# byungsook/neural-flow-style

Measured on AMD Instinct MI355X. Metric: stylization iters/sec on 200^3 smoke grid, 8 views, higher is better.
Workload: dtype f32 (3xbf16 split-limb MFMA, f32 accumulate)

## Files before the change

include/nfs_hip.h:

```cpp
#ifndef NFS_HIP_H
#define NFS_HIP_H

#include <stdint.h>

#ifdef __cplusplus
extern "C" {
#endif

#define NFS_OK 0
#define NFS_EINVAL (-1)
#define NFS_ELAUNCH (-2)

typedef void* nfs_stream_t;

int nfs_version(void);
const char* nfs_last_error(void);
int nfs_device_cus(void);
int nfs_gemm_timer(int enable);

int nfs_gemm_mode(int mode);
int nfs_gemm_force(int variant, int bm, int bn, int nbuf, int pre);
int nfs_gemm_last(long long* out);
int nfs_gemm_timer_read(double* ms_total, double* flops_total, long long* launches);
int nfs_gemm_timer_read_kind(int split_limb, double* ms_total, double* flops_total, long long* launches,
                             double* bytes_total);

int nfs_warp3d_fwd(const float* imgs, const float* coords, float* out,
                   int B, int X, int Y, int Z, int C, nfs_stream_t stream);
int nfs_warp3d_bwd(const float* imgs, const float* coords, const float* g_out,
                   float* g_imgs_acc, float* g_coords,
                   int B, int X, int Y, int Z, int C, nfs_stream_t stream);

int nfs_rotate_fwd(const float* d, const float* rot, float* out,
                   int V, int D, int H, int W, int C, nfs_stream_t stream);
int nfs_rotate_bwd(const float* g_out, const float* rot, float* g_d_acc,
                   int V, int D, int H, int W, int C, float* workspace, const float* g_max,
                   int overwrite, nfs_stream_t stream);

int nfs_advect_fwd(const float* d, const float* vel, float* out,
                   int D, int H, int W, int C, nfs_stream_t stream);
int nfs_advect_bwd(const float* d, const float* vel, const float* g_out,
                   float* g_d_acc, float* g_vel,
                   int D, int H, int W, int C, nfs_stream_t stream);

int nfs_advect_bwd_adam(const float* d, float* vel, const float* g_out, float* m, float* v,
                        int D, int H, int W, float lr_t, float beta1, float beta2, float eps,
                        nfs_stream_t stream);

int nfs_advect_bwd_adam_fwd(const float* d, float* vel, const float* g_out, float* m, float* v, float* adv_next,
                            int D, int H, int W, float lr_t, float beta1, float beta2, float eps,
                            nfs_stream_t stream);

int nfs_advect_fwd_slab(const float* d, const float* vel, float* out, int D, int H, int W, int z0, int nz,
                        nfs_stream_t stream);
int nfs_advect_bwd_adam_slab(const float* d, float* vel, const float* g_out, float* m, float* v,
                             int D, int H, int W, int z0, int nz, float lr_t, float beta1, float beta2, float eps,
                             nfs_stream_t stream);
int nfs_advect_bwd_adam_fwd_slab(const float* d, float* vel, const float* g_out, float* m, float* v, float* adv_next,
                                 int D, int H, int W, int z0, int nz, float lr_t, float beta1, float beta2,
                                 float eps, nfs_stream_t stream);

int nfs_hist_loss(const float* feat, const float* templ, float* loss_acc, float* g_acc,
                  int B, int Bt, int HW, int HWt, int C, float weight, int relu_mask, nfs_stream_t stream);
int nfs_hist_loss_masked(const float* feat, const float* templ, const float* mask, float* loss_acc, float* g_acc,
                         int B, int Bt, int HW, int HWt, int C, float weight, int relu_mask, nfs_stream_t stream);
int64_t nfs_hist_loss_wide_workspace_floats(int B, int C, int HW, int HWt);
int nfs_hist_loss_wide(const float* feat, const float* templ, const float* mask, float* loss_acc, float* g_acc,
                       float* workspace, int64_t workspace_floats, int B, int Bt, int HW, int HWt, int C, float weight,
                       int relu_mask, nfs_stream_t stream);

int nfs_resize_bicubic_tf1(const float* x, float* out, int B, int H, int W, int C, int oh, int ow,
                           nfs_stream_t stream);
int nfs_style_mask_apply(const float* F, const float* mask, float* Fm, float* scale, int B, int HW, int C,
                         nfs_stream_t stream);
int nfs_style_mask_bwd(const float* dFm, const float* mask, const float* F, float* dF, int B, int HW, int C,
                       nfs_stream_t stream);

int nfs_warp2d_fwd(const float* imgs, const float* coords, float* out, int B, int X, int Y, int C,
                   nfs_stream_t stream);
int nfs_warp2d_bwd(const float* imgs, const float* coords, const float* g_out, float* g_imgs_acc,
                   float* g_coords, int B, int X, int Y, int C, nfs_stream_t stream);

int nfs_advect2d_fwd(const float* d, const float* vel, float* out, int H, int W, int C, nfs_stream_t stream);
int nfs_advect2d_bwd(const float* d, const float* vel, const float* g_out, float* g_d_acc, float* g_vel,
                     int H, int W, int C, nfs_stream_t stream);

int nfs_advect_maccormack(const float* d, const float* vel, const float* d_fwd, float* out,
                          int D, int H, int W, int C, int nd, nfs_stream_t stream);
int nfs_maccormack_mask_words(int D, int H, int W, int C);
int nfs_advect_maccormack_keep(const float* d, const float* vel, const float* d_fwd, float* out, unsigned long long* keep,
                               int D, int H, int W, int C, int nd, nfs_stream_t stream);
int64_t nfs_advect_maccormack_bwd_workspace_floats(int D, int H, int W, int C, int nd);
int nfs_advect_maccormack_bwd(const float* d, const float* vel, const float* d_fwd, const unsigned long long* keep,
                              const float* g_out, float* g_d_acc, float* g_vel, float* workspace, int64_t workspace_floats,
                              int D, int H, int W, int C, int nd, nfs_stream_t stream);

int nfs_curl_fwd(const float* s, float* out, int D, int H, int W, int nd, nfs_stream_t stream);
int nfs_curl_bwd(const float* g_out, float* g_s, int D, int H, int W, int nd, nfs_stream_t stream);

int nfs_advect_stream_fwd(const float* d, const float* s, float* out, unsigned long long* live,
                          int D, int H, int W, nfs_stream_t stream);
int nfs_advect_stream_bwd(const float* d, const float* s, const float* g_out, float* g_vel,
                          int D, int H, int W, nfs_stream_t stream);
int nfs_stream_bwd_adam(const float* g_vel, float* s, float* m, float* v, int D, int H, int W,
                        float lr_t, float beta1, float beta2, float eps, nfs_stream_t stream);

int nfs_lap_down(const float* x, const float* k, float* out, int D, int H, int W, int C, int nd, nfs_stream_t stream);
int nfs_lap_up(const float* lo, const float* k, float scale, const float* addend, float* out,
               int D, int H, int W, int C, int nd, nfs_stream_t stream);
int nfs_lap_up_rms_parts(int D, int H, int W, int C, int nd);
int nfs_lap_up_rms(const float* lo, const float* k, float scale, const float* addend, const float* addend_part,
                   int addend_nparts, int64_t addend_n, float eps, float* out, float* out_part, int D, int H, int W, int C,
                   int nd, nfs_stream_t stream);
int nfs_normalize_mean(const float* x, float* out, int64_t n, int use_abs, float eps, float* workspace, int ws_floats,
                       nfs_stream_t stream);

int nfs_transport_step(const float* g, const float* u, float scale, float w_g, const float* addend,
                       float w_addend, float* out, int D, int H, int W, int C, nfs_stream_t stream);

int nfs_smooth3d_relu_fwd(const float* d, float* out, int D, int H, int W, float k,
                          nfs_stream_t stream);
int nfs_smooth3d_relu_bwd(const float* out, const float* g_out, float* g_d,
                          int D, int H, int W, float k, nfs_stream_t stream);

int nfs_render_fwd(const float* d, float* img, float* raysum,
                   int V, int D, int H, int W, float tau, int liquid, nfs_stream_t stream);
int nfs_render_bwd(const float* d, const float* raysum, const float* g_img, float* g_d,
                   int V, int D, int H, int W, float tau, int liquid, float* gmax_out,
                   nfs_stream_t stream);

int nfs_rotate_render_fwd(const float* d, const float* rot, float* img, float* raysum, float* d_rot,
                          int V, int D, int H, int W, float tau, int liquid,
                          nfs_stream_t stream);
int nfs_rotate_render_bwd(const float* d, const float* rot, const float* raysum,
                          const float* g_img, float* g_d_acc,
                          int V, int D, int H, int W, float tau, int liquid,
                          nfs_stream_t stream);

int nfs_render_coef_layout(int V, int D, int H, int W, int* nseg, int* seg_len);
int nfs_rotate_render_fwd_coef(const float* d, const float* rot, float* img, float* raysum, float* u_rot, float* seg,
                               int V, int D, int H, int W, float tau, nfs_stream_t stream);
int nfs_render_ray_coef_bounds(int V, int H, int W);
int nfs_render_ray_coef(const float* g_img, const float* seg, float* ab, float* bounds,
                        int V, int H, int W, float tau, nfs_stream_t stream);
int nfs_rotate_bwd_coef(const float* u_rot, const float* ab, const float* rot, float* g_d_acc,
                        int V, int D, int H, int W, int nseg, int seg_len, const float* bounds, int nbounds,
                        int overwrite, nfs_stream_t stream);

int nfs_live_mask_words(int D, int H, int W);
int nfs_advect_fwd_live(const float* d, const float* vel, float* out, unsigned long long* live,
                        int D, int H, int W, nfs_stream_t stream);
int nfs_advect_bwd_adam_fwd_live(const float* d, float* vel, const float* g_out, float* m, float* v, float* adv_next,
                                 unsigned long long* live_next, int D, int H, int W, float lr_t, float beta1,
                                 float beta2, float eps, nfs_stream_t stream);
int nfs_advect_bwd_adam_fwd_live_ever(const float* d, float* vel, const float* g_out, float* m, float* v, float* adv_next,
                                      unsigned long long* live, unsigned long long* ever, int D, int H, int W,
                                      float lr_t, float beta1, float beta2, float eps, nfs_stream_t stream);
int nfs_rotate_bwd_coef_live(const float* u_rot, const float* ab, const float* rot, float* g_d_acc,
                             int V, int D, int H, int W, int nseg, int seg_len, const float* bounds, int nbounds,
                             int overwrite, const unsigned long long* live, int dilate, int* workspace,
                             nfs_stream_t stream);
int nfs_rotate_live_workspace_ints(int D, int H, int W);

int nfs_maxnorm_fwd(const float* img, float* out, float* gmax, int G, int n,
                    nfs_stream_t stream);
int nfs_maxnorm_bwd(const float* img, const float* gmax, const float* g_out, float* g_img,
                    int G, int n, float* workspace, nfs_stream_t stream);
int nfs_maxnorm_input_fwd(const float* img, float* x, float* gmax, int G, int n, nfs_stream_t stream);
int nfs_maxnorm_input_bwd(const float* img, const float* gmax, const float* g_x, float* g_img, int G, int n,
                          float* workspace, nfs_stream_t stream);


int nfs_loss_net_input_fwd(const float* img, float* d_img, float* x,
                           int B, int H, int W, int Cin, int H2, int W2, nfs_stream_t stream);
int nfs_loss_net_input_bwd(const float* g_x, float* g_img,
                           int B, int H, int W, int Cin, int H2, int W2, nfs_stream_t stream);

int64_t nfs_conv3x3_packed_floats(int Ci, int Co, int kind);
int nfs_conv3x3_pack(const float* w_hwio, float* packed, int Ci, int Co, int kind,
                     nfs_stream_t stream);
int64_t nfs_conv3x3_workspace_floats(int B, int H, int W, int Ci, int Co);
int64_t nfs_conv3x3_relu_bits_words(int B, int H, int W, int Ci, int Co, int pooled);
double nfs_conv3x3_executed_flops(int B, int H, int W, int K, int N, int pooled);
int nfs_conv3x3_fwd(const float* x, const float* packed_fwd, const float* bias, float* y,
                    int B, int H, int W, int Ci, int Co, int relu,
                    float* workspace, int64_t workspace_floats, uint32_t* relu_bits,
                    nfs_stream_t stream);
int nfs_conv3x3_dgrad(const float* gy, const float* packed_dgrad, const float* x_in,
                      const float* addend, float* gx,
                      int B, int H, int W, int Ci, int Co,
                      float* workspace, int64_t workspace_floats, const uint32_t* relu_bits,
                      int addend_unmasked, nfs_stream_t stream);
int nfs_conv3x3_fwd_pool(const float* x, const float* packed_fwd, const float* bias, float* y,
                         float* y_pool, int B, int H, int W, int Ci, int Co, int relu,
                         float* workspace, int64_t workspace_floats, uint32_t* relu_bits,
                         nfs_stream_t stream);
int nfs_conv3x3_dgrad_pool(const float* gy_pool, const float* x_out, const float* packed_dgrad,
                           const float* x_in, const float* addend, float* gx,
                           int B, int H, int W, int Ci, int Co,
                           float* workspace, int64_t workspace_floats, const uint32_t* relu_bits,
                           int addend_unmasked, nfs_stream_t stream);
int nfs_avgpool2_fwd(const float* x, float* y, int B, int H, int W, int C, nfs_stream_t stream);
int nfs_avgpool2_bwd(const float* gy, const float* x, const float* addend, float* gx,
                     int B, int H, int W, int C, nfs_stream_t stream);

int64_t nfs_gram_workspace_floats(int B, int HW, int C);
int nfs_gram_fwd(const float* F, float* G, int B, int HW, int C, const float* scale_dev, float scale,
                 float* workspace, int64_t workspace_floats, nfs_stream_t stream);
int nfs_style_loss_fwd(const float* G, const float* Gs, float* loss_acc, float* Dmat,
                       int B, int Bs, int C, float weight, nfs_stream_t stream);
int nfs_gram_bwd(const float* F, const float* Dmat, float* dF, int B, int HW, int C,
                 const float* scale_dev, float scale, int relu_mask, nfs_stream_t stream);

typedef struct {
  const float* F;
  const float* Gs;
  float* G;
  float* Dmat;
  float* dF;
  int B, Bs, HW, C;
  float scale;
  float weight;
  int relu_mask;
} nfs_gram_layer_t;
int64_t nfs_gram_style_group_workspace_floats(const nfs_gram_layer_t* layers, int n);
int nfs_gram_style_group_parts(const nfs_gram_layer_t* layers, int n);
int nfs_gram_style_group_fwd(const nfs_gram_layer_t* layers, int n, float* loss_parts, float* workspace,
                             int64_t workspace_floats, nfs_stream_t stream);
int nfs_gram_group_bwd(const nfs_gram_layer_t* layers, int n, nfs_stream_t stream);

int nfs_content_loss(const float* F, const float* target, float* loss_acc, float* g_acc, int B, int Bt,
                     int HW, int C, int channel, int mode, float weight, float amp, nfs_stream_t stream);
int nfs_content_loss_signed(const float* F, const float* target, float* loss_acc, float* g_acc, int B, int Bt,
                            int HW, int C, int channel, int mode, float weight, float amp, nfs_stream_t stream);

int64_t nfs_conv2d_packed_floats(int kh, int kw, int Ci, int Co, int transpose);
int nfs_conv2d_pack(const float* w_hwio, float* packed, int kh, int kw, int Ci, int Co, int transpose,
                    nfs_stream_t stream);
int64_t nfs_conv2d_workspace_floats(int B, int H, int W, int Cin, int Cout, int kh, int kw, int stride);
int nfs_conv2d_fwd(const float* x, int ldx, const float* x_mask, int ldm, const float* packed, const float* bias,
                   float* y, int ldy, float* y_pre, int ldp, int B, int H, int W, int Cin, int Cout, int kh, int kw,
                   int stride, int relu, int accumulate, float* workspace, int64_t workspace_floats,
                   nfs_stream_t stream);
typedef struct {
  const float* x;
  const float* x_mask;
  const float* packed;
  const float* bias;
  float* y;
  float* y_pre;
  int ldx, ldm, ldy, ldp;
  int H, W, Cin, Cout, kh, kw;
  int relu, accumulate, sum_with_prev;
} nfs_conv2d_desc_t;
int64_t nfs_conv2d_group_workspace_floats(const nfs_conv2d_desc_t* descs, int n, int B);
int nfs_conv2d_group(const nfs_conv2d_desc_t* descs, int n, int B, float* workspace, int64_t workspace_floats,
                     nfs_stream_t stream);
int nfs_conv2d_dgrad_small(const float* gy, int ldg, const float* y_act, int lda, const float* w_hwio, float* gx,
                           int B, int H, int W, int Ci, int Co, int kh, int kw, int stride, nfs_stream_t stream);
int nfs_maxpool3_fwd(const float* x, float* y, uint8_t* arg, int B, int H, int W, int C, int stride,
                     nfs_stream_t stream);
int nfs_maxpool3_bwd(const float* gy, const uint8_t* arg, float* gx, int B, int H, int W, int C, int stride,
                     int accumulate, const float* relu_of, nfs_stream_t stream);
int nfs_lrn_fwd(const float* x, float* y, float* scale, int64_t npix, int C, int ld, int radius, float bias,
                float alpha, float beta, nfs_stream_t stream);
int nfs_lrn_bwd(const float* x, const float* y, const float* scale, const float* gy, float* gx, int64_t npix, int C,
                int ld, int radius, float alpha, float beta, int accumulate, nfs_stream_t stream);
int nfs_avgpool_valid_fwd(const float* x, float* y, int B, int H, int W, int C, int k, nfs_stream_t stream);
int nfs_avgpool_valid_bwd(const float* gy, float* gx, int B, int H, int W, int C, int k, int accumulate,
                          nfs_stream_t stream);
int nfs_relu_mask_add(const float* g, int ldg, const float* act, int lda, const float* addend, int ldadd, float* out,
                      int ldo, int64_t npix, int C, nfs_stream_t stream);

int nfs_tv_loss(const float* d_img, float* loss_acc, float* g_acc, int B, int H, int W, int C,
                float weight, nfs_stream_t stream);

typedef struct {
  int nd;
  int res[3];
  float domain[3];
  float radius, support, rest_density;
  int nsize, clip, mode;
} nfs_splat_cfg;
int nfs_p2g_fwd(const float* p, const float* attr, const float* pd, float* grid, float* wsum,
                int N, int C, const nfs_splat_cfg* cfg_host, nfs_stream_t stream);
int nfs_p2g_bwd(const float* p, const float* attr, const float* pd, const float* g_grid,
                const float* g_wsum, float* g_p, float* g_attr, float* g_pd,
                int N, int C, const nfs_splat_cfg* cfg_host, nfs_stream_t stream);
int nfs_p2g_wavg_finish(const float* xsum, const float* wsum, float* out, int64_t n, int C,
                        float eps, nfs_stream_t stream);
int nfs_p2g_wavg_bwd(const float* p, const float* attr, const float* xsum, const float* wsum, const float* g_out,
                     float* g_p, float* g_attr, int N, int C, float eps, const nfs_splat_cfg* cfg_host,
                     nfs_stream_t stream);
int nfs_p2g_wavg_finish_bwd(const float* xsum, const float* wsum, const float* g_out,
                            float* g_xsum, float* g_wsum, int64_t n, int C, float eps,
                            nfs_stream_t stream);
int nfs_p2g_has_instance(const nfs_splat_cfg* cfg_host);

int nfs_g2p_fwd(const float* g, const float* p, float* out, int nd, int X, int Y, int Z, int C,
                int64_t N, int cubic, nfs_stream_t stream);

int nfs_adam_tf_step(float* x, float* m, float* v, const float* g, int64_t n,
                     float lr_t, float beta1, float beta2, float eps, nfs_stream_t stream);

int nfs_fill(float* x, float value, int64_t n, nfs_stream_t stream);
int nfs_axpy(float* y, const float* x, float a, int64_t n, nfs_stream_t stream);

int nfs_colour_clamp_gather(const float* var, const long long* order, float* out, int64_t N, int C, nfs_stream_t stream);
int nfs_clamp01_bwd(const float* g, const float* x, float* out, int64_t n, nfs_stream_t stream);
int nfs_colour_clamp_scatter_bwd(const float* g_cc, const long long* order, const float* var, float* g_var, int64_t N,
                                 int C, nfs_stream_t stream);
int nfs_iterate_update(float* x, float* g_opt, int64_t n, nfs_stream_t stream);

int nfs_slab_pack(const float* gpad, float* pack, int D, int64_t plane, int world, int cs, nfs_stream_t stream);

#ifdef __cplusplus
}
#endif
#endif
```

neural-flow-style_amd/_lib.py:

```python
from __future__ import annotations

import ctypes as C
import os
import subprocess

_HERE = os.path.dirname(os.path.abspath(__file__))
LIB_PATH = os.environ.get("NFS_LIB_PATH") or os.path.join(_HERE, "libnfs_hip.so")
CSRC_DIR = os.path.join(_HERE, "csrc")


class NfsLibraryError(RuntimeError):
    pass


NFS_EINVAL, NFS_ELAUNCH = -1, -2


class NfsError(RuntimeError):

    def __init__(self, name, code, msg):
        RuntimeError.__init__(self, "%s failed (%d): %s" % (name, code, msg))
        self.name, self.code = name, int(code)


class SplatCfg(C.Structure):
    _fields_ = [("nd", C.c_int), ("res", C.c_int * 3), ("domain", C.c_float * 3),
                ("radius", C.c_float), ("support", C.c_float), ("rest_density", C.c_float),
                ("nsize", C.c_int), ("clip", C.c_int), ("mode", C.c_int)]


class GramLayer(C.Structure):
    _fields_ = [("F", C.c_void_p), ("Gs", C.c_void_p), ("G", C.c_void_p), ("Dmat", C.c_void_p), ("dF", C.c_void_p),
                ("B", C.c_int), ("Bs", C.c_int), ("HW", C.c_int), ("C", C.c_int),
                ("scale", C.c_float), ("weight", C.c_float), ("relu_mask", C.c_int)]


class ConvDesc(C.Structure):
    _fields_ = [("x", C.c_void_p), ("x_mask", C.c_void_p), ("packed", C.c_void_p), ("bias", C.c_void_p),
                ("y", C.c_void_p), ("y_pre", C.c_void_p),
                ("ldx", C.c_int), ("ldm", C.c_int), ("ldy", C.c_int), ("ldp", C.c_int),
                ("H", C.c_int), ("W", C.c_int), ("Cin", C.c_int), ("Cout", C.c_int), ("kh", C.c_int), ("kw", C.c_int),
                ("relu", C.c_int), ("accumulate", C.c_int), ("sum_with_prev", C.c_int)]


_P, _I, _F, _L = C.c_void_p, C.c_int, C.c_float, C.c_int64

SIGNATURES = {
    "nfs_version": [],
    "nfs_last_error": [],
    "nfs_device_cus": [],
    "nfs_gemm_timer": [_I],
    "nfs_gemm_mode": [_I],
    "nfs_gemm_force": [_I, _I, _I, _I, _I],
    "nfs_gemm_last": [_P],
    "nfs_gemm_timer_read": [_P, _P, _P],
    "nfs_gemm_timer_read_kind": [_I, _P, _P, _P, _P],
    "nfs_warp3d_fwd": [_P, _P, _P, _I, _I, _I, _I, _I, _P],
    "nfs_warp3d_bwd": [_P, _P, _P, _P, _P, _I, _I, _I, _I, _I, _P],
    "nfs_rotate_fwd": [_P, _P, _P, _I, _I, _I, _I, _I, _P],
    "nfs_rotate_bwd": [_P, _P, _P, _I, _I, _I, _I, _I, _P, _P, _I, _P],
    "nfs_advect_fwd": [_P, _P, _P, _I, _I, _I, _I, _P],
    "nfs_advect_bwd": [_P, _P, _P, _P, _P, _I, _I, _I, _I, _P],
    "nfs_advect_bwd_adam": [_P, _P, _P, _P, _P, _I, _I, _I, _F, _F, _F, _F, _P],
    "nfs_advect_fwd_slab": [_P, _P, _P, _I, _I, _I, _I, _I, _P],
    "nfs_advect_bwd_adam_slab": [_P, _P, _P, _P, _P, _I, _I, _I, _I, _I, _F, _F, _F, _F, _P],
    "nfs_advect_bwd_adam_fwd": [_P, _P, _P, _P, _P, _P, _I, _I, _I, _F, _F, _F, _F, _P],
    "nfs_advect_bwd_adam_fwd_slab": [_P, _P, _P, _P, _P, _P, _I, _I, _I, _I, _I, _F, _F, _F, _F, _P],
    "nfs_warp2d_fwd": [_P, _P, _P, _I, _I, _I, _I, _P],
    "nfs_warp2d_bwd": [_P, _P, _P, _P, _P, _I, _I, _I, _I, _P],
    "nfs_advect2d_fwd": [_P, _P, _P, _I, _I, _I, _P],
    "nfs_advect2d_bwd": [_P, _P, _P, _P, _P, _I, _I, _I, _P],
    "nfs_advect_maccormack": [_P, _P, _P, _P, _I, _I, _I, _I, _I, _P],
    "nfs_maccormack_mask_words": [_I, _I, _I, _I],
    "nfs_advect_maccormack_keep": [_P, _P, _P, _P, _P, _I, _I, _I, _I, _I, _P],
    "nfs_advect_maccormack_bwd_workspace_floats": [_I, _I, _I, _I, _I],
    "nfs_advect_maccormack_bwd": [_P, _P, _P, _P, _P, _P, _P, _P, _L, _I, _I, _I, _I, _I, _P],
    "nfs_curl_fwd": [_P, _P, _I, _I, _I, _I, _P],
    "nfs_curl_bwd": [_P, _P, _I, _I, _I, _I, _P],
    "nfs_advect_stream_fwd": [_P, _P, _P, _P, _I, _I, _I, _P],
    "nfs_advect_stream_bwd": [_P, _P, _P, _P, _I, _I, _I, _P],
    "nfs_stream_bwd_adam": [_P, _P, _P, _P, _I, _I, _I, _F, _F, _F, _F, _P],
    "nfs_lap_down": [_P, _P, _P, _I, _I, _I, _I, _I, _P],
    "nfs_lap_up": [_P, _P, _F, _P, _P, _I, _I, _I, _I, _I, _P],
    "nfs_lap_up_rms_parts": [_I, _I, _I, _I, _I],
    "nfs_lap_up_rms": [_P, _P, _F, _P, _P, _I, _L, _F, _P, _P, _I, _I, _I, _I, _I, _P],
    "nfs_normalize_mean": [_P, _P, _L, _I, _F, _P, _I, _P],
    "nfs_transport_step": [_P, _P, _F, _F, _P, _F, _P, _I, _I, _I, _I, _P],
    "nfs_smooth3d_relu_fwd": [_P, _P, _I, _I, _I, _F, _P],
    "nfs_smooth3d_relu_bwd": [_P, _P, _P, _I, _I, _I, _F, _P],
    "nfs_render_fwd": [_P, _P, _P, _I, _I, _I, _I, _F, _I, _P],
    "nfs_render_bwd": [_P, _P, _P, _P, _I, _I, _I, _I, _F, _I, _P, _P],
    "nfs_rotate_render_fwd": [_P, _P, _P, _P, _P, _I, _I, _I, _I, _F, _I, _P],
    "nfs_render_coef_layout": [_I, _I, _I, _I, _P, _P],
    "nfs_rotate_render_fwd_coef": [_P, _P, _P, _P, _P, _P, _I, _I, _I, _I, _F, _P],
    "nfs_render_ray_coef": [_P, _P, _P, _P, _I, _I, _I, _F, _P],
    "nfs_render_ray_coef_bounds": [_I, _I, _I],
    "nfs_rotate_bwd_coef": [_P, _P, _P, _P, _I, _I, _I, _I, _I, _I, _P, _I, _I, _P],
    "nfs_live_mask_words": [_I, _I, _I],
    "nfs_advect_fwd_live": [_P, _P, _P, _P, _I, _I, _I, _P],
    "nfs_advect_bwd_adam_fwd_live": [_P, _P, _P, _P, _P, _P, _P, _I, _I, _I, _F, _F, _F, _F, _P],
    "nfs_advect_bwd_adam_fwd_live_ever": [_P, _P, _P, _P, _P, _P, _P, _P, _I, _I, _I, _F, _F, _F, _F, _P],
    "nfs_rotate_bwd_coef_live": [_P, _P, _P, _P, _I, _I, _I, _I, _I, _I, _P, _I, _I, _P, _I, _P, _P],
    "nfs_rotate_live_workspace_ints": [_I, _I, _I],
    "nfs_rotate_render_bwd": [_P, _P, _P, _P, _P, _I, _I, _I, _I, _F, _I, _P],
    "nfs_maxnorm_fwd": [_P, _P, _P, _I, _I, _P],
    "nfs_maxnorm_bwd": [_P, _P, _P, _P, _I, _I, _P, _P],
    "nfs_maxnorm_input_fwd": [_P, _P, _P, _I, _I, _P],
    "nfs_maxnorm_input_bwd": [_P, _P, _P, _P, _I, _I, _P, _P],
    "nfs_loss_net_input_fwd": [_P, _P, _P, _I, _I, _I, _I, _I, _I, _P],
    "nfs_loss_net_input_bwd": [_P, _P, _I, _I, _I, _I, _I, _I, _P],
    "nfs_conv3x3_packed_floats": [_I, _I, _I],
    "nfs_conv3x3_pack": [_P, _P, _I, _I, _I, _P],
    "nfs_conv3x3_workspace_floats": [_I, _I, _I, _I, _I],
    "nfs_conv3x3_relu_bits_words": [_I, _I, _I, _I, _I, _I],
    "nfs_conv3x3_fwd": [_P, _P, _P, _P, _I, _I, _I, _I, _I, _I, _P, _L, _P, _P],
    "nfs_conv3x3_dgrad": [_P, _P, _P, _P, _P, _I, _I, _I, _I, _I, _P, _L, _P, _I, _P],
    "nfs_conv3x3_fwd_pool": [_P, _P, _P, _P, _P, _I, _I, _I, _I, _I, _I, _P, _L, _P, _P],
    "nfs_conv3x3_dgrad_pool": [_P, _P, _P, _P, _P, _P, _I, _I, _I, _I, _I, _P, _L, _P, _I, _P],
    "nfs_avgpool2_fwd": [_P, _P, _I, _I, _I, _I, _P],
    "nfs_avgpool2_bwd": [_P, _P, _P, _P, _I, _I, _I, _I, _P],
    "nfs_gram_workspace_floats": [_I, _I, _I],
    "nfs_gram_fwd": [_P, _P, _I, _I, _I, _P, _F, _P, _L, _P],
    "nfs_style_loss_fwd": [_P, _P, _P, _P, _I, _I, _I, _F, _P],
    "nfs_content_loss": [_P, _P, _P, _P, _I, _I, _I, _I, _I, _I, _F, _F, _P],
    "nfs_content_loss_signed": [_P, _P, _P, _P, _I, _I, _I, _I, _I, _I, _F, _F, _P],
    "nfs_gram_bwd": [_P, _P, _P, _I, _I, _I, _P, _F, _I, _P],
    "nfs_hist_loss": [_P, _P, _P, _P, _I, _I, _I, _I, _I, _F, _I, _P],
    "nfs_conv3x3_executed_flops": [_I, _I, _I, _I, _I, _I],
    "nfs_conv2d_packed_floats": [_I, _I, _I, _I, _I],
    "nfs_conv2d_pack": [_P, _P, _I, _I, _I, _I, _I, _P],
    "nfs_conv2d_workspace_floats": [_I, _I, _I, _I, _I, _I, _I, _I],
    "nfs_conv2d_fwd": [_P, _I, _P, _I, _P, _P, _P, _I, _P, _I, _I, _I, _I, _I, _I, _I, _I, _I, _I, _I, _P, _L, _P],
    "nfs_conv2d_group_workspace_floats": [_P, _I, _I],
    "nfs_conv2d_group": [_P, _I, _I, _P, _L, _P],
    "nfs_conv2d_dgrad_small": [_P, _I, _P, _I, _P, _P, _I, _I, _I, _I, _I, _I, _I, _I, _P],
    "nfs_maxpool3_fwd": [_P, _P, _P, _I, _I, _I, _I, _I, _P],
    "nfs_maxpool3_bwd": [_P, _P, _P, _I, _I, _I, _I, _I, _I, _P, _P],
    "nfs_lrn_fwd": [_P, _P, _P, _L, _I, _I, _I, _F, _F, _F, _P],
    "nfs_lrn_bwd": [_P, _P, _P, _P, _P, _L, _I, _I, _I, _F, _F, _I, _P],
    "nfs_avgpool_valid_fwd": [_P, _P, _I, _I, _I, _I, _I, _P],
    "nfs_avgpool_valid_bwd": [_P, _P, _I, _I, _I, _I, _I, _I, _P],
    "nfs_relu_mask_add": [_P, _I, _P, _I, _P, _I, _P, _I, _L, _I, _P],
    "nfs_gram_style_group_workspace_floats": [_P, _I],
    "nfs_gram_style_group_parts": [_P, _I],
    "nfs_gram_style_group_fwd": [_P, _I, _P, _P, _L, _P],
    "nfs_gram_group_bwd": [_P, _I, _P],
    "nfs_hist_loss_masked": [_P, _P, _P, _P, _P, _I, _I, _I, _I, _I, _F, _I, _P],
    "nfs_hist_loss_wide_workspace_floats": [_I, _I, _I, _I],
    "nfs_hist_loss_wide": [_P, _P, _P, _P, _P, _P, _L, _I, _I, _I, _I, _I, _F, _I, _P],
    "nfs_resize_bicubic_tf1": [_P, _P, _I, _I, _I, _I, _I, _I, _P],
    "nfs_style_mask_apply": [_P, _P, _P, _P, _I, _I, _I, _P],
    "nfs_style_mask_bwd": [_P, _P, _P, _P, _I, _I, _I, _P],
    "nfs_tv_loss": [_P, _P, _P, _I, _I, _I, _I, _F, _P],
    "nfs_p2g_fwd": [_P, _P, _P, _P, _P, _I, _I, C.POINTER(SplatCfg), _P],
    "nfs_p2g_bwd": [_P, _P, _P, _P, _P, _P, _P, _P, _I, _I, C.POINTER(SplatCfg), _P],
    "nfs_p2g_wavg_finish": [_P, _P, _P, _L, _I, _F, _P],
    "nfs_p2g_wavg_finish_bwd": [_P, _P, _P, _P, _P, _L, _I, _F, _P],
    "nfs_p2g_has_instance": [C.POINTER(SplatCfg)],
    "nfs_p2g_wavg_bwd": [_P, _P, _P, _P, _P, _P, _P, _I, _I, _F, C.POINTER(SplatCfg), _P],
    "nfs_g2p_fwd": [_P, _P, _P, _I, _I, _I, _I, _I, _L, _I, _P],
    "nfs_adam_tf_step": [_P, _P, _P, _P, _L, _F, _F, _F, _F, _P],
    "nfs_fill": [_P, _F, _L, _P],
    "nfs_axpy": [_P, _P, _F, _L, _P],
    "nfs_slab_pack": [_P, _P, _I, _L, _I, _I, _P],
    "nfs_colour_clamp_gather": [_P, _P, _P, _L, _I, _P],
    "nfs_clamp01_bwd": [_P, _P, _P, _L, _P],
    "nfs_colour_clamp_scatter_bwd": [_P, _P, _P, _P, _L, _I, _P],
    "nfs_iterate_update": [_P, _P, _L, _P],
}
_RESTYPE = {"nfs_last_error": C.c_char_p, "nfs_conv3x3_packed_floats": C.c_int64,
            "nfs_conv3x3_workspace_floats": C.c_int64, "nfs_gram_workspace_floats": C.c_int64,
            "nfs_conv3x3_relu_bits_words": C.c_int64, "nfs_gram_style_group_workspace_floats": C.c_int64, "nfs_hist_loss_wide_workspace_floats": C.c_int64,
            "nfs_advect_maccormack_bwd_workspace_floats": C.c_int64,
            "nfs_conv3x3_executed_flops": C.c_double, "nfs_conv2d_packed_floats": C.c_int64,
            "nfs_conv2d_workspace_floats": C.c_int64, "nfs_conv2d_group_workspace_floats": C.c_int64}

_lib = None
ABI_VERSION = 154


def build(verbose=False):
    jobs = os.environ.get("MAX_JOBS") or str(min(os.cpu_count() or 4, 16))
    r = subprocess.run(["make", "-C", CSRC_DIR, "-j", jobs],
                       capture_output=True, text=True)
    if verbose or r.returncode != 0:
        print(r.stdout[-4000:], r.stderr[-4000:])
    if r.returncode != 0:
        raise NfsLibraryError("building libnfs_hip.so failed")
    return LIB_PATH


def lib():
    global _lib
    if _lib is None:
        if not os.path.exists(LIB_PATH):
            raise NfsLibraryError(
                "libnfs_hip.so is missing (%s): run `python -c 'import __graft_entry__ as g; g.build()'` "
                "-- there is no CPU fallback for the product path" % LIB_PATH)
        import torch
        try:
            L = C.CDLL(LIB_PATH)
        except OSError as e:
            raise NfsLibraryError("cannot load %s: %s" % (LIB_PATH, e))
        for name, argt in SIGNATURES.items():
            try:
                f = getattr(L, name)
            except AttributeError:
                raise NfsLibraryError("libnfs_hip.so does not export %s (stale build?)" % name)
            f.argtypes = argt
            f.restype = _RESTYPE.get(name, C.c_int)
        if L.nfs_version() < ABI_VERSION:
            raise NfsLibraryError("libnfs_hip.so reports ABI %d, this binding needs >= %d: rebuild (make -C %s)"
                                  % (L.nfs_version(), ABI_VERSION, CSRC_DIR))
        _lib = L
    return _lib


PROFILE = None


def call(name, *args):
    L = lib()
    if PROFILE is not None:
        import torch
        e0 = torch.cuda.Event(enable_timing=True); e1 = torch.cuda.Event(enable_timing=True)
        e0.record()
        rc = getattr(L, name)(*args)
        e1.record()
        PROFILE.setdefault(name, []).append((e0, e1, args))
    else:
        rc = getattr(L, name)(*args)
    if rc != 0:
        raise NfsError(name, rc, L.nfs_last_error().decode())
    return rc
```

neural-flow-style_amd/csrc/api.hip:

```cpp
#include "common.h"

namespace nfs {
static thread_local char g_err[512] = "";
void set_error(const char* fmt, ...) {
  va_list ap;
  va_start(ap, fmt);
  vsnprintf(g_err, sizeof(g_err), fmt, ap);
  va_end(ap);
}
}

extern "C" {
int nfs_version(void) { return 154; }
const char* nfs_last_error(void) { return nfs::g_err; }
int nfs_device_cus(void) {
  int dev = 0;
  hipDeviceProp_t p;
  if (hipGetDevice(&dev) != hipSuccess || hipGetDeviceProperties(&p, dev) != hipSuccess) {
    nfs::set_error("nfs_device_cus: no HIP device");
    return NFS_ELAUNCH;
  }
  return p.multiProcessorCount;
}
}
```

neural-flow-style_amd/csrc/gram.hip:

```cpp
#include "common.h"

namespace nfs {

typedef float f32x16 __attribute__((ext_vector_type(16)));

struct GramArgs {
  const float* F;
  float* G;
  float* ws;
  const float* scale_dev;
  float scale;
  int B, HW, C;
  int ts;
  int cps;
  int nslab;
  int ntile;
  const float* Gs = nullptr;
  float* Dmat = nullptr;
  float* part = nullptr;
  float weight = 0.f;
  int Bs = 1;
  int slot0 = 0;
};

constexpr int GR_MAXL = 8;
struct GramGroupArgs {
  GramArgs L[GR_MAXL];
  int ustart[GR_MAXL + 1];
  int n;
};

constexpr int GR_KC = 32;

template <int TS>
__device__ __forceinline__ void gram_tn_block(const GramArgs& a, float* smem, int block, int nblocks) {
  constexpr int MT = TS / 64;
  constexpr int J = TS / 32;
  constexpr int R4 = TS / 4;
  float* As = smem;
  float* Bs = smem + 2 * GR_KC * TS;
  const int t = threadIdx.x, lane = t & 63, wid = t >> 6;
  const int wm = wid >> 1, wn = wid & 1, i = lane & 31, h = lane >> 5;
  const int npair = a.ntile * (a.ntile + 1) / 2;
  const int64_t per_xcd = nblocks / 8;
  int64_t unit = (int64_t)(block % 8) * per_xcd + block / 8;
  const int64_t per_img = (int64_t)a.nslab * npair;
  if (unit >= per_img * a.B) return;
  const int b = (int)(unit / per_img);
  unit -= (int64_t)b * per_img;
  const int sl = (int)(unit / npair);
  const int pair = (int)(unit - (int64_t)sl * npair);
  int t1 = 0, t2 = pair;
  while (t2 >= a.ntile - t1) { t2 -= a.ntile - t1; ++t1; }
  t2 += t1;
  const bool diag = t1 == t2;
  const int total_chunks = (a.HW + GR_KC - 1) / GR_KC;
  const int c_begin = sl * a.cps;
  const int nchunks = min(a.cps, total_chunks - c_begin);
  const float* Fb = a.F + (int64_t)b * a.HW * a.C;

  const int col4 = t % R4, row0 = t / R4;
  constexpr int RSTEP = 256 / R4;
  const float* ga = Fb + t1 * TS + 4 * col4;
  const float* gb = Fb + t2 * TS + 4 * col4;
  float4 a0, a1, a2, a3, b0, b1, b2, b3;
#define NFS_GR_LD(dst_, base_, j_, c_)                                                          \
  {                                                                                             \
    const int p_ = (c_begin + (c_)) * GR_KC + row0 + RSTEP * (j_);                              \
    dst_ = make_float4(0.f, 0.f, 0.f, 0.f);                                                     \
    if (p_ < a.HW) dst_ = *reinterpret_cast<const float4*>(base_ + (int64_t)p_ * a.C);          \
  }
#define NFS_GR_LOAD(c_)                                                                         \
  {                                                                                             \
    NFS_GR_LD(a0, ga, 0, c_) NFS_GR_LD(a1, ga, 1, c_)                                           \
    if (J > 2) { NFS_GR_LD(a2, ga, 2, c_) NFS_GR_LD(a3, ga, 3, c_) }                            \
    if (!diag) {                                                                                \
      NFS_GR_LD(b0, gb, 0, c_) NFS_GR_LD(b1, gb, 1, c_)                                         \
      if (J > 2) { NFS_GR_LD(b2, gb, 2, c_) NFS_GR_LD(b3, gb, 3, c_) }                          \
    }                                                                                           \
  }
  b0 = b1 = b2 = b3 = make_float4(0.f, 0.f, 0.f, 0.f);
  a2 = a3 = b0;
  NFS_GR_LOAD(0)

  f32x16 acc[MT][MT];
#pragma unroll
  for (int x = 0; x < MT; ++x)
#pragma unroll
    for (int y = 0; y < MT; ++y)
#pragma unroll
      for (int r = 0; r < 16; ++r) acc[x][y][r] = 0.f;

  const int afrag = h * TS + wm * (TS / 2) + i;
  const int bfrag = h * TS + wn * (TS / 2) + i;
  for (int c = 0; c < nchunks; ++c) {
    float* Ac = As + (c & 1) * GR_KC * TS;
    float* Bc = diag ? Ac : Bs + (c & 1) * GR_KC * TS;
    {
      float* ad = Ac + row0 * TS + 4 * col4;
      *reinterpret_cast<float4*>(ad) = a0;
      *reinterpret_cast<float4*>(ad + RSTEP * TS) = a1;
      if (J > 2) {
        *reinterpret_cast<float4*>(ad + 2 * RSTEP * TS) = a2;
        *reinterpret_cast<float4*>(ad + 3 * RSTEP * TS) = a3;
      }
      if (!diag) {
        float* bd = Bc + row0 * TS + 4 * col4;
        *reinterpret_cast<float4*>(bd) = b0;
        *reinterpret_cast<float4*>(bd + RSTEP * TS) = b1;
        if (J > 2) {
          *reinterpret_cast<float4*>(bd + 2 * RSTEP * TS) = b2;
          *reinterpret_cast<float4*>(bd + 3 * RSTEP * TS) = b3;
        }
      }
    }
    __syncthreads();
    if (c + 1 < nchunks) NFS_GR_LOAD(c + 1)
#pragma unroll
    for (int st = 0; st < GR_KC / 2; ++st) {
      float af[MT], bf[MT];
#pragma unroll
      for (int m = 0; m < MT; ++m) af[m] = Ac[afrag + 2 * st * TS + 32 * m];
#pragma unroll
      for (int n = 0; n < MT; ++n) bf[n] = Bc[bfrag + 2 * st * TS + 32 * n];
#pragma unroll
      for (int n = 0; n < MT; ++n)
#pragma unroll
        for (int m = 0; m < MT; ++m)
          acc[m][n] = __builtin_amdgcn_mfma_f32_32x32x2f32(af[m], bf[n], acc[m][n], 0, 0, 0);
    }
  }
#undef NFS_GR_LOAD
#undef NFS_GR_LD

  constexpr int OS = TS + 4;
  float* otile = smem;
  __syncthreads();
#pragma unroll
  for (int m = 0; m < MT; ++m)
#pragma unroll
    for (int r = 0; r < 16; ++r) {
      const int row = wm * (TS / 2) + m * 32 + (r & 3) + 8 * (r >> 2) + 4 * h;
#pragma unroll
      for (int n = 0; n < MT; ++n) otile[row * OS + wn * (TS / 2) + n * 32 + i] = acc[m][n][r];
    }
  __syncthreads();
  if (a.ws) {
    float* wt = a.ws + (((int64_t)b * npair + pair) * a.nslab + sl) * TS * TS;
#pragma unroll
    for (int e = 0; e < (TS * R4) / 256; ++e) {
      const int f = t + 256 * e;
      const int row = f / R4, q = f - row * R4;
      *reinterpret_cast<float4*>(wt + row * TS + 4 * q) = *reinterpret_cast<const float4*>(otile + row * OS + 4 * q);
    }
    return;
  }
  const float sc = a.scale * (a.scale_dev ? a.scale_dev[b] : 1.f);
  float* Gb = a.G + (int64_t)b * a.C * a.C;
  if (a.nslab == 1 && a.Dmat) {
    const float* Gsb = a.Gs + (int64_t)(b % a.Bs) * a.C * a.C;
    float* Db = a.Dmat + (int64_t)b * a.C * a.C;
    float* Go = a.G ? a.G + (int64_t)b * a.C * a.C : nullptr;
    const float w2 = 2.f * a.weight;
    float lp = 0.f;
    for (int f = t; f < TS * R4; f += 256) {
      const int row = f / R4, q = f - row * R4;
      const int64_t o = (int64_t)(t1 * TS + row) * a.C + t2 * TS + 4 * q;
      float4 v = *reinterpret_cast<const float4*>(otile + row * OS + 4 * q);
      v.x *= sc; v.y *= sc; v.z *= sc; v.w *= sc;
      if (Go) *reinterpret_cast<float4*>(Go + o) = v;
      const float4 g = *reinterpret_cast<const float4*>(Gsb + o);
      const float4 d = make_float4(v.x - g.x, v.y - g.y, v.z - g.z, v.w - g.w);
      lp += (d.x * d.x + d.y * d.y) + (d.z * d.z + d.w * d.w);
      *reinterpret_cast<float4*>(Db + o) = make_float4(w2 * d.x, w2 * d.y, w2 * d.z, w2 * d.w);
    }
    if (!diag)
      for (int f = t; f < TS * R4; f += 256) {
        const int col = f / R4, q = f - col * R4;
        const float4 v = make_float4(otile[(4 * q) * OS + col] * sc, otile[(4 * q + 1) * OS + col] * sc,
                                     otile[(4 * q + 2) * OS + col] * sc, otile[(4 * q + 3) * OS + col] * sc);
        const int64_t o = (int64_t)(t2 * TS + col) * a.C + t1 * TS + 4 * q;
        if (Go) *reinterpret_cast<float4*>(Go + o) = v;
        const float4 g = *reinterpret_cast<const float4*>(Gsb + o);
        *reinterpret_cast<float4*>(Db + o) = make_float4(w2 * (v.x - g.x), w2 * (v.y - g.y), w2 * (v.z - g.z),
                                                         w2 * (v.w - g.w));
      }
    lp = block_sum(lp, smem + TS * OS);
    if (t == 0) a.part[(int64_t)(a.slot0 + pair) * a.B + b] = a.weight * (diag ? lp : 2.f * lp);
    return;
  }
  if (a.nslab == 1) {
    for (int f = t; f < TS * R4; f += 256) {
      const int row = f / R4, q = f - row * R4;
      float4 v = *reinterpret_cast<const float4*>(otile + row * OS + 4 * q);
      v.x *= sc; v.y *= sc; v.z *= sc; v.w *= sc;
      *reinterpret_cast<float4*>(Gb + (int64_t)(t1 * TS + row) * a.C + t2 * TS + 4 * q) = v;
    }
    if (!diag)
      for (int f = t; f < TS * R4; f += 256) {
        const int col = f / R4, q = f - col * R4;
        const float4 v = make_float4(otile[(4 * q) * OS + col] * sc, otile[(4 * q + 1) * OS + col] * sc,
                                     otile[(4 * q + 2) * OS + col] * sc, otile[(4 * q + 3) * OS + col] * sc);
        *reinterpret_cast<float4*>(Gb + (int64_t)(t2 * TS + col) * a.C + t1 * TS + 4 * q) = v;
      }
    return;
  }
  for (int f = t; f < TS * TS; f += 256) {
    const int row = f / TS, col = f - row * TS;
    const float v = otile[row * OS + col] * sc;
    const int gr = t1 * TS + row, gc = t2 * TS + col;
    atomicAdd(Gb + (int64_t)gr * a.C + gc, v);
    if (!diag) atomicAdd(Gb + (int64_t)gc * a.C + gr, v);
  }
}

template <int TS>
__global__ void __launch_bounds__(256, 2) gram_tn_kernel(GramArgs a) {
  extern __shared__ __attribute__((aligned(16))) float smem[];
  gram_tn_block<TS>(a, smem, (int)blockIdx.x, (int)gridDim.x);
}

__global__ void __launch_bounds__(256, 2) gram_tn_group_kernel(GramGroupArgs g) {
  extern __shared__ __attribute__((aligned(16))) float smem[];
  int l = 0;
  while (l + 1 < g.n && (int)blockIdx.x >= g.ustart[l + 1]) ++l;
  gram_tn_block<64>(g.L[l], smem, (int)blockIdx.x - g.ustart[l], g.ustart[l + 1] - g.ustart[l]);
}

constexpr int GRD_ROWS = 4;
__device__ __forceinline__ void gram_reduce_block(const GramArgs& a, int unit) {
  constexpr int TS = 64;
  __shared__ float4 part[4][64];
  __shared__ float tile[GRD_ROWS][TS + 1];
  const int t = threadIdx.x, lane = t & 63, g = t >> 6;
  const int row = lane >> 4, q = lane & 15;
  constexpr int groups = TS / GRD_ROWS;
  const int npair = a.ntile * (a.ntile + 1) / 2;
  const int rg = unit % groups;
  unit /= groups;
  const int pair = unit % npair, b = unit / npair;
  int t1 = 0, t2 = pair;
  while (t2 >= a.ntile - t1) { t2 -= a.ntile - t1; ++t1; }
  t2 += t1;
  const int64_t tsz = (int64_t)TS * TS;
  const float* p = a.ws + (((int64_t)b * npair + pair) * a.nslab) * tsz + (int64_t)(rg * GRD_ROWS + row) * TS + 4 * q;
  float4 s = make_float4(0.f, 0.f, 0.f, 0.f);
  for (int k = g; k < a.nslab; k += 4) {
    const float4 x = *reinterpret_cast<const float4*>(p + (int64_t)k * tsz);
    s.x += x.x; s.y += x.y; s.z += x.z; s.w += x.w;
  }
  part[g][lane] = s;
  __syncthreads();
  if (g > 0) return;
  const float sc = a.scale * (a.scale_dev ? a.scale_dev[b] : 1.f);
  const float4 p1 = part[1][lane], p2 = part[2][lane], p3 = part[3][lane];
  s.x = ((s.x + p1.x) + (p2.x + p3.x)) * sc; s.y = ((s.y + p1.y) + (p2.y + p3.y)) * sc;
  s.z = ((s.z + p1.z) + (p2.z + p3.z)) * sc; s.w = ((s.w + p1.w) + (p2.w + p3.w)) * sc;
  float* Gb = a.G ? a.G + (int64_t)b * a.C * a.C : nullptr;
  const int64_t o = (int64_t)(t1 * TS + rg * GRD_ROWS + row) * a.C + t2 * TS + 4 * q;
  if (Gb) *reinterpret_cast<float4*>(Gb + o) = s;
  const float* Gsb = a.Dmat ? a.Gs + (int64_t)(b % a.Bs) * a.C * a.C : nullptr;
  float* Db = a.Dmat ? a.Dmat + (int64_t)b * a.C * a.C : nullptr;
  const float w2 = 2.f * a.weight;
  if (Db) {
    const float4 gs = *reinterpret_cast<const float4*>(Gsb + o);
    const float4 d = make_float4(s.x - gs.x, s.y - gs.y, s.z - gs.z, s.w - gs.w);
    *reinterpret_cast<float4*>(Db + o) = make_float4(w2 * d.x, w2 * d.y, w2 * d.z, w2 * d.w);
    const float lp = wave_sum((d.x * d.x + d.y * d.y) + (d.z * d.z + d.w * d.w));
    if (lane == 0) a.part[(int64_t)(a.slot0 + pair * groups + rg) * a.B + b] = a.weight * (t1 == t2 ? lp : 2.f * lp);
  }
  if (t1 == t2) return;
  tile[row][4 * q] = s.x; tile[row][4 * q + 1] = s.y; tile[row][4 * q + 2] = s.z; tile[row][4 * q + 3] = s.w;
  __builtin_amdgcn_s_waitcnt(0xc07f);
  __builtin_amdgcn_wave_barrier();
  const float4 v = make_float4(tile[0][lane], tile[1][lane], tile[2][lane], tile[3][lane]);
  const int64_t om = (int64_t)(t2 * TS + lane) * a.C + t1 * TS + rg * GRD_ROWS;
  if (Gb) *reinterpret_cast<float4*>(Gb + om) = v;
  if (Db) {
    const float4 gs = *reinterpret_cast<const float4*>(Gsb + om);
    *reinterpret_cast<float4*>(Db + om) = make_float4(w2 * (v.x - gs.x), w2 * (v.y - gs.y), w2 * (v.z - gs.z),
                                                      w2 * (v.w - gs.w));
  }
}

__global__ void __launch_bounds__(256) gram_reduce_kernel(GramArgs a) { gram_reduce_block(a, (int)blockIdx.x); }

__global__ void __launch_bounds__(256) gram_reduce_group_kernel(GramGroupArgs g) {
  int l = 0;
  while (l + 1 < g.n && (int)blockIdx.x >= g.ustart[l + 1]) ++l;
  gram_reduce_block(g.L[l], (int)blockIdx.x - g.ustart[l]);
}

__global__ void __launch_bounds__(256) style_loss_kernel(const float* __restrict__ G, const float* __restrict__ Gs,
                                                         float* __restrict__ loss, float* __restrict__ Dmat, int B,
                                                         int Bs, int CC, float weight) {
  __shared__ float red[16];
  const int b = blockIdx.y;
  float part = 0.f;
  for (int64_t e = (int64_t)blockIdx.x * blockDim.x + threadIdx.x; e < CC; e += (int64_t)gridDim.x * blockDim.x) {
    const float diff = G[(int64_t)b * CC + e] - Gs[(int64_t)(b % Bs) * CC + e];
    part += weight * diff * diff;
    Dmat[(int64_t)b * CC + e] = 2.f * weight * diff;
  }
  part = block_sum(part, red);
  if (threadIdx.x == 0) atomicAdd(loss + b, part);
}

__global__ void __launch_bounds__(256) content_loss_kernel(const float* __restrict__ F, const float* __restrict__ target,
                                                           float* __restrict__ loss, float* __restrict__ g_acc,
                                                           int B, int Bt, int64_t HWC, int C, int channel, int mode,
                                                           float weight, float amp, int signed_f) {
  __shared__ float red[16];
  const int b = blockIdx.y;
  const float n_all = (float)B * (float)HWC;
  const float n_pix = n_all / (float)C;
  const float c_on = -weight / n_pix;
  const float c_lo = channel > 0 ? weight / (n_pix * (float)channel) : 0.f;
  const float c_hi = channel + 1 < C ? weight / (n_pix * (float)(C - channel - 1)) : 0.f;
  float part = 0.f;
  for (int64_t e = (int64_t)blockIdx.x * blockDim.x + threadIdx.x; e < HWC; e += (int64_t)gridDim.x * blockDim.x) {
    const int64_t i = (int64_t)b * HWC + e;
    const float f = F[i];
    float l, g;
    if (mode == 0) {
      const int ch = (int)(e % C);
      const float k = ch == channel ? c_on : (ch < channel ? c_lo : c_hi);
      if (ch == channel || !signed_f) {
        l = k * f;
        g = k;
      } else {
        l = k * fabsf(f);
        g = f > 0.f ? k : (f < 0.f ? -k : 0.f);
      }
    } else if (mode == 1) {
      l = -weight / n_all * f;
      g = -weight / n_all;
    } else {
      const float diff = f - amp * target[(int64_t)(b % Bt) * HWC + e];
      l = weight / n_all * diff * diff;
      g = 2.f * weight / n_all * diff;
    }
    part += l;
    if (signed_f || f > 0.f) g_acc[i] += g;
  }
  part = block_sum(part, red);
  if (threadIdx.x == 0) atomicAdd(loss + b, part);
}

int gram_bwd_gemm(const float* F, const float* Dm, float* dF, int B, int HW, int C, float alpha, const float* alpha_dev,
                  int relu_mask, int cus, hipStream_t s);
int gram_bwd_gemm_group(const float* const* F, const float* const* Dm, float* const* dF, const int* HW, const int* C,
                        const float* alpha, const int* relu_mask, int n, int B, hipStream_t s);

}

using namespace nfs;

extern "C" {

static int gram_cus() {
  static int cus = 0;
  if (cus == 0) { const int c = nfs_device_cus(); cus = c > 0 ? c : 256; }
  return cus;
}

static void gram_plan(GramArgs& a, int cus) {
  static const int env_cps = [] { const char* e = getenv("NFS_GRAM_CPS"); return e ? atoi(e) : 0; }();
  a.ts = 64;
  a.ntile = a.C / a.ts;
  const int64_t pairs = (int64_t)a.B * a.ntile * (a.ntile + 1) / 2;
  const int total_chunks = (a.HW + GR_KC - 1) / GR_KC;
  int cps = 16;
  while (cps > 4 && pairs * ((total_chunks + cps - 1) / cps) < 2 * (int64_t)cus) cps >>= 1;
  if (cps > total_chunks) cps = total_chunks;
  if ((total_chunks + cps - 1) / cps > 256) cps = (total_chunks + 255) / 256;
  if (pairs >= cus && total_chunks <= 32) cps = total_chunks;
  if (env_cps > 0) cps = env_cps < total_chunks ? env_cps : total_chunks;
  a.cps = cps;
  a.nslab = (total_chunks + cps - 1) / cps;
}

int64_t nfs_gram_workspace_floats(int B, int HW, int C) {
  if (B <= 0 || HW <= 0 || C <= 0 || C % 64) return 0;
  GramArgs a;
  a.B = B; a.HW = HW; a.C = C;
  gram_plan(a, gram_cus());
  return (int64_t)B * (a.ntile * (a.ntile + 1) / 2) * a.nslab * a.ts * a.ts + 4 * 4096;
}

int nfs_gram_fwd(const float* F, float* G, int B, int HW, int C, const float* scale_dev, float scale,
                 float* workspace, int64_t workspace_floats, nfs_stream_t stream) {
  NFS_REQUIRE(F && G, "nfs_gram_fwd: null pointer");
  NFS_REQUIRE(B > 0 && HW > 0, "nfs_gram_fwd: non-positive dimension");
  NFS_REQUIRE(C > 0 && C % 64 == 0, "nfs_gram_fwd: C must be a multiple of 64");
  GramArgs a;
  a.F = F; a.G = G; a.scale_dev = scale_dev; a.scale = scale; a.B = B; a.HW = HW; a.C = C;
  gram_plan(a, gram_cus());
  const int64_t units = (int64_t)B * (a.ntile * (a.ntile + 1) / 2) * a.nslab;
  a.ws = (workspace && workspace_floats >= nfs_gram_workspace_floats(B, HW, C) && a.nslab > 1) ? workspace : nullptr;
  const size_t lds = 4 * GR_KC * 64 * sizeof(float);
  hipLaunchKernelGGL(gram_tn_kernel<64>, dim3((unsigned)((units + 7) / 8 * 8)), dim3(256), lds, as_stream(stream), a);
  if (a.ws) {
    const unsigned rb = (unsigned)((int64_t)B * (a.ntile * (a.ntile + 1) / 2) * (64 / GRD_ROWS));
    hipLaunchKernelGGL(gram_reduce_kernel, dim3(rb), dim3(256), 0, as_stream(stream), a);
  }
  return check_launch("nfs_gram_fwd");
}

struct GramGroupPlan {
  GramGroupArgs tn, rd;
  int tn_blocks, rd_blocks, parts;
  int64_t ws_floats;
};

static int gram_group_plan(const nfs_gram_layer_t* layers, int n, GramGroupPlan& P) {
  if (!layers || n < 1 || n > GR_MAXL) return -1;
  int order[GR_MAXL];
  GramArgs L[GR_MAXL];
  for (int l = 0; l < n; ++l) {
    const nfs_gram_layer_t& y = layers[l];
    if (!y.F || !y.Gs || !y.Dmat || y.B <= 0 || y.Bs <= 0 || y.HW <= 0 || y.C <= 0 || y.C % 64 || y.B != layers[0].B)
      return -1;
    GramArgs& a = L[l];
    a = GramArgs();
    a.F = y.F; a.G = y.G; a.scale_dev = nullptr; a.scale = y.scale; a.B = y.B; a.HW = y.HW; a.C = y.C;
    a.Gs = y.Gs; a.Dmat = y.Dmat; a.weight = y.weight; a.Bs = y.Bs;
    a.ts = 64;
    a.ntile = y.C / 64;
    const int total_chunks = (y.HW + GR_KC - 1) / GR_KC;
    a.cps = total_chunks <= 32 ? total_chunks : 16;
    a.nslab = (total_chunks + a.cps - 1) / a.cps;
    order[l] = l;
  }
  for (int i = 1; i < n; ++i)
    for (int j = i; j > 0 && (L[order[j]].cps > L[order[j - 1]].cps ||
                              (L[order[j]].cps == L[order[j - 1]].cps && L[order[j]].ntile > L[order[j - 1]].ntile)); --j) {
      const int tmp = order[j]; order[j] = order[j - 1]; order[j - 1] = tmp;
    }
  P.tn.n = n;
  P.rd.n = 0;
  int ub = 0, rb = 0, slot = 0;
  int64_t ws = 0;
  for (int k = 0; k < n; ++k) {
    GramArgs a = L[order[k]];
    const int npair = a.ntile * (a.ntile + 1) / 2;
    a.slot0 = slot;
    a.ws = nullptr;
    P.tn.ustart[k] = ub;
    ub += (int)(((int64_t)a.B * npair * a.nslab + 7) / 8 * 8);
    if (a.nslab > 1) {
      a.ws = reinterpret_cast<float*>(ws * sizeof(float));
      ws += (int64_t)a.B * npair * a.nslab * 64 * 64;
      slot += npair * (64 / GRD_ROWS);
      P.rd.ustart[P.rd.n] = rb;
      rb += a.B * npair * (64 / GRD_ROWS);
      P.rd.L[P.rd.n++] = a;
    } else {
      slot += npair;
    }
    P.tn.L[k] = a;
  }
  P.tn.ustart[n] = ub;
  P.rd.ustart[P.rd.n] = rb;
  P.tn_blocks = ub; P.rd_blocks = rb; P.parts = slot; P.ws_floats = ws;
  return 0;
}

int64_t nfs_gram_style_group_workspace_floats(const nfs_gram_layer_t* layers, int n) {
  GramGroupPlan P;
  return gram_group_plan(layers, n, P) == 0 ? P.ws_floats : -1;
}

int nfs_gram_style_group_parts(const nfs_gram_layer_t* layers, int n) {
  GramGroupPlan P;
  return gram_group_plan(layers, n, P) == 0 ? P.parts : -1;
}

int nfs_gram_style_group_fwd(const nfs_gram_layer_t* layers, int n, float* loss_parts, float* workspace,
                             int64_t workspace_floats, nfs_stream_t stream) {
  GramGroupPlan P;
  NFS_REQUIRE(gram_group_plan(layers, n, P) == 0,
              "nfs_gram_style_group_fwd: 1..8 layers with F, Gs, Dmat set, one batch size, C a multiple of 64");
  NFS_REQUIRE(loss_parts, "nfs_gram_style_group_fwd: null loss_parts");
  NFS_REQUIRE(P.ws_floats == 0 || (workspace && workspace_floats >= P.ws_floats),
              "nfs_gram_style_group_fwd: workspace smaller than nfs_gram_style_group_workspace_floats");
  for (int k = 0; k < n; ++k) {
    P.tn.L[k].part = loss_parts;
    if (P.tn.L[k].nslab > 1) P.tn.L[k].ws = workspace + reinterpret_cast<int64_t>(P.tn.L[k].ws) / (int64_t)sizeof(float);
  }
  for (int k = 0; k < P.rd.n; ++k) {
    P.rd.L[k].part = loss_parts;
    P.rd.L[k].ws = workspace + reinterpret_cast<int64_t>(P.rd.L[k].ws) / (int64_t)sizeof(float);
  }
  const size_t lds = 4 * GR_KC * 64 * sizeof(float);
  hipLaunchKernelGGL(gram_tn_group_kernel, dim3((unsigned)P.tn_blocks), dim3(256), lds, as_stream(stream), P.tn);
  if (P.rd_blocks > 0)
    hipLaunchKernelGGL(gram_reduce_group_kernel, dim3((unsigned)P.rd_blocks), dim3(256), 0, as_stream(stream), P.rd);
  return check_launch("nfs_gram_style_group_fwd");
}

int nfs_gram_group_bwd(const nfs_gram_layer_t* layers, int n, nfs_stream_t stream) {
  NFS_REQUIRE(layers && n >= 1 && n <= GR_MAXL, "nfs_gram_group_bwd: 1..8 layers");
  const float* F[GR_MAXL]; const float* Dm[GR_MAXL]; float* dF[GR_MAXL];
  int HW[GR_MAXL], C[GR_MAXL], mask[GR_MAXL];
  float alpha[GR_MAXL];
  for (int l = 0; l < n; ++l) {
    const nfs_gram_layer_t& y = layers[l];
    NFS_REQUIRE(y.F && y.Dmat && y.dF, "nfs_gram_group_bwd: null pointer");
    NFS_REQUIRE(y.B > 0 && y.B == layers[0].B && y.HW > 0 && y.C > 0 && y.C % 64 == 0,
                "nfs_gram_group_bwd: one batch size, C a multiple of 64");
    F[l] = y.F; Dm[l] = y.Dmat; dF[l] = y.dF; HW[l] = y.HW; C[l] = y.C; mask[l] = y.relu_mask; alpha[l] = 2.f * y.scale;
  }
  NFS_REQUIRE(gram_bwd_gemm_group(F, Dm, dF, HW, C, alpha, mask, n, layers[0].B, as_stream(stream)) == 0,
              "nfs_gram_group_bwd: shape outside the 16-row GEMM's 32-bit operand offsets");
  return 0;
}

int nfs_style_loss_fwd(const float* G, const float* Gs, float* loss_acc, float* Dmat, int B, int Bs, int C,
                       float weight, nfs_stream_t stream) {
  NFS_REQUIRE(G && Gs && loss_acc && Dmat, "nfs_style_loss_fwd: null pointer");
  NFS_REQUIRE(B > 0 && Bs > 0 && C > 0, "nfs_style_loss_fwd: non-positive dimension");
  const int CC = C * C;
  const unsigned nb = blocks_for(CC, 256) < 32u ? blocks_for(CC, 256) : 32u;
  hipLaunchKernelGGL(style_loss_kernel, dim3(nb, B), dim3(256), 0, as_stream(stream), G, Gs, loss_acc, Dmat, B, Bs,
                     CC, weight);
  return check_launch("nfs_style_loss_fwd");
}

static int content_loss_launch(const char* who, const float* F, const float* target, float* loss_acc, float* g_acc, int B,
                               int Bt, int HW, int C, int channel, int mode, float weight, float amp, int signed_f,
                               nfs_stream_t stream) {
  NFS_REQUIRE(F && loss_acc && g_acc, "%s: null pointer", who);
  NFS_REQUIRE(B > 0 && HW > 0 && C > 0, "%s: non-positive dimension", who);
  NFS_REQUIRE(mode >= 0 && mode <= 2, "%s: mode must be 0 (channel), 1 (all) or 2 (target)", who);
  NFS_REQUIRE(mode != 0 || (channel > 0 && channel < C), "%s: channel out of range", who);
  NFS_REQUIRE(mode != 2 || (target && Bt > 0), "%s: mode 2 needs the target features", who);
  const int64_t HWC = (int64_t)HW * C;
  const unsigned nb = blocks_for(HWC, 256) < 64u ? blocks_for(HWC, 256) : 64u;
  hipLaunchKernelGGL(content_loss_kernel, dim3(nb, B), dim3(256), 0, as_stream(stream), F, target, loss_acc, g_acc, B,
                     Bt > 0 ? Bt : 1, HWC, C, channel, mode, weight, amp, signed_f);
  return check_launch(who);
}

int nfs_content_loss(const float* F, const float* target, float* loss_acc, float* g_acc, int B, int Bt, int HW, int C,
                     int channel, int mode, float weight, float amp, nfs_stream_t stream) {
  return content_loss_launch("nfs_content_loss", F, target, loss_acc, g_acc, B, Bt, HW, C, channel, mode, weight, amp, 0,
                             stream);
}

int nfs_content_loss_signed(const float* F, const float* target, float* loss_acc, float* g_acc, int B, int Bt, int HW,
                            int C, int channel, int mode, float weight, float amp, nfs_stream_t stream) {
  return content_loss_launch("nfs_content_loss_signed", F, target, loss_acc, g_acc, B, Bt, HW, C, channel, mode, weight,
                             amp, 1, stream);
}

int nfs_gram_bwd(const float* F, const float* Dmat, float* dF, int B, int HW, int C, const float* scale_dev,
                 float scale, int relu_mask, nfs_stream_t stream) {
  NFS_REQUIRE(F && Dmat && dF, "nfs_gram_bwd: null pointer");
  NFS_REQUIRE(B > 0 && HW > 0, "nfs_gram_bwd: non-positive dimension");
  NFS_REQUIRE(C > 0 && C % 64 == 0, "nfs_gram_bwd: C must be a multiple of 64");
  return gram_bwd_gemm(F, Dmat, dF, B, HW, C, 2.f * scale, scale_dev, relu_mask, gram_cus(), as_stream(stream));
}

}
```

neural-flow-style_amd/csrc/render.hip:

```cpp
#include "common.h"

namespace nfs {

__global__ void __launch_bounds__(256) render_fwd_kernel(const float* __restrict__ d, float* __restrict__ img,
                                                         float* __restrict__ raysum, int V, int D, int HW, float tau,
                                                         int liquid) {
  const int64_t gid = (int64_t)blockIdx.x * blockDim.x + threadIdx.x;
  if (gid >= (int64_t)V * HW) return;
  const int v = (int)(gid / HW);
  const int px = (int)(gid - (int64_t)v * HW);
  const float* col = d + (int64_t)v * D * HW + px;
  if (liquid >= 2) {
    float m = -INFINITY, sum = 0.f;
#pragma unroll 4
    for (int z = 0; z < D; ++z) {
      const float s = col[(int64_t)z * HW];
      m = fmaxf(m, s);
      sum += s;
    }
    img[gid] = liquid == 2 ? m : sum / (float)D;
    if (raysum) raysum[gid] = liquid == 2 ? m : sum;
    return;
  }
  float acc = 0.f, I = 0.f;
// ... 533 lines not shown
  const float corr = s / (m * m) / ties;
  for (int i = blockIdx.x * blockDim.x + threadIdx.x; i < n; i += gridDim.x * blockDim.x) {
    float g = gy[i] / m;
    if (x[i] == m) g -= corr;
    gx[i] = g;
  }
}

__constant__ float kInputMean[3] = {0.485f * 255.f, 0.456f * 255.f, 0.406f * 255.f};

__global__ void __launch_bounds__(256) maxnorm_input_kernel(const float* __restrict__ img, const float* __restrict__ gmax,
                                                            float* __restrict__ xo, int n) {
  const float m = gmax[blockIdx.y];
  const float* x = img + (int64_t)blockIdx.y * n;
  float* o = xo + (int64_t)blockIdx.y * n * 3;
  for (int i = blockIdx.x * blockDim.x + threadIdx.x; i < n; i += gridDim.x * blockDim.x) {
    const float v = __fmul_rn(x[i] / m, 255.f);
    o[3 * (int64_t)i] = __fsub_rn(v, kInputMean[0]);
    o[3 * (int64_t)i + 1] = __fsub_rn(v, kInputMean[1]);
    o[3 * (int64_t)i + 2] = __fsub_rn(v, kInputMean[2]);
  }
}

__global__ void __launch_bounds__(256) maxnorm_input_allmax_kernel(const float* __restrict__ img, float* __restrict__ gmax,
                                                                   float* __restrict__ xo, int n) {
  __shared__ float red[16];
  const float* x = img + (int64_t)blockIdx.y * n;
  float* o = xo + (int64_t)blockIdx.y * n * 3;
  float m = -INFINITY;
  const int n4 = n >> 2;
  if ((reinterpret_cast<uintptr_t>(x) & 15) == 0) {
    const float4* x4 = reinterpret_cast<const float4*>(x);
    for (int i = threadIdx.x; i < n4; i += 256) {
      const float4 v = x4[i];
      m = fmaxf(m, fmaxf(fmaxf(v.x, v.y), fmaxf(v.z, v.w)));
    }
    for (int i = 4 * n4 + threadIdx.x; i < n; i += 256) m = fmaxf(m, x[i]);
  } else {
    for (int i = threadIdx.x; i < n; i += 256) m = fmaxf(m, x[i]);
  }
  m = block_max(m, red);
  if (blockIdx.x == 0 && threadIdx.x == 0) gmax[blockIdx.y] = m;
  for (int i = blockIdx.x * blockDim.x + threadIdx.x; i < n; i += gridDim.x * blockDim.x) {
    const float v = __fmul_rn(x[i] / m, 255.f);
    o[3 * (int64_t)i] = __fsub_rn(v, kInputMean[0]);
    o[3 * (int64_t)i + 1] = __fsub_rn(v, kInputMean[1]);
    o[3 * (int64_t)i + 2] = __fsub_rn(v, kInputMean[2]);
  }
}

__global__ void __launch_bounds__(1024) maxnorm_input_small_kernel(const float* __restrict__ img, float* __restrict__ gmax,
                                                                   float* __restrict__ xo, int n) {
  __shared__ float red[16];
  const float* x = img + (int64_t)blockIdx.x * n;
  float* o = xo + (int64_t)blockIdx.x * n * 3;
  float m = -INFINITY;
  for (int i = threadIdx.x; i < n; i += blockDim.x) m = fmaxf(m, x[i]);
  m = block_max(m, red);
  if (threadIdx.x == 0) gmax[blockIdx.x] = m;
  for (int i = threadIdx.x; i < n; i += blockDim.x) {
    const float v = __fmul_rn(x[i] / m, 255.f);
    o[3 * (int64_t)i] = __fsub_rn(v, kInputMean[0]);
    o[3 * (int64_t)i + 1] = __fsub_rn(v, kInputMean[1]);
    o[3 * (int64_t)i + 2] = __fsub_rn(v, kInputMean[2]);
  }
}

__device__ __forceinline__ float input_grad_sum(const float* g, int64_t i) {
  return __fadd_rn(__fadd_rn(__fmul_rn(g[3 * i], 255.f), __fmul_rn(g[3 * i + 1], 255.f)), __fmul_rn(g[3 * i + 2], 255.f));
}

__global__ void __launch_bounds__(256) maxnorm_input_bwd_part_kernel(const float* __restrict__ img,
                                                                     const float* __restrict__ gmax,
                                                                     const float* __restrict__ g_x,
                                                                     float* __restrict__ part, int n) {
  __shared__ float red[16];
  const float* x = img + (int64_t)blockIdx.y * n;
  const float* gx = g_x + (int64_t)blockIdx.y * n * 3;
  const float m = gmax[blockIdx.y];
  float s = 0.f, ties = 0.f;
  for (int i = blockIdx.x * blockDim.x + threadIdx.x; i < n; i += gridDim.x * blockDim.x) {
    const float xi = x[i];
    s += input_grad_sum(gx, i) * xi;
    ties += (xi == m) ? 1.f : 0.f;
  }
  s = block_sum(s, red);
  ties = block_sum(ties, red);
  if (threadIdx.x == 0) {
    part[((int64_t)blockIdx.y * MN_NB + blockIdx.x) * 2] = s;
    part[((int64_t)blockIdx.y * MN_NB + blockIdx.x) * 2 + 1] = ties;
  }
}

__global__ void __launch_bounds__(256) maxnorm_input_bwd_apply_kernel(const float* __restrict__ img,
                                                                      const float* __restrict__ gmax,
                                                                      const float* __restrict__ g_x,
                                                                      const float* __restrict__ part,
                                                                      float* __restrict__ g_img, int n) {
  const float* x = img + (int64_t)blockIdx.y * n;
  const float* gx = g_x + (int64_t)blockIdx.y * n * 3;
  float* go = g_img + (int64_t)blockIdx.y * n;
  const float m = gmax[blockIdx.y];
  float s = 0.f, ties = 0.f;
#pragma unroll 8
  for (int k = 0; k < MN_NB; ++k) {
    s += part[((int64_t)blockIdx.y * MN_NB + k) * 2];
    ties += part[((int64_t)blockIdx.y * MN_NB + k) * 2 + 1];
  }
  const float corr = s / (m * m) / ties;
  for (int i = blockIdx.x * blockDim.x + threadIdx.x; i < n; i += gridDim.x * blockDim.x) {
    float g = input_grad_sum(gx, i) / m;
    if (x[i] == m) g -= corr;
    go[i] = g;
  }
}

__global__ void __launch_bounds__(1024) maxnorm_fwd_kernel(const float* __restrict__ img, float* __restrict__ out,
                                                           float* __restrict__ gmax, int n) {
  __shared__ float red[16];
  const float* x = img + (int64_t)blockIdx.x * n;
  float* o = out + (int64_t)blockIdx.x * n;
  float m = -INFINITY;
  for (int i = threadIdx.x; i < n; i += blockDim.x) m = fmaxf(m, x[i]);
  m = block_max(m, red);
  if (threadIdx.x == 0) gmax[blockIdx.x] = m;
  for (int i = threadIdx.x; i < n; i += blockDim.x) o[i] = x[i] / m;
}

__global__ void __launch_bounds__(1024) maxnorm_bwd_kernel(const float* __restrict__ img,
                                                           const float* __restrict__ gmax,
                                                           const float* __restrict__ g_out,
                                                           float* __restrict__ g_img, int n) {
  __shared__ float red[16];
  const float* x = img + (int64_t)blockIdx.x * n;
  const float* gy = g_out + (int64_t)blockIdx.x * n;
  float* gx = g_img + (int64_t)blockIdx.x * n;
  const float m = gmax[blockIdx.x];
  float s = 0.f, ties = 0.f;
  for (int i = threadIdx.x; i < n; i += blockDim.x) {
    const float xi = x[i];
    s += gy[i] * xi;
    ties += (xi == m) ? 1.f : 0.f;
  }
  s = block_sum(s, red);
  ties = block_sum(ties, red);
  const float corr = s / (m * m) / ties;
  for (int i = threadIdx.x; i < n; i += blockDim.x) {
    float g = gy[i] / m;
    if (x[i] == m) g -= corr;
    gx[i] = g;
  }
}

__global__ void __launch_bounds__(256) render_ray_coef_kernel(const float* __restrict__ g_img,
                                                              const float* __restrict__ seg, float2* __restrict__ ab,
                                                              int V, int HW, float tau, float* __restrict__ bounds) {
  __shared__ float red[16];
  const int64_t total = (int64_t)V * HW, gid = (int64_t)blockIdx.x * blockDim.x + threadIdx.x;
  float bound = 0.f;
  if (gid < total) {
    const int v = (int)(gid / HW), px = (int)(gid - (int64_t)v * HW);
    const int64_t plane = (int64_t)V * RR_SEG * HW, at0 = (int64_t)v * RR_SEG * HW + px;
    const float ntau = -tau * 1.44269504088896341f, g = g_img[gid];
    float S[RR_SEG], Is[RR_SEG], um[RR_SEG], E[RR_SEG], F[RR_SEG];
    float P = 0.f, Itot = 0.f;
#pragma unroll
    for (int s2 = 0; s2 < RR_SEG; ++s2) {
      S[s2] = seg[at0 + (int64_t)s2 * HW];
      Is[s2] = seg[plane + at0 + (int64_t)s2 * HW];
      um[s2] = seg[2 * plane + at0 + (int64_t)s2 * HW];
      E[s2] = __builtin_amdgcn_exp2f(P * ntau);
      F[s2] = Itot;
      Itot = fmaf(E[s2], Is[s2], Itot);
      P += S[s2];
    }
#pragma unroll
    for (int s2 = 0; s2 < RR_SEG; ++s2) {
      const float A = g * E[s2], B = g * tau * (Itot - F[s2]);
      ab[at0 + (int64_t)s2 * HW] = make_float2(A, B);
      bound = fmaxf(bound, fmaf(fabsf(A), um[s2], fabsf(B)));
    }
  }
  bound = block_max(bound, red);
  if (threadIdx.x == 0) bounds[blockIdx.x] = bound > 0.f ? fminf(bound, 3.0e38f) : 0.f;
}

}

using namespace nfs;

extern "C" {

int nfs_render_fwd(const float* d, float* img, float* raysum, int V, int D, int H, int W, float tau, int liquid,
                   nfs_stream_t stream) {
  NFS_REQUIRE(d && img, "nfs_render_fwd: null pointer");
  NFS_REQUIRE(V > 0 && D > 0 && H > 0 && W > 0, "nfs_render_fwd: non-positive dimension");
  NFS_REQUIRE(liquid >= 0 && liquid <= 3, "nfs_render_fwd: mode must be 0 (transmittance), 1 (liquid), 2 (max) or 3 (mean)");
  const int64_t n = (int64_t)V * H * W;
  hipLaunchKernelGGL(render_fwd_kernel, dim3(blocks_for(n, 256)), dim3(256), 0, as_stream(stream), d, img, raysum, V, D,
                     H * W, tau, liquid);
  return check_launch("nfs_render_fwd");
}

extern "C++" {
template <int NSEG>
__global__ void __launch_bounds__(64 * NSEG) render_bwd_seg_kernel(const float* d, const float* __restrict__ raysum,
                                                                   const float* __restrict__ g_img, float* g_d, int V,
                                                                   int D, int HW, float tau,
                                                                   unsigned* __restrict__ gmax_bits) {
  __shared__ float seg_S[NSEG][64], seg_R[NSEG][64], red[16];
  const int lane = threadIdx.x & 63, seg = threadIdx.x >> 6;
  const int64_t total_rays = (int64_t)V * HW;
  const int64_t gid_raw = (int64_t)blockIdx.x * 64 + lane;
  const bool live = gid_raw < total_rays;
  const int64_t gid = live ? gid_raw : total_rays - 1;
  const int v = (int)(gid / HW);
  const int px = (int)(gid - (int64_t)v * HW);
  const int64_t base = (int64_t)v * D * HW + px;
  const float total = raysum[gid], g = g_img[gid];
  const float ntau = -tau * 1.44269504088896341f;
  const int L = (D + NSEG - 1) / NSEG;
  const int zlo = min(seg * L, D), zhi = min(zlo + L, D);
  float S = 0.f, R = 0.f;
#pragma unroll 4
  for (int z = zlo; z < zhi; ++z) {
    const float sv = d[base + (int64_t)z * HW];
    R = fmaf(sv, __builtin_amdgcn_exp2f((total - S) * ntau), R);
    S += sv;
  }
  seg_S[seg][lane] = S;
  seg_R[seg][lane] = R;
  __syncthreads();
  float p0 = 0.f, P = 0.f;
  for (int j = 0; j < seg; ++j) {
    P = fmaf(__builtin_amdgcn_exp2f(-p0 * ntau), seg_R[j][lane], P);
    p0 += seg_S[j][lane];
  }
  float prefix = p0, amax = 0.f;
#pragma unroll 4
  for (int z = zlo; z < zhi; ++z) {
    const float sv = d[base + (int64_t)z * HW];
    const float T = __builtin_amdgcn_exp2f((total - prefix) * ntau);
    P = fmaf(sv, T, P);
    const float o = g * (T - tau * P);
    if (live) g_d[base + (int64_t)z * HW] = o;
    amax = fmaxf(amax, fabsf(o));
    prefix += sv;
  }
  if (gmax_bits) {
    amax = block_max(live ? amax : 0.f, red);
    if (threadIdx.x == 0 && amax > 0.f) atomicMax(gmax_bits, __float_as_uint(fminf(amax, 3.0e38f)));
  }
}
}

int nfs_render_bwd(const float* d, const float* raysum, const float* g_img, float* g_d, int V, int D, int H, int W,
                   float tau, int liquid, float* gmax_out, nfs_stream_t stream) {
  NFS_REQUIRE(d && raysum && g_img && g_d, "nfs_render_bwd: null pointer");
  NFS_REQUIRE(V > 0 && D > 0 && H > 0 && W > 0, "nfs_render_bwd: non-positive dimension");
  const int64_t n = (int64_t)V * H * W;
  if (gmax_out) zero_words(gmax_out, 1, as_stream(stream));
  static const bool no_seg = getenv("NFS_RB_NOSEG") != nullptr;
  NFS_REQUIRE(liquid >= 0 && liquid <= 3, "nfs_render_bwd: mode must be 0 (transmittance), 1 (liquid), 2 (max) or 3 (mean)");
  if (!liquid && !no_seg && D >= 4 * RR_SEG && (int64_t)V * D * H * W <= ((int64_t)16 << 20)) {
    static const int seg_env = getenv("NFS_RB_SEG") ? atoi(getenv("NFS_RB_SEG")) : 0;
    const int64_t blocks = blocks_for(n, 64);
    int nseg = blocks >= 2048 ? 4 : 8;
    if (seg_env == 4 || seg_env == 8 || seg_env == 16) nseg = seg_env;
    while (nseg > 4 && D < 4 * nseg) nseg /= 2;
    unsigned* gm = reinterpret_cast<unsigned*>(gmax_out);
    if (nseg == 16)
      hipLaunchKernelGGL(render_bwd_seg_kernel<16>, dim3(blocks), dim3(1024), 0, as_stream(stream), d, raysum, g_img, g_d,
                         V, D, H * W, tau, gm);
    else if (nseg == 8)
      hipLaunchKernelGGL(render_bwd_seg_kernel<8>, dim3(blocks), dim3(512), 0, as_stream(stream), d, raysum, g_img, g_d,
                         V, D, H * W, tau, gm);
    else
      hipLaunchKernelGGL(render_bwd_seg_kernel<4>, dim3(blocks), dim3(256), 0, as_stream(stream), d, raysum, g_img, g_d,
                         V, D, H * W, tau, gm);
    return check_launch("nfs_render_bwd(segmented)");
  }
  hipLaunchKernelGGL(render_bwd_kernel, dim3(blocks_for(n, 256)), dim3(256), 0, as_stream(stream), d, raysum, g_img, g_d,
                     V, D, H * W, tau, liquid, reinterpret_cast<unsigned*>(gmax_out));
  return check_launch("nfs_render_bwd");
}

int nfs_rotate_render_fwd(const float* d, const float* rot, float* img, float* raysum, float* d_rot, int V, int D,
                          int H, int W, float tau, int liquid, nfs_stream_t stream) {
  NFS_REQUIRE(d && rot && img, "nfs_rotate_render_fwd: null pointer");
  NFS_REQUIRE(V > 0 && D > 0 && H > 0 && W > 0, "nfs_rotate_render_fwd: non-positive dimension");
  NFS_REQUIRE(liquid == 0 || liquid == 1, "nfs_rotate_render_fwd: ray modes 2 / 3 go through nfs_rotate_fwd + nfs_render_fwd");
  const int64_t n = (int64_t)V * H * W;
  static const bool no_seg = getenv("NFS_RR_NOSEG") != nullptr;
  static const bool no_reuse = getenv("NFS_RR_NOREUSE") != nullptr;
  static const int tile_env = getenv("NFS_RR_TILE") ? atoi(getenv("NFS_RR_TILE")) : -1;
  if (W >= 2 && H >= 2 && D >= 4 * RR_SEG && (int64_t)D * H * W < (1ll << 31) && !no_seg) {
    const int lxb = tile_env >= 0 ? tile_env : (W >= 16 && H >= 4 ? 4 : 0);
    static const int band = getenv("NFS_RR_BAND") ? atoi(getenv("NFS_RR_BAND")) : 1;
    int64_t waves = blocks_for(n, 64);
    const int64_t tiles_v = (int64_t)((W + (1 << lxb) - 1) >> lxb) * ((H + (64 >> lxb) - 1) / (64 >> lxb));
    if (lxb) waves = (int64_t)V * tiles_v;
    if (lxb && band) waves = (int64_t)V * ((tiles_v + 7) / 8) * 8;
    const dim3 grid((waves + 7) / 8 * 8);
    const bool fits32 = (int64_t)V * D * H * W < (1ll << 30);
    if (fits32 && !no_reuse)
      hipLaunchKernelGGL(rotate_render_fwd_seg_kernel<true>, grid, dim3(256), 0, as_stream(stream), d, rot, img,
                         raysum, d_rot, V, D, H, W, tau, liquid, lxb, lxb ? band : 0);
    else
      hipLaunchKernelGGL(rotate_render_fwd_seg_kernel<false>, grid, dim3(256), 0, as_stream(stream), d, rot, img,
                         raysum, d_rot, V, D, H, W, tau, liquid, lxb, lxb ? band : 0);
  } else
    hipLaunchKernelGGL(rotate_render_fwd_kernel, dim3(blocks_for(n, 256)), dim3(256), 0, as_stream(stream), d, rot,
                       img, raysum, d_rot, V, D, H, W, tau, liquid);
  return check_launch("nfs_rotate_render_fwd");
}

int nfs_render_coef_layout(int V, int D, int H, int W, int* nseg, int* seg_len) {
  NFS_REQUIRE(V > 0 && D > 0 && H > 0 && W > 0, "nfs_render_coef_layout: non-positive dimension");
  if (nseg) *nseg = RR_SEG;
  if (seg_len) *seg_len = (D + RR_SEG - 1) / RR_SEG;
  const bool ok = W >= 2 && H >= 2 && D >= 4 * RR_SEG && (int64_t)D * H * W < (1ll << 31) &&
                  (int64_t)V * D * H * W < (1ll << 30);
  if (!ok) {
    set_error("nfs_render_coef_layout: shape outside the segmented forward (needs D >= 16, H, W >= 2, V*D*H*W < 2^30)");
    return NFS_EINVAL;
  }
  return NFS_OK;
}

int nfs_rotate_render_fwd_coef(const float* d, const float* rot, float* img, float* raysum, float* u_rot, float* seg,
                               int V, int D, int H, int W, float tau, nfs_stream_t stream) {
  NFS_REQUIRE(d && rot && img && u_rot && seg, "nfs_rotate_render_fwd_coef: null pointer");
  if (int e = nfs_render_coef_layout(V, D, H, W, nullptr, nullptr)) return e;
  const int lxb = W >= 16 && H >= 4 ? 4 : 0;
  int64_t waves = blocks_for((int64_t)V * H * W, 64);
  const int64_t tiles_v = (int64_t)((W + (1 << lxb) - 1) >> lxb) * ((H + (64 >> lxb) - 1) / (64 >> lxb));
  if (lxb) waves = (int64_t)V * ((tiles_v + 7) / 8) * 8;
  hipLaunchKernelGGL((rotate_render_fwd_seg_kernel<true, true>), dim3((waves + 7) / 8 * 8), dim3(256), 0,
                     as_stream(stream), d, rot, img, raysum, u_rot, V, D, H, W, tau, 0, lxb, lxb ? 1 : 0, seg);
  return check_launch("nfs_rotate_render_fwd_coef");
}

int nfs_render_ray_coef_bounds(int V, int H, int W) {
  if (V <= 0 || H <= 0 || W <= 0) return 0;
  return (int)blocks_for((int64_t)V * H * W, 256);
}

int nfs_render_ray_coef(const float* g_img, const float* seg, float* ab, float* bounds, int V, int H, int W, float tau,
                        nfs_stream_t stream) {
  NFS_REQUIRE(g_img && seg && ab && bounds, "nfs_render_ray_coef: null pointer");
  NFS_REQUIRE(V > 0 && H > 0 && W > 0, "nfs_render_ray_coef: non-positive dimension");
  const int64_t n = (int64_t)V * H * W;
  hipLaunchKernelGGL(render_ray_coef_kernel, dim3(blocks_for(n, 256)), dim3(256), 0, as_stream(stream), g_img, seg,
                     reinterpret_cast<float2*>(ab), V, H * W, tau, bounds);
  return check_launch("nfs_render_ray_coef");
}

int nfs_rotate_render_bwd(const float* d, const float* rot, const float* raysum, const float* g_img, float* g_d_acc,
                          int V, int D, int H, int W, float tau, int liquid, nfs_stream_t stream) {
  NFS_REQUIRE(d && rot && raysum && g_img && g_d_acc, "nfs_rotate_render_bwd: null pointer");
  NFS_REQUIRE(V > 0 && D > 0 && H > 0 && W > 0, "nfs_rotate_render_bwd: non-positive dimension");
  NFS_REQUIRE(liquid == 0 || liquid == 1, "nfs_rotate_render_bwd: ray modes 2 / 3 go through nfs_render_bwd + nfs_rotate_bwd");
  const int64_t n = (int64_t)V * H * W;
  hipLaunchKernelGGL(rotate_render_bwd_kernel, dim3(blocks_for(n, 256)), dim3(256), 0, as_stream(stream), d, rot, raysum,
                     g_img, g_d_acc, V, D, H, W, tau, liquid);
  return check_launch("nfs_rotate_render_bwd");
}

int nfs_maxnorm_fwd(const float* img, float* out, float* gmax, int G, int n, nfs_stream_t stream) {
  NFS_REQUIRE(img && out && gmax, "nfs_maxnorm_fwd: null pointer");
  NFS_REQUIRE(G > 0 && n > 0, "nfs_maxnorm_fwd: non-positive size");
  if (n >= 16384) {
    hipLaunchKernelGGL(maxnorm_init_kernel, dim3((G + 63) / 64), dim3(64), 0, as_stream(stream), gmax, G);
    hipLaunchKernelGGL(maxnorm_max_kernel, dim3(MN_NB, G), dim3(256), 0, as_stream(stream), img, gmax, n);
    hipLaunchKernelGGL(maxnorm_div_kernel, dim3(MN_NB, G), dim3(256), 0, as_stream(stream), img, gmax, out, n);
    return check_launch("nfs_maxnorm_fwd(multi-block)");
  }
  hipLaunchKernelGGL(maxnorm_fwd_kernel, dim3(G), dim3(1024), 0, as_stream(stream), img, out, gmax, n);
  return check_launch("nfs_maxnorm_fwd");
}

int nfs_maxnorm_input_fwd(const float* img, float* x, float* gmax, int G, int n, nfs_stream_t stream) {
  NFS_REQUIRE(img && x && gmax, "nfs_maxnorm_input_fwd: null pointer");
  NFS_REQUIRE(G > 0 && n > 0, "nfs_maxnorm_input_fwd: non-positive size");
  if (n < 16384) {
    hipLaunchKernelGGL(maxnorm_input_small_kernel, dim3(G), dim3(1024), 0, as_stream(stream), img, gmax, x, n);
    return check_launch("nfs_maxnorm_input_fwd");
  }
  static const bool three = [] { const char* e = getenv("NFS_MAXNORM_3K"); return e && atoi(e) != 0; }();
  if (!three && (int64_t)n <= (1 << 20)) {
    hipLaunchKernelGGL(maxnorm_input_allmax_kernel, dim3(MN_NB, G), dim3(256), 0, as_stream(stream), img, gmax, x, n);
    return check_launch("nfs_maxnorm_input_fwd(one launch)");
  }
  hipLaunchKernelGGL(maxnorm_init_kernel, dim3((G + 63) / 64), dim3(64), 0, as_stream(stream), gmax, G);
  hipLaunchKernelGGL(maxnorm_max_kernel, dim3(MN_NB, G), dim3(256), 0, as_stream(stream), img, gmax, n);
  hipLaunchKernelGGL(maxnorm_input_kernel, dim3(MN_NB, G), dim3(256), 0, as_stream(stream), img, gmax, x, n);
  return check_launch("nfs_maxnorm_input_fwd");
}

int nfs_maxnorm_input_bwd(const float* img, const float* gmax, const float* g_x, float* g_img, int G, int n,
                          float* workspace, nfs_stream_t stream) {
  NFS_REQUIRE(img && gmax && g_x && g_img && workspace, "nfs_maxnorm_input_bwd: null pointer");
  NFS_REQUIRE(G > 0 && n > 0, "nfs_maxnorm_input_bwd: non-positive size");
  hipLaunchKernelGGL(maxnorm_input_bwd_part_kernel, dim3(MN_NB, G), dim3(256), 0, as_stream(stream), img, gmax, g_x,
                     workspace, n);
  hipLaunchKernelGGL(maxnorm_input_bwd_apply_kernel, dim3(MN_NB, G), dim3(256), 0, as_stream(stream), img, gmax, g_x,
                     workspace, g_img, n);
  return check_launch("nfs_maxnorm_input_bwd");
}

int nfs_maxnorm_bwd(const float* img, const float* gmax, const float* g_out, float* g_img, int G, int n,
                    float* workspace, nfs_stream_t stream) {
  NFS_REQUIRE(img && gmax && g_out && g_img, "nfs_maxnorm_bwd: null pointer");
  NFS_REQUIRE(G > 0 && n > 0, "nfs_maxnorm_bwd: non-positive size");
  if (workspace && n >= 16384) {
    hipLaunchKernelGGL(maxnorm_bwd_part_kernel, dim3(MN_NB, G), dim3(256), 0, as_stream(stream), img, gmax, g_out,
                       workspace, n);
    hipLaunchKernelGGL(maxnorm_bwd_apply_kernel, dim3(MN_NB, G), dim3(256), 0, as_stream(stream), img, gmax, g_out,
                       workspace, g_img, n);
    return check_launch("nfs_maxnorm_bwd(multi-block)");
  }
  hipLaunchKernelGGL(maxnorm_bwd_kernel, dim3(G), dim3(1024), 0, as_stream(stream), img, gmax, g_out, g_img, n);
  return check_launch("nfs_maxnorm_bwd");
}

}
```

neural-flow-style_amd/csrc/vgg.hip:

```cpp
#include "common.h"

#include <mutex>
#include <stdlib.h>

namespace nfs {

int64_t winograd_workspace_floats(int B, int H, int W, int K, int N);
int64_t winograd_packed_floats(int Ci, int Co);
int winograd_path(int B, int H, int W, int K, int N);
int winograd_tile();
int64_t winograd5_bits_words(int B, int H, int W, int C);
int winograd_pack(const float* w_hwio, float* up, int Ci, int Co, int kind, hipStream_t s);
int winograd_conv(const float* x, const float* U, const float* aux0, const float* aux1, float* y, float* ws, int B,
                  int H, int W, int K, int N, int mode, int relu, int cus, hipStream_t s, float* ypool,
                  const float* xmask, uint32_t* in_bits, uint32_t* out_bits, bool pooled_grad);
static inline bool winograd_eligible(int K, int N) {
  static const int min_ch = [] { const char* e = getenv("NFS_WINOGRAD_MIN_CH"); return e ? atoi(e) : 64; }();
  return K >= min_ch && N >= min_ch && K % 32 == 0 && N % 64 == 0;
}

typedef float f32x16 __attribute__((ext_vector_type(16)));

constexpr int KC = 32;
constexpr int LDS_STRIDE = 36;
// ... 260 lines not shown
    const int k = 2 * s2 + h;
#pragma unroll
    for (int nt = 0; nt < 2; ++nt) bfr[s2][nt] = k < 27 ? w[k * 64 + nt * 32 + i] : 0.f;
  }
  float bv2[2];
#pragma unroll
  for (int nt = 0; nt < 2; ++nt) bv2[nt] = bias ? bias[nt * 32 + i] : 0.f;
  const int ntiles_all = B * tiles_x * tiles_y;
  for (int tile_id = blockIdx.x; tile_id < ntiles_all; tile_id += gridDim.x) {
  const int tx = tile_id % tiles_x, ty = (tile_id / tiles_x) % tiles_y, b = tile_id / (tiles_x * tiles_y);
  const int y0 = ty * C3F_TH, x0 = tx * C3F_TW;
  for (int e = t; e < (C3F_TH + 2) * C3F_PW * 3; e += 256) {
    const int r = e / (C3F_PW * 3), rem = e - r * (C3F_PW * 3);
    const int c = rem / 3, ci = rem - c * 3;
    const int gy_ = y0 - 1 + r, gx_ = x0 - 1 + c;
    float v = 0.f;
    if (gy_ >= 0 && gy_ < H && gx_ >= 0 && gx_ < W) v = x[(((int64_t)b * H + gy_) * W + gx_) * 3 + ci];
    patch[e] = v;
  }
  __syncthreads();
  const int m = wid * 32 + i;
  const int base = ((m / C3F_TW) * C3F_PW + (m % C3F_TW)) * 3;
  f32x16 acc[2];
#pragma unroll
  for (int nt = 0; nt < 2; ++nt)
#pragma unroll
    for (int r = 0; r < 16; ++r) acc[nt][r] = 0.f;
#pragma unroll
  for (int s2 = 0; s2 < 14; ++s2) {
    const int k = 2 * s2 + h;
    const int ky = k / 9, kx = (k / 3) % 3, ci = k % 3;
    const float av = k < 27 ? patch[base + (ky * C3F_PW + kx) * 3 + ci] : 0.f;
    acc[0] = __builtin_amdgcn_mfma_f32_32x32x2f32(av, bfr[s2][0], acc[0], 0, 0, 0);
    acc[1] = __builtin_amdgcn_mfma_f32_32x32x2f32(av, bfr[s2][1], acc[1], 0, 0, 0);
  }
#pragma unroll
  for (int nt = 0; nt < 2; ++nt) {
    const float bv = bv2[nt];
#pragma unroll
    for (int r = 0; r < 16; ++r) {
      const int row = wid * 32 + (r & 3) + 8 * (r >> 2) + 4 * h;
      float v = acc[nt][r] + bv;
      if (relu) v = fmaxf(v, 0.f);
      otile[row * C3F_OS + nt * 32 + i] = v;
    }
  }
  __syncthreads();
  for (int f = t; f < C3F_TH * C3F_TW * 16; f += 256) {
    const int row = f >> 4, q = f & 15;
    const int gy_ = y0 + row / C3F_TW, gx_ = x0 + row % C3F_TW;
    if (gy_ < H && gx_ < W)
      *reinterpret_cast<float4*>(y + (((int64_t)b * H + gy_) * W + gx_) * 64 + 4 * q) =
          *reinterpret_cast<const float4*>(otile + row * C3F_OS + 4 * q);
  }
  __syncthreads();
  }
}

__global__ void __launch_bounds__(256) conv3x3_c3_fwd_kernel(const float* __restrict__ x, const float* __restrict__ w,
                                                             const float* __restrict__ bias, float* __restrict__ y,
                                                             int B, int H, int W, int Co, int relu) {
  extern __shared__ __attribute__((aligned(16))) float sw[];
  for (int k = threadIdx.x; k < 27 * Co; k += blockDim.x) sw[k] = w[k];
  __syncthreads();
  const int CQ = Co >> 2;
  const int64_t gid = (int64_t)blockIdx.x * blockDim.x + threadIdx.x;
  if (gid >= (int64_t)B * H * W * CQ) return;
  const int cq = (int)(gid % CQ);
  const int64_t pix = gid / CQ;
  const int xx = (int)(pix % W);
  const int yy = (int)((pix / W) % H);
  float4 acc = bias ? *reinterpret_cast<const float4*>(bias + 4 * cq) : make_float4(0.f, 0.f, 0.f, 0.f);
#pragma unroll
  for (int dy = -1; dy <= 1; ++dy) {
    if (yy + dy < 0 || yy + dy >= H) continue;
#pragma unroll
    for (int dx = -1; dx <= 1; ++dx) {
      if (xx + dx < 0 || xx + dx >= W) continue;
      const float* xp = x + (pix + (int64_t)dy * W + dx) * 3;
      const int tap = (dy + 1) * 3 + dx + 1;
#pragma unroll
      for (int ci = 0; ci < 3; ++ci) {
        const float xv = xp[ci];
        const float4 wv = *reinterpret_cast<const float4*>(sw + (tap * 3 + ci) * Co + 4 * cq);
        acc.x += xv * wv.x; acc.y += xv * wv.y; acc.z += xv * wv.z; acc.w += xv * wv.w;
      }
    }
  }
  if (relu) { acc.x = fmaxf(acc.x, 0.f); acc.y = fmaxf(acc.y, 0.f); acc.z = fmaxf(acc.z, 0.f); acc.w = fmaxf(acc.w, 0.f); }
  *reinterpret_cast<float4*>(y + pix * Co + 4 * cq) = acc;
}

constexpr int C3D_TH = 14, C3D_TW = 14, C3D_PH = C3D_TH + 2, C3D_PW = C3D_TW + 2, C3D_M = 256, C3D_TS = 33;
__global__ void __launch_bounds__(256) conv3x3_c3co64_dgrad_kernel(const float* __restrict__ gy,
                                                                   const float* __restrict__ wd,
                                                                   float* __restrict__ gx, int B, int H, int W,
                                                                   int tiles_x, int tiles_y) {
  __shared__ float Tt[C3D_M * C3D_TS];
  const int t = threadIdx.x, lane = t & 63, wid = t >> 6, i = lane & 31, h = lane >> 5;
  float bw[8][4];
#pragma unroll
  for (int j = 0; j < 8; ++j)
#pragma unroll
    for (int u = 0; u < 4; ++u) bw[j][u] = i < 27 ? wd[((i / 3) * 64 + 8 * j + 4 * h + u) * 3 + i % 3] : 0.f;
  const int ntiles_all = B * tiles_x * tiles_y;
  for (int tile_id = blockIdx.x; tile_id < ntiles_all; tile_id += gridDim.x) {
  const int tx = tile_id % tiles_x, ty = (tile_id / tiles_x) % tiles_y, b = tile_id / (tiles_x * tiles_y);
  const int y0 = ty * C3D_TH, x0 = tx * C3D_TW;
  constexpr int ntile = C3D_PH * C3D_PW / 128;
  static_assert(ntile * 128 == C3D_M && C3D_PH * C3D_PW == C3D_M, "the halo'd tile must fill whole M tiles");
  const int tile0 = ntile * wid;
  for (int mt = 0; mt < ntile; ++mt) {
    const int q = (tile0 + mt) * 32 + i;
    const int qy = y0 - 1 + q / C3D_PW, qx = x0 - 1 + q % C3D_PW;
    const bool ok = qy >= 0 && qy < H && qx >= 0 && qx < W;
    const float* gp = gy + (((int64_t)b * H + (ok ? qy : 0)) * W + (ok ? qx : 0)) * 64 + 4 * h;
    float4 av[8];
#pragma unroll
    for (int j = 0; j < 8; ++j) av[j] = ok ? *reinterpret_cast<const float4*>(gp + 8 * j) : make_float4(0.f, 0.f, 0.f, 0.f);
    f32x16 acc;
#pragma unroll
    for (int r = 0; r < 16; ++r) acc[r] = 0.f;
#pragma unroll
    for (int j = 0; j < 8; ++j) {
      acc = __builtin_amdgcn_mfma_f32_32x32x2f32(av[j].x, bw[j][0], acc, 0, 0, 0);
      acc = __builtin_amdgcn_mfma_f32_32x32x2f32(av[j].y, bw[j][1], acc, 0, 0, 0);
      acc = __builtin_amdgcn_mfma_f32_32x32x2f32(av[j].z, bw[j][2], acc, 0, 0, 0);
      acc = __builtin_amdgcn_mfma_f32_32x32x2f32(av[j].w, bw[j][3], acc, 0, 0, 0);
    }
#pragma unroll
    for (int r = 0; r < 16; ++r) {
      const int row = (tile0 + mt) * 32 + (r & 3) + 8 * (r >> 2) + 4 * h;
      Tt[row * C3D_TS + i] = acc[r];
    }
  }
  __syncthreads();
  if (t < C3D_TH * C3D_TW) {
    const int ly = t / C3D_TW, lx = t % C3D_TW;
    const int py = y0 + ly, px = x0 + lx;
    if (py < H && px < W) {
      float o0 = 0.f, o1 = 0.f, o2 = 0.f;
#pragma unroll
      for (int dy = 0; dy < 3; ++dy)
#pragma unroll
        for (int dx = 0; dx < 3; ++dx) {
          const float* tp = Tt + ((ly + dy) * C3D_PW + lx + dx) * C3D_TS + (dy * 3 + dx) * 3;
          o0 += tp[0]; o1 += tp[1]; o2 += tp[2];
        }
      float* o = gx + (((int64_t)b * H + py) * W + px) * 3;
      o[0] = o0; o[1] = o1; o[2] = o2;
    }
  }
  __syncthreads();
  }
}

__global__ void __launch_bounds__(256) conv3x3_c3_dgrad_kernel(const float* __restrict__ gy,
                                                               const float* __restrict__ wp, float* __restrict__ gx,
                                                               int B, int H, int W, int Co) {
  extern __shared__ __attribute__((aligned(16))) float sw[];
  for (int k = threadIdx.x; k < 27 * Co; k += blockDim.x) sw[k] = wp[k];
  __syncthreads();
  const int64_t pix = (int64_t)blockIdx.x * blockDim.x + threadIdx.x;
  if (pix >= (int64_t)B * H * W) return;
  const int xx = (int)(pix % W);
  const int yy = (int)((pix / W) % H);
  float a0 = 0.f, a1 = 0.f, a2 = 0.f;
  for (int dy = -1; dy <= 1; ++dy) {
    if (yy + dy < 0 || yy + dy >= H) continue;
    for (int dx = -1; dx <= 1; ++dx) {
      if (xx + dx < 0 || xx + dx >= W) continue;
      const float4* gp = reinterpret_cast<const float4*>(gy + (pix + (int64_t)dy * W + dx) * Co);
      const float* ws = sw + ((dy + 1) * 3 + dx + 1) * Co * 3;
      for (int c4 = 0; c4 < (Co >> 2); ++c4) {
        const float4 g = gp[c4];
        const float* wq = ws + c4 * 12;
        a0 += g.x * wq[0] + g.y * wq[3] + g.z * wq[6] + g.w * wq[9];
        a1 += g.x * wq[1] + g.y * wq[4] + g.z * wq[7] + g.w * wq[10];
        a2 += g.x * wq[2] + g.y * wq[5] + g.z * wq[8] + g.w * wq[11];
      }
    }
  }
  gx[pix * 3] = a0; gx[pix * 3 + 1] = a1; gx[pix * 3 + 2] = a2;
}

__global__ void __launch_bounds__(256) pack_kernel(const float* __restrict__ w, float* __restrict__ wp, int Ci, int Co,
                                                   int kind) {
  const int64_t gid = (int64_t)blockIdx.x * blockDim.x + threadIdx.x;
  if (gid >= (int64_t)9 * Ci * Co) return;
  if (Ci == 3) {
    if (kind == 0) { wp[gid] = w[gid]; return; }
    const int ci = (int)(gid % 3);
    const int co = (int)((gid / 3) % Co);
    const int tp = (int)(gid / (3 * Co));
    wp[gid] = w[((int64_t)(8 - tp) * 3 + ci) * Co + co];
    return;
  }
  const int Nc = kind == 0 ? Co : Ci;
  const int kc = (int)(gid % KC);
  const int n = (int)((gid / KC) % Nc);
  const int tap = (int)((gid / ((int64_t)KC * Nc)) % 9);
  const int chunk = (int)(gid / ((int64_t)KC * Nc * 9));
  float v;
  if (kind == 0) v = w[((int64_t)tap * Ci + chunk * KC + kc) * Co + n];
  else v = w[((int64_t)(8 - tap) * Ci + n) * Co + chunk * KC + kc];
  wp[gid] = v;
}

static void pick_tile(int B, int H, int W, int& TH, int& TW, int& tiles_r, int& tiles_c) {
  double best = -1.0;
  const int rows = B * H;
  for (int tw = 4; tw <= 128 && tw <= ((W + 3) / 4) * 4; ++tw) {
    const int twc = tw > W ? W : tw;
    int th = BM / twc;
    if (th > rows) th = rows;
    if (th < 1) continue;
    while (th > 1 && (th + 2) * (twc + 2) > PATCH_MAX) --th;
    if ((th + 2) * (twc + 2) > PATCH_MAX) continue;
    const int tr = (rows + th - 1) / th, tcn = (W + twc - 1) / twc;
    const double eff = (double)rows * W / ((double)tr * tcn * BM);
    if (eff > best + 1e-9) { best = eff; TH = th; TW = twc; tiles_r = tr; tiles_c = tcn; }
  }
}

static int g_cus = 0;
static int device_cus() {
  if (g_cus == 0) {
    int c = nfs_device_cus();
    g_cus = c > 0 ? c : 256;
  }
  return g_cus;
}

struct ConvPlan { int bn, ksplit; };
static ConvPlan plan_conv(int mtiles, int Nc, int nchunks, int64_t mn, int64_t ws_floats) {
  const int cus = device_cus();
  ConvPlan best{64, 1};
  double best_t = 1e30;
  for (int bn = 64; bn <= 128; bn += 64) {
    if (Nc % bn) continue;
    const int slots = cus * (bn == 64 ? 3 : 2);
    const double unit = bn == 64 ? 0.55 : 1.0;
    for (int ks = 1; ks <= nchunks && ks <= 16; ++ks) {
      if (ks > 1 && (int64_t)ks * mn > ws_floats) break;
      const int64_t blocks = (int64_t)mtiles * (Nc / bn) * ks;
      const double rounds = (double)((blocks + slots - 1) / slots);
      const int steps = ((nchunks + ks - 1) / ks) * 9 + 3;
      double tms = rounds * steps * unit * 1.9e-3 * (slots / (double)cus) / 2.0;
      if (ks > 1) tms += (double)(ks + 1) * mn * 4.0 / 4.0e9 + 2.5e-3;
      if (tms < best_t) { best_t = tms; best = ConvPlan{bn, ks}; }
    }
  }
  return best;
}

static bool takes_winograd(const ConvArgs& a, const float* ws, int64_t ws_floats) {
  static const bool no_wg = getenv("NFS_NO_WINOGRAD") != nullptr;
  return !no_wg && winograd_eligible(a.Kc, a.Nc) && a.H >= 2 && a.W >= 2 && ws &&
         ws_floats >= winograd_workspace_floats(a.B, a.H, a.W, a.Kc, a.Nc);
}

static bool takes_fused_pool(const ConvArgs& a, const float* ws, int64_t ws_floats) {
  static const bool tile4 = [] { const char* e = getenv("NFS_WINOGRAD_TILE"); return !(e && atoi(e) == 2); }();
  static const bool off = getenv("NFS_NO_POOL_FUSION") != nullptr;
  return tile4 && !off && takes_winograd(a, ws, ws_floats);
}

template <int MODE>
static int launch_conv(const ConvArgs& base, float* ws, int64_t ws_floats, hipStream_t s, float* ypool = nullptr,
                       const float* xmask = nullptr, uint32_t* in_bits = nullptr, uint32_t* out_bits = nullptr,
                       bool pooled_grad = false) {
  ConvArgs a = base;
  if (takes_winograd(a, ws, ws_floats)) {
    const float* U = a.wp + (int64_t)9 * a.Kc * a.Nc;
    const bool cache = takes_fused_pool(a, ws, ws_floats);
    return winograd_conv(a.x, U, a.aux0, a.aux1, a.y, ws, a.B, a.H, a.W, a.Kc, a.Nc, MODE, a.relu, device_cus(), s,
                         ypool, xmask, cache ? in_bits : nullptr, cache ? out_bits : nullptr, pooled_grad);
  }
  NFS_REQUIRE(!ypool && !xmask && !pooled_grad, "conv3x3: fused pooling needs the Winograd path");
  int tiles_r = 0;
  a.TH = 0;
  pick_tile(a.B, a.H, a.W, a.TH, a.TW, tiles_r, a.tiles_c);
  NFS_REQUIRE(a.TH > 0, "conv3x3: no valid tile for %dx%dx%d", a.B, a.H, a.W);
  const int mtiles = tiles_r * a.tiles_c;
  const int64_t mn = (int64_t)a.B * a.H * a.W * a.Nc;
  const ConvPlan plan = plan_conv(mtiles, a.Nc, a.Kc / KC, mn, ws ? ws_floats : 0);
  a.ksplit = plan.ksplit;
  a.ws = ws;
#ifdef NFS_ABLATE
  static const int dbg = getenv("NFS_CONV_DBG") ? atoi(getenv("NFS_CONV_DBG")) : 0;
  a.dbg = dbg;
#endif
  const dim3 grid(mtiles, a.Nc / plan.bn, plan.ksplit);
  if (plan.bn == 128) {
    constexpr int BN = 128;
    const size_t oper = PATCH_MAX * LDS_STRIDE + 2 * BN * LDS_STRIDE, tile = BM * (BN + 4);
    const size_t lds = (oper > tile ? oper : tile) * sizeof(float) + BM * sizeof(int);
    static std::once_flag attr_once;
    std::call_once(attr_once, [&] {
      (void)hipFuncSetAttribute(reinterpret_cast<const void*>(conv3x3_mfma_kernel<BN, MODE>),
                          hipFuncAttributeMaxDynamicSharedMemorySize, (int)lds); });
    hipLaunchKernelGGL((conv3x3_mfma_kernel<BN, MODE>), grid, dim3(256), lds, s, a);
  } else {
    constexpr int BN = 64;
    const size_t oper = PATCH_MAX * LDS_STRIDE + 2 * BN * LDS_STRIDE, tile = BM * (BN + 4);
    const size_t lds = (oper > tile ? oper : tile) * sizeof(float) + BM * sizeof(int);
    hipLaunchKernelGGL((conv3x3_mfma_kernel<BN, MODE>), grid, dim3(256), lds, s, a);
  }
  if (plan.ksplit > 1)
    hipLaunchKernelGGL(conv_reduce_kernel<MODE>, dim3(blocks_for(mn / 4, 256)), dim3(256), 0, s, a, mn);
  return check_launch(MODE == 0 ? "nfs_conv3x3_fwd" : "nfs_conv3x3_dgrad");
}

}

using namespace nfs;

extern "C" {

int64_t nfs_conv3x3_packed_floats(int Ci, int Co, int kind) {
  if (Ci <= 0 || Co <= 0) return 0;
  const int K = kind == 0 ? Ci : Co, N = kind == 0 ? Co : Ci;
  return (int64_t)9 * Ci * Co + (winograd_eligible(K, N) ? winograd_packed_floats(Ci, Co) : 0);
}

int nfs_conv3x3_pack(const float* w_hwio, float* packed, int Ci, int Co, int kind, nfs_stream_t stream) {
  NFS_REQUIRE(w_hwio && packed, "nfs_conv3x3_pack: null pointer");
  NFS_REQUIRE(kind == 0 || kind == 1, "nfs_conv3x3_pack: kind must be 0 or 1");
  NFS_REQUIRE(Ci == 3 || (Ci % 64 == 0), "nfs_conv3x3_pack: Ci must be 3 or a multiple of 64");
  NFS_REQUIRE(Co % 64 == 0, "nfs_conv3x3_pack: Co must be a multiple of 64");
  const int64_t n = (int64_t)9 * Ci * Co;
  hipLaunchKernelGGL(pack_kernel, dim3(blocks_for(n, 256)), dim3(256), 0, as_stream(stream), w_hwio, packed, Ci, Co,
                     kind);
  const int K = kind == 0 ? Ci : Co, N = kind == 0 ? Co : Ci;
  if (winograd_eligible(K, N))
    if (int e = winograd_pack(w_hwio, packed + n, Ci, Co, kind, as_stream(stream))) return e;
  return check_launch("nfs_conv3x3_pack");
}

int64_t nfs_conv3x3_workspace_floats(int B, int H, int W, int Ci, int Co) {
  if (B <= 0 || H <= 0 || W <= 0 || Ci <= 0 || Co <= 0) return 0;
  if (winograd_eligible(Ci, Co) && winograd_eligible(Co, Ci) && H >= 2 && W >= 2)
    return winograd_workspace_floats(B, H, W, Ci > Co ? Ci : Co, Ci > Co ? Ci : Co);
  const int64_t n = Ci > Co ? Ci : Co;
  const int64_t want = (int64_t)16 * B * H * W * n;
  return want < ((int64_t)32 << 20) ? want : ((int64_t)32 << 20);
}

int64_t nfs_conv3x3_relu_bits_words(int B, int H, int W, int Ci, int Co, int pooled) {
  if (B <= 0 || H < 2 || W < 2 || Ci <= 0 || Co <= 0 || Ci % 64 || Co % 64) return 0;
  static const bool off = getenv("NFS_NO_RELU_BITS") != nullptr;
  ConvArgs a{nullptr, nullptr, nullptr, nullptr, nullptr, nullptr, B, H, W, Ci, Co, 0, 0, 0, 1, 1, 0};
  float dummy = 0.f;
  if (off || !takes_fused_pool(a, &dummy, INT64_MAX)) return 0;
  if (!pooled && winograd_path(B, H, W, Ci, Co) == 2) return winograd5_bits_words(B, H, W, Ci);
  const int64_t T = (int64_t)B * ((H + 3) / 4) * ((W + 3) / 4);
  return T * (Ci / 2) + (pooled ? T * (Co / 2) : 0);
}

double nfs_conv3x3_executed_flops(int B, int H, int W, int K, int N, int pooled) {
  if (B <= 0 || H <= 0 || W <= 0 || K <= 0 || N <= 0) return 0.0;
  static const bool no_wg = getenv("NFS_NO_WINOGRAD") != nullptr;
  const double direct = 2.0 * B * H * W * 9.0 * K * N;
  if (no_wg || !winograd_eligible(K, N) || H < 2 || W < 2) return direct;
  const int m = winograd_tile();
  if (m == 4 && !pooled && winograd_path(B, H, W, K, N) == 2)
    return 2.0 * 49.0 * B * ((H + 4) / 5) * ((W + 4) / 5) * (double)K * N;
  return 2.0 * (m + 2) * (m + 2) * B * ((H + m - 1) / m) * ((W + m - 1) / m) * (double)K * N;
}

static inline uint32_t* out_bits_of(uint32_t* relu_bits, int B, int H, int W, int Ci) {
  return relu_bits ? relu_bits + (int64_t)B * ((H + 3) / 4) * ((W + 3) / 4) * (Ci / 2) : nullptr;
}

int nfs_conv3x3_fwd(const float* x, const float* packed_fwd, const float* bias, float* y, int B, int H, int W, int Ci,
                    int Co, int relu, float* workspace, int64_t workspace_floats, uint32_t* relu_bits,
                    nfs_stream_t stream) {
  NFS_REQUIRE(x && packed_fwd && y, "nfs_conv3x3_fwd: null pointer");
  NFS_REQUIRE(B > 0 && H > 0 && W > 0, "nfs_conv3x3_fwd: non-positive dimension");
  NFS_REQUIRE((int64_t)B * H * W < ((int64_t)1 << 31) / 4, "nfs_conv3x3_fwd: too many pixels");
  NFS_REQUIRE(Co > 0 && Co % 64 == 0, "nfs_conv3x3_fwd: Co must be a multiple of 64");
  static const bool old_c3 = getenv("NFS_C3_OLD") != nullptr;
  if (Ci == 3 && Co == 64 && !old_c3) {
    const int tiles_x = (W + C3F_TW - 1) / C3F_TW, tiles_y = (H + C3F_TH - 1) / C3F_TH;
    static const int per_cu = [] { const char* e = getenv("NFS_C3F_BLOCKS"); return e ? atoi(e) : 4; }();
    const int64_t ntiles = (int64_t)B * tiles_x * tiles_y, cap = 256 * (int64_t)per_cu;
    hipLaunchKernelGGL(conv3x3_c3co64_fwd_kernel, dim3((unsigned)(per_cu > 0 && ntiles > cap ? cap : ntiles)), dim3(256), 0,
                       as_stream(stream), x, packed_fwd, bias, y, B, H, W, relu, tiles_x, tiles_y);
    return check_launch("nfs_conv3x3_fwd(c3, Co=64, MFMA)");
  }
  if (Ci == 3) {
    const int64_t n = (int64_t)B * H * W * (Co / 4);
    hipLaunchKernelGGL(conv3x3_c3_fwd_kernel, dim3(blocks_for(n, 256)), dim3(256), 27 * Co * sizeof(float),
                       as_stream(stream), x, packed_fwd, bias, y, B, H, W, Co, relu);
    return check_launch("nfs_conv3x3_fwd(c3)");
  }
  NFS_REQUIRE(Ci > 0 && Ci % 32 == 0, "nfs_conv3x3_fwd: Ci must be 3 or a multiple of 32");
  ConvArgs a{x, packed_fwd, bias, nullptr, y, nullptr, B, H, W, Ci, Co, 0, 0, 0, relu, 1, 0};
  return launch_conv<0>(a, workspace, workspace_floats, as_stream(stream), nullptr, nullptr, relu_bits, nullptr);
}

int nfs_conv3x3_dgrad(const float* gy, const float* packed_dgrad, const float* x_in, const float* addend, float* gx,
                      int B, int H, int W, int Ci, int Co, float* workspace, int64_t workspace_floats,
                      const uint32_t* relu_bits, int addend_unmasked, nfs_stream_t stream) {
  NFS_REQUIRE(gy && packed_dgrad && gx, "nfs_conv3x3_dgrad: null pointer");
  NFS_REQUIRE(B > 0 && H > 0 && W > 0, "nfs_conv3x3_dgrad: non-positive dimension");
  NFS_REQUIRE((int64_t)B * H * W < ((int64_t)1 << 31) / 4, "nfs_conv3x3_dgrad: too many pixels");
  NFS_REQUIRE(Co > 0 && Co % 32 == 0, "nfs_conv3x3_dgrad: Co must be a multiple of 32");
  if (Ci == 3) {
    NFS_REQUIRE(!x_in && !addend, "nfs_conv3x3_dgrad: Ci=3 takes no mask/addend");
    static const bool old_c3 = getenv("NFS_C3_OLD") != nullptr;
    if (Co == 64 && !old_c3) {
      const int tiles_x = (W + C3D_TW - 1) / C3D_TW, tiles_y = (H + C3D_TH - 1) / C3D_TH;
      static const int per_cu = [] { const char* e = getenv("NFS_C3D_BLOCKS"); return e ? atoi(e) : 2; }();
      const int64_t ntiles = (int64_t)B * tiles_x * tiles_y, cap = 256 * (int64_t)per_cu;
      hipLaunchKernelGGL(conv3x3_c3co64_dgrad_kernel, dim3((unsigned)(per_cu > 0 && ntiles > cap ? cap : ntiles)),
                         dim3(256), 0, as_stream(stream), gy, packed_dgrad, gx, B, H, W, tiles_x, tiles_y);
      return check_launch("nfs_conv3x3_dgrad(c3, Co=64, MFMA)");
    }
    const int64_t n = (int64_t)B * H * W;
    hipLaunchKernelGGL(conv3x3_c3_dgrad_kernel, dim3(blocks_for(n, 256)), dim3(256), 27 * Co * sizeof(float),
                       as_stream(stream), gy, packed_dgrad, gx, B, H, W, Co);
    return check_launch("nfs_conv3x3_dgrad(c3)");
  }
  NFS_REQUIRE(Ci > 0 && Ci % 64 == 0, "nfs_conv3x3_dgrad: Ci must be 3 or a multiple of 64");
  ConvArgs a{gy, packed_dgrad, x_in, addend, gx, nullptr, B, H, W, Co, Ci, 0, 0, 0, addend_unmasked ? 1 : 0, 1, 0};
  NFS_REQUIRE(!addend_unmasked || (x_in && takes_fused_pool(a, workspace, workspace_floats)),
              "nfs_conv3x3_dgrad: addend_unmasked needs x_in and the F(4x4) Winograd path");
  return launch_conv<1>(a, workspace, workspace_floats, as_stream(stream), nullptr, nullptr,
                        const_cast<uint32_t*>(relu_bits), nullptr);
}

int nfs_conv3x3_fwd_pool(const float* x, const float* packed_fwd, const float* bias, float* y, float* y_pool, int B, int H,
                         int W, int Ci, int Co, int relu, float* workspace, int64_t workspace_floats,
                         uint32_t* relu_bits, nfs_stream_t stream) {
  NFS_REQUIRE(x && packed_fwd && y_pool, "nfs_conv3x3_fwd_pool: null pointer");
  NFS_REQUIRE(B > 0 && H > 1 && W > 1, "nfs_conv3x3_fwd_pool: need H, W >= 2");
  NFS_REQUIRE((int64_t)B * H * W < ((int64_t)1 << 31) / 4, "nfs_conv3x3_fwd_pool: too many pixels");
  NFS_REQUIRE(Co > 0 && Co % 64 == 0 && Ci > 0 && Ci % 32 == 0, "nfs_conv3x3_fwd_pool: Ci %% 32, Co %% 64 required");
  ConvArgs a{x, packed_fwd, bias, nullptr, y, nullptr, B, H, W, Ci, Co, 0, 0, 0, relu, 1, 0};
  if (takes_fused_pool(a, workspace, workspace_floats)) {
    NFS_REQUIRE(y || relu_bits, "nfs_conv3x3_fwd_pool: without y the ReLU bit cache must be recorded");
    return launch_conv<0>(a, workspace, workspace_floats, as_stream(stream), y_pool, nullptr, relu_bits,
                          out_bits_of(relu_bits, B, H, W, Ci));
  }
  NFS_REQUIRE(!relu_bits, "nfs_conv3x3_fwd_pool: the ReLU bit cache needs the fused Winograd path "
                          "(nfs_conv3x3_relu_bits_words returned 0 for this layer)");
  NFS_REQUIRE(y, "nfs_conv3x3_fwd_pool: y may only be NULL on the fused Winograd path with a ReLU bit cache");
  if (int e = launch_conv<0>(a, workspace, workspace_floats, as_stream(stream))) return e;
  return nfs_avgpool2_fwd(y, y_pool, B, H, W, Co, stream);
}

int nfs_conv3x3_dgrad_pool(const float* gy_pool, const float* x_out, const float* packed_dgrad, const float* x_in,
                           const float* addend, float* gx, int B, int H, int W, int Ci, int Co, float* workspace,
                           int64_t workspace_floats, const uint32_t* relu_bits, int addend_unmasked,
                           nfs_stream_t stream) {
  NFS_REQUIRE(gy_pool && packed_dgrad && gx, "nfs_conv3x3_dgrad_pool: null pointer");
  NFS_REQUIRE(x_out || relu_bits, "nfs_conv3x3_dgrad_pool: x_out or the layer's ReLU bit cache is required");
  NFS_REQUIRE(B > 0 && H > 1 && W > 1, "nfs_conv3x3_dgrad_pool: need H, W >= 2");
  NFS_REQUIRE((int64_t)B * H * W < ((int64_t)1 << 31) / 4, "nfs_conv3x3_dgrad_pool: too many pixels");
  NFS_REQUIRE(Co > 0 && Co % 32 == 0 && Ci > 0 && Ci % 64 == 0, "nfs_conv3x3_dgrad_pool: Co %% 32, Ci %% 64 required");
  ConvArgs a{gy_pool, packed_dgrad, x_in, addend, gx, nullptr, B, H, W, Co, Ci, 0, 0, 0, addend_unmasked ? 1 : 0, 1, 0};
  NFS_REQUIRE(!addend_unmasked || (x_in && takes_fused_pool(a, workspace, workspace_floats)),
              "nfs_conv3x3_dgrad_pool: addend_unmasked needs x_in and the F(4x4) Winograd path");
  if (takes_fused_pool(a, workspace, workspace_floats)) {
    uint32_t* rb = const_cast<uint32_t*>(relu_bits);
    return launch_conv<1>(a, workspace, workspace_floats, as_stream(stream), nullptr, x_out, rb,
                          out_bits_of(rb, B, H, W, Ci), true);
  }
  NFS_REQUIRE(x_out, "nfs_conv3x3_dgrad_pool: x_out may only be NULL on the fused Winograd path");
  const int64_t n = (int64_t)B * H * W * Co;
  NFS_REQUIRE(workspace && workspace_floats >= n, "nfs_conv3x3_dgrad_pool: workspace of >= B*H*W*Co floats required");
  if (int e = nfs_avgpool2_bwd(gy_pool, x_out, nullptr, workspace, B, H, W, Co, stream)) return e;
  a.x = workspace;
  return launch_conv<1>(a, workspace + n, workspace_floats - n, as_stream(stream));
}

}
```

neural-flow-style_amd/engine.py:

```python
from __future__ import annotations

import os

import numpy as np
import torch

from . import ops, parallel


def _channels(acts, name, F):
    ch = getattr(acts, "channels", None)
    return int(ch[name]) if ch is not None and name in ch else int(F.shape[-1])


def _post_relu(name):
    return not (name.endswith("_pre_relu") or name.endswith("_pre_activation"))


def _logical(acts, name):
    F = acts[name]
    c = _channels(acts, name, F)
    return (F, False) if c == F.shape[-1] else (F[..., :c].contiguous(), True)


# ... 50 lines not shown
        for name in self.hist_layers:
            if "input" not in name and name not in order:
                raise KeyError("hist_layer %r is not a layer of the loss network" % (name,))
        self.hist_targets = None
        vgg_hist = [n for n in self.hist_layers if "input" not in n]
        wanted = self.layers + vgg_hist + ([self.content_layer] if self.content_layer else [])
        if not wanted:
            raise ValueError("no loss term reaches the loss network: w_style 0 (or no style layer) and no content / "
                             "histogram layer")
        for n in wanted:
            if n not in order:
                raise KeyError("%r is not a tensor of the loss network" % (n,))
        self.top = max(wanted, key=order.index)
        self.style_grams = None

    @property
    def liquid(self):
        return self.mode != 0

    @liquid.setter
    def liquid(self, on):
        self.mode = (1 if on else 0) if self.mode < 2 else self.mode

    def set_hist_image(self, style_img):
        if not self.hist_layers:
            self.hist_targets = None
            return None
        dev = self.net.device
        s = torch.as_tensor(np.asarray(style_img, np.float32)).to(dev)
        mean = torch.tensor([0.485 * 255, 0.456 * 255, 0.406 * 255], dtype=torch.float32, device=dev)
        vgg_hist = [n for n in self.hist_layers if "input" not in n]
        acts = {}
        if vgg_hist:
            order = [q[0] for q in self.net.seq]
            acts = self.net.forward((s - mean).unsqueeze(0).contiguous(), max(vgg_hist, key=order.index))
        self.hist_targets = {n: (s.unsqueeze(0).contiguous() if "input" in n else _logical(acts, n)[0].clone())
                             for n in self.hist_layers}
        return self.hist_targets

    def _hist_job(self, acts, sg, loss, d_gray=None):
        for name, wl in zip(self.hist_layers, self.w_hist_layers):
            if "input" in name:
                continue
            assert self.hist_targets is not None, "call set_hist_image first"
            F, padded = _logical(acts, name)
            m = None if d_gray is None else ops.resize_bicubic_tf1(d_gray.contiguous(), F.shape[1], F.shape[2])
            if padded:
                g = torch.zeros_like(F)
            else:
                g = sg.get(name)
                if g is None:
                    g = sg[name] = torch.zeros_like(F)
            ops.hist_loss(F, self.hist_targets[name], wl * self.w_hist, loss, g, relu_mask=_post_relu(name), mask=m)
            if padded:
                _add_logical(sg, name, acts[name], g)

    def _hist_input(self, dimg, loss, g_x, d_gray=None):
        for name, wl in zip(self.hist_layers, self.w_hist_layers):
            if "input" in name:
                assert self.hist_targets is not None, "call set_hist_image first"
                m = None if d_gray is None else ops.resize_bicubic_tf1(d_gray.contiguous(), dimg.shape[1], dimg.shape[2])
                ops.hist_loss(dimg, self.hist_targets[name], wl * self.w_hist, loss, g_x, relu_mask=False, mask=m)

    def set_content_image(self, content_img, top_k=0):
        if content_img is None or self.content_layer is None:
            self.content_feature = None
            return None
        dev = self.net.device
        s = torch.as_tensor(np.asarray(content_img, np.float32)).to(dev)
        mean = torch.tensor([0.485 * 255, 0.456 * 255, 0.406 * 255], dtype=torch.float32, device=dev)
        acts = self.net.forward((s - mean).unsqueeze(0).contiguous(), self.content_layer)
        cf = _logical(acts, self.content_layer)[0].clone()
        if top_k and top_k > 0:
            if "softmax2_pre_activation" not in self.content_layer:
                raise AssertionError("top_k > 0 needs content_layer softmax2_pre_activation (styler_base.py:241)")
            rows = cf.reshape(-1, cf.shape[-1])
            keep = torch.zeros_like(rows, dtype=torch.bool)
            keep.scatter_(1, rows.abs().topk(int(top_k), dim=1).indices, True)
            cf = (rows * keep).reshape(cf.shape).contiguous()
        self.content_feature = cf
        return self.content_feature

    def out_hw(self, H, W):
        if np.isclose(self.resize_scale, 1):
            return H, W
        return int(np.float32(self.resize_scale) * np.float32(H)), int(np.float32(self.resize_scale) * np.float32(W))

    def set_style_image(self, style_img):
        dev = self.net.device
        s = torch.as_tensor(np.asarray(style_img, np.float32)).to(dev)
        mean = torch.tensor([0.485 * 255, 0.456 * 255, 0.406 * 255], dtype=torch.float32, device=dev)
        x = (s - mean).unsqueeze(0).contiguous()
        acts = self.net.forward(x, self.top)
        self.style_grams = {}
        for name in self.layers:
            F = acts[name]
            _, h, w, _ = F.shape
            self.style_grams[name] = ops.gram_fwd(F, 1.0 / (2.0 * h * w * _channels(acts, name, F)))
        return self.style_grams

    def _coef_form(self, V, shape):
        return (self.mode == 0 and os.environ.get("NFS_RENDER_COEF", "1") != "0"
                and ops.render_coef_layout(V, *shape) is not None)

    def render(self, d, rot, keep_rotated=False, normalise=True):
        self.d_rot = None
        self._seg = None
        if self.rotate:
            if keep_rotated:
                self.d_rot = torch.empty((rot.shape[0],) + tuple(d.shape), dtype=torch.float32, device=d.device)
            if self.mode >= 2:
                self.d_rot = ops.rotate_fwd(d.unsqueeze(-1), rot).squeeze(-1)
                img, rs = ops.render_fwd(self.d_rot, self.tau, self.mode)
                if not keep_rotated:
                    self.d_rot = None
            elif keep_rotated and self._coef_form(rot.shape[0], d.shape):
                img, rs, _, self._seg = ops.rotate_render_fwd_coef(d, rot, self.tau, u_rot=self.d_rot)
            else:
                img, rs = ops.rotate_render_fwd(d, rot, self.tau, self.mode, d_rot=self.d_rot)
        else:
            img, rs = ops.render_fwd(d.unsqueeze(0), self.tau, self.mode)
        gmax = None
        V = img.shape[0]
        if self.liquid:
            norm = img
        elif normalise:
            norm, gmax = ops.maxnorm_fwd(img, max(V // self.v_batch, 1))
        else:
            norm = None
        return img, rs, norm, gmax

    def d_img(self, d, rot):
        _, _, norm, _ = self.render(d, rot)
        V, H, W = norm.shape
        H2, W2 = self.out_hw(H, W)
        dimg, _ = ops.loss_net_input_fwd(norm.unsqueeze(-1), H2, W2, want_x=False)
        return dimg

    def _gram_job(self, name, F, loss, unmasked=None, channels=None):
        wl = self.w_layers[self.layers.index(name)]
        _, h, w, c = F.shape
        scale = 1.0 / (2.0 * h * w * (channels or c))
        G = ops.gram_fwd(F, scale)
        Dm = ops.style_loss_fwd(G, self.style_grams[name], wl * self.w_style, loss)
        defer = unmasked is not None and self._defers_mask(name, F)
        if defer:
            unmasked.add(name)
        return ops.gram_bwd(F, Dm, scale, relu_mask=_post_relu(name) and not defer)

    def _defers_mask(self, name, F):
        return (name != self.top and name != self.content_layer and os.environ.get("NFS_NO_DEFER_MASK") is None
                and self.net.masks_addend_of(name, F.shape))

    def _vgg_loss_grad(self, x, total_out=None):
        sg = {}
        unmasked = set()
        if not self.layers:
            acts = self.net.forward(x, self.top, keep=self._keep())
            loss = torch.zeros(x.shape[0], dtype=torch.float32, device=x.device)
            self._content_job(acts, sg, loss)
            self._hist_job(acts, sg, loss)
            return self.net.backward(acts, sg, self.top, unmasked=unmasked), loss
        if self.gram_grouped:
            acts = self.net.forward(x, self.top, keep=self._keep())
            Fs = [acts[n] for n in self.layers]
            masks = []
            for n, F in zip(self.layers, Fs):
                d = self._defers_mask(n, F)
                if d:
                    unmasked.add(n)
                masks.append(_post_relu(n) and not d)
            parts, dFs, _ = ops.gram_style_group(Fs, [self.style_grams[n] for n in self.layers],
                                                 [w * self.w_style for w in self.w_layers], masks,
                                                 channels=[_channels(acts, n, F) for n, F in zip(self.layers, Fs)])
            sg.update(zip(self.layers, dFs))
            if total_out is not None:
                torch.sum(parts.view(-1), dim=0, keepdim=True, out=total_out)
                return self.net.backward(acts, sg, self.top, unmasked=unmasked), None
            loss = parts.sum(0)
            self._content_job(acts, sg, loss)
            self._hist_job(acts, sg, loss)
            return self.net.backward(acts, sg, self.top, unmasked=unmasked), loss
        loss = torch.zeros(x.shape[0], dtype=torch.float32, device=x.device)
        if not self.gram_side_stream:
            acts = self.net.forward(x, self.top, keep=self._keep())
            for name in self.layers:
                sg[name] = self._gram_job(name, acts[name], loss, unmasked, _channels(acts, name, acts[name]))
            self._content_job(acts, sg, loss)
            self._hist_job(acts, sg, loss)
            return self.net.backward(acts, sg, self.top, unmasked=unmasked), loss
        main = torch.cuda.current_stream(x.device)
        if self._side is None:
            self._side = torch.cuda.Stream(device=x.device)
        side = self._side
        side.wait_stream(main)

        top_inline = os.environ.get("NFS_GRAM_TOP_INLINE", "1") != "0"

        def on_layer(name, F):
            if name not in self.layers:
                return
            if name == self.top and top_inline:
                sg[name] = self._gram_job(name, F, loss, unmasked)
                return
            ev = torch.cuda.Event()
            ev.record(main)
            side.wait_event(ev)
            capturing = torch.cuda.is_current_stream_capturing()
            if not capturing:
                F.record_stream(side)
            with torch.cuda.stream(side):
                sg[name] = self._gram_job(name, F, loss, unmasked)
            if not capturing:
                sg[name].record_stream(main)

        acts = self.net.forward(x, self.top, on_layer=on_layer, keep=self._keep())
        main.wait_stream(side)
        self._content_job(acts, sg, loss)
        self._hist_job(acts, sg, loss)
        return self.net.backward(acts, sg, self.top, unmasked=unmasked), loss

    def _batch_views(self, V):
        return float(V) if self.v_batch is None else float(max(int(self.v_batch), 1))

    def _keep(self):
        return (set(self.layers) | ({self.content_layer} if self.content_layer else set())
                | set(n for n in getattr(self, "hist_layers", []) if "input" not in n))

    def _content_job(self, acts, sg, loss):
        if self.content_layer is None:
            return
        F, padded = _logical(acts, self.content_layer)
        V = F.shape[0]
        w = self.w_content * V / self._batch_views(V)
        if padded:
            g = torch.zeros_like(F)
        else:
            g = sg.get(self.content_layer)
            if g is None:
                g = sg[self.content_layer] = torch.zeros_like(F)
        ops.content_loss(F, w, loss, g, channel=self.content_channel, target=self.content_feature,
                         amp=self.w_content_amp, signed=not _post_relu(self.content_layer))
        if padded:
            _add_logical(sg, self.content_layer, acts[self.content_layer], g)

    accepts_live = True

    def _chain(self, d, rot, g_d, overwrite=False, total_out=None, live=None, dilate=1):
        D, H, W = d.shape
        H2, W2 = self.out_hw(H, W)
        hist_in = any("input" in n for n in self.hist_layers)
        fused_in = (not self.liquid and (H2, W2) == (H, W) and not (self.w_tv > 0 or hist_in)
                    and os.environ.get("NFS_FUSE_INPUT", "1") != "0")
        img, rs, norm, gmax = self.render(d, rot, keep_rotated=self.two_pass_adjoint, normalise=not fused_in)
        d_rot, seg = self.d_rot, self._seg
        self.d_rot = self._seg = None
        V = img.shape[0]
        if fused_in:
            dimg = None
            x, gmax = ops.maxnorm_input_fwd(img, max(V // self.v_batch, 1))
        else:
            dimg, x = ops.loss_net_input_fwd(norm.unsqueeze(-1), H2, W2, want_d_img=self.w_tv > 0 or hist_in)
        g_x, loss = self._vgg_loss_grad(x, total_out=total_out)
        if hist_in:
            self._hist_input(dimg, loss, g_x)
        if self.w_tv > 0:
            tv = torch.zeros(1, dtype=torch.float32, device=d.device)
            ops.tv_loss(dimg, self.w_tv * V / self._batch_views(V), tv, g_x)
            loss = loss + tv / V
        if fused_in:
            g_img = ops.maxnorm_input_bwd(img, gmax, g_x)
        else:
            g_norm = ops.loss_net_input_bwd(g_x, H, W, 1).reshape(V, H, W)
            g_img = g_norm if self.liquid else ops.maxnorm_bwd(img, gmax, g_norm)
        if self.rotate and d_rot is not None and seg is not None:
            ab, bounds = ops.render_ray_coef(g_img, seg, self.tau)
            ops.rotate_bwd_coef(d_rot, ab, rot, bounds, g_d_acc=g_d, overwrite=overwrite, live=live, dilate=dilate)
        elif self.rotate and d_rot is not None:
            g_rot, g_max = ops.render_bwd(d_rot, rs, g_img, self.tau, self.mode, g_d=d_rot, want_max=True)
            ops.rotate_bwd(g_rot.unsqueeze(-1), rot, g_d_acc=g_d.unsqueeze(-1), g_max=g_max, overwrite=overwrite)
        elif self.rotate:
            assert self.mode < 2, "the max / mean ray modes use the two-pass adjoint"
            ops.rotate_render_bwd(d, rot, rs, g_img, self.tau, self.mode, g_d_acc=g_d)
        elif overwrite:
            ops.render_bwd(d.unsqueeze(0), rs, g_img, self.tau, self.mode, g_d=g_d.unsqueeze(0))
        else:
            g_d.add_(ops.render_bwd(d.unsqueeze(0), rs, g_img, self.tau, self.mode)[0])
        return loss

    def writes_gradient(self, V):
        if not self.rotate:
            return True
        ngroups = self.view_groups if (V >= 4 and self.rotate and self.v_batch == 1) else 1
        return bool(self.two_pass_adjoint and min(ngroups, V) <= 1)

    def sums_total(self, V):
        ngroups = self.view_groups if (V >= 4 and self.rotate and self.v_batch == 1) else 1
        return bool(self.gram_grouped and self.layers and not self.w_tv and not self.hist_layers
                    and not self.content_layer and min(ngroups, V) <= 1)

    def loss_and_grad(self, d, rot, g_d, overwrite=False, total_out=None, live=None, dilate=1):
        assert self.style_grams is not None or not self.layers, "call set_style_image first"
        V = rot.shape[0] if self.rotate else 1
        ngroups = self.view_groups if (V >= 4 and self.rotate and self.v_batch == 1) else 1
        ngroups = min(ngroups, V)
        if ngroups <= 1:
            return self._chain(d, rot, g_d, overwrite=overwrite and self.writes_gradient(V),
                               total_out=total_out if (total_out is not None and self.sums_total(V)) else None,
                               live=live, dilate=dilate)
        assert not overwrite, "overwrite needs a single view batch (see writes_gradient)"
        assert total_out is None, "total_out needs a single view batch (see sums_total)"
        nst = min(self.vgg_streams, ngroups)
        main = torch.cuda.current_stream(d.device)
        if len(self._streams) < nst:
            self._streams = [torch.cuda.Stream(d.device) for _ in range(nst)]
        loss = torch.empty(V, dtype=torch.float32, device=d.device)
        g_parts = [torch.zeros_like(g_d) for _ in range(nst)]
        bounds = [V * i // ngroups for i in range(ngroups + 1)]
        for si in range(nst):
            self._streams[si].wait_stream(main)
        for gi in range(ngroups):
            si = gi % nst
            with torch.cuda.stream(self._streams[si]):
                lo, hi = bounds[gi], bounds[gi + 1]
                loss[lo:hi].copy_(self._chain(d, rot[lo:hi].contiguous(), g_parts[si], live=live, dilate=dilate))
        for si in range(nst):
            main.wait_stream(self._streams[si])
        for gp in g_parts:
            ops.axpy(g_d, gp, 1.0)
        return loss


def loss_capture_key(L):
    grams = tuple(int(t.data_ptr()) for t in (L.style_grams or {}).values())
    cf = getattr(L, "content_feature", None)
    hyper = tuple(getattr(L, a, None) for a in ("w_style", "tau", "mode", "resize_scale", "rotate", "w_tv",
                                                "v_batch", "w_content", "content_layer", "content_channel",
                                                "w_content_amp"))
    hist = (tuple(sorted((n, int(t.data_ptr())) for n, t in (getattr(L, "hist_targets", None) or {}).items())),
            getattr(L, "w_hist", 0.0), tuple(getattr(L, "hist_layers", ())), tuple(getattr(L, "w_hist_layers", ())),
            getattr(L, "style_mask", False))
    return (grams, tuple(getattr(L, "layers", ())), tuple(getattr(L, "w_layers", ())), hyper,
            None if cf is None else int(cf.data_ptr()), hist, id(getattr(L, "net", None)))


class GraphedLoss(object):

    def __init__(self, loss, force=None):
        self.loss = loss
        self.force = force
        self._reset()

    def _reset(self):
        self._graph = None
        self._key = None
        self._calls = 0
        self.mode = None if self.force is None else ("graph" if self.force else "eager")
        self.trial = None
        self._trials = []

    def _eager(self, d, rot):
        if isinstance(self.loss, ImageStyleLoss):
            return self.loss.loss_and_grad(d, rot)
        V = 1 if rot is None else int(rot.shape[0])
        if hasattr(self.loss, "writes_gradient") and self.loss.writes_gradient(V):
            g_d = torch.empty_like(d)
            return self.loss.loss_and_grad(d, rot, g_d, overwrite=True), g_d
        g_d = torch.zeros_like(d)
        return self.loss.loss_and_grad(d, rot, g_d), g_d

    def __call__(self, d, rot):
        import time
        key = (loss_capture_key(self.loss), tuple(d.shape), None if rot is None else tuple(rot.shape))
        if self._key is not None and key != self._key:
            self._reset()
        self._key = key
        self._calls += 1
        if self.mode == "eager" or self._calls == 1:
            return self._eager(d, rot)
        if self.mode is None:
            torch.cuda.synchronize()
            t0 = time.perf_counter()
            out = self._eager(d, rot)
            t_issue = time.perf_counter() - t0
            torch.cuda.synchronize()
            t_wall = time.perf_counter() - t0
            self._trials.append((t_issue, t_wall))
            if len(self._trials) == 3:
                self.trial = sorted(self._trials, key=lambda tw: tw[0] / tw[1])[1]
                self.mode = "graph" if self.trial[0] > 0.85 * self.trial[1] else "eager"
                if os.environ.get("NFS_VERBOSE"):
                    print("GraphedLoss: %s (issue %.3f ms of %.3f ms wall, median of 3; NFS_GRAPH=0/1 fixes the choice)"
                          % (self.mode, 1e3 * self.trial[0], 1e3 * self.trial[1]))
            return out
        if self._graph is None:
            self._d = d.clone()
            self._rot = None if rot is None else rot.clone()
            self._gd = torch.zeros_like(d)
            torch.cuda.synchronize()
            g = torch.cuda.CUDAGraph()
            with torch.cuda.graph(g):
                if isinstance(self.loss, ImageStyleLoss):
                    self._losses, self._gd = self.loss.loss_and_grad(self._d, self._rot)
                elif hasattr(self.loss, "writes_gradient") and self.loss.writes_gradient(
                        1 if self._rot is None else int(self._rot.shape[0])):
                    self._losses = self.loss.loss_and_grad(self._d, self._rot, self._gd, overwrite=True)
                else:
                    self._gd.zero_()
                    self._losses = self.loss.loss_and_grad(self._d, self._rot, self._gd)
            self._graph = g
        else:
            self._d.copy_(d)
            if rot is not None and rot.data_ptr() != self._rot.data_ptr():
                self._rot.copy_(rot)
        self._graph.replay()
        return self._losses, self._gd


class argparse_ns(object):
    """plain attribute bag"""


class TFAdamState(object):

    def __init__(self, beta1=0.9, beta2=0.999, eps=1e-8):
        self.b1, self.b2, self.eps = np.float32(beta1), np.float32(beta2), np.float32(eps)
        self.b1p, self.b2p = np.float32(1.0), np.float32(1.0)
        self.m = None
        self.v = None
# ... 614 lines not shown
```

neural-flow-style_amd/ops.py:

```python
from __future__ import annotations

import ctypes as C

import torch

from . import _lib
from ._lib import SplatCfg


def _ptr(t):
    if t is None:
        return None
    if not (t.is_cuda and t.dtype == torch.float32 and t.is_contiguous()):
        raise ValueError("expected a contiguous float32 CUDA tensor, got %s %s contiguous=%s"
                         % (t.device, t.dtype, t.is_contiguous()))
    return t.data_ptr()


_raw_stream = getattr(torch._C, "_cuda_getCurrentRawStream", None)


def _stream(device=None):
    if _raw_stream is not None:
        idx = torch.cuda.current_device() if device is None or device.index is None else device.index
# ... 333 lines not shown
        out = _empty(d.shape, d)
    _lib.call("nfs_smooth3d_relu_fwd", _ptr(d), _ptr(out), D, H, W, float(k), _stream())
    return out


def smooth3d_relu_bwd(out, g_out, k, g_d=None):
    D, H, W = out.shape
    if g_d is None:
        g_d = _empty(out.shape, out)
    _lib.call("nfs_smooth3d_relu_bwd", _ptr(out), _ptr(g_out), _ptr(g_d), D, H, W, float(k), _stream())
    return g_d



def render_fwd(d, tau, liquid=False):
    V, D, H, W = d.shape
    img = _empty((V, H, W), d); rs = _empty((V, H, W), d)
    _lib.call("nfs_render_fwd", _ptr(d), _ptr(img), _ptr(rs), V, D, H, W, float(tau), int(liquid), _stream())
    return img, rs


def render_bwd(d, raysum, g_img, tau, liquid=False, g_d=None, want_max=False):
    V, D, H, W = d.shape
    if g_d is None:
        g_d = _empty(d.shape, d)
    gmax = _empty((1,), d) if want_max else None
    _lib.call("nfs_render_bwd", _ptr(d), _ptr(raysum), _ptr(g_img), _ptr(g_d), V, D, H, W, float(tau),
              int(liquid), _ptr(gmax), _stream())
    return (g_d, gmax) if want_max else g_d


def rotate_render_fwd(d, rot, tau, liquid=False, img=None, raysum=None, d_rot=None):
    D, H, W = d.shape
    V = rot.shape[0]
    if img is None:
        img = _empty((V, H, W), d)
    if raysum is None:
        raysum = _empty((V, H, W), d)
    _lib.call("nfs_rotate_render_fwd", _ptr(d), _ptr(rot), _ptr(img), _ptr(raysum), _ptr(d_rot), V, D, H, W,
              float(tau), int(liquid), _stream())
    return img, raysum


_coef_layouts = {}


def render_coef_layout(V, D, H, W):
    key = (int(V), int(D), int(H), int(W))
    if key not in _coef_layouts:
        import ctypes
        nseg, seg_len = ctypes.c_int(0), ctypes.c_int(0)
        rc = _lib.lib().nfs_render_coef_layout(key[0], key[1], key[2], key[3], ctypes.byref(nseg), ctypes.byref(seg_len))
        _coef_layouts[key] = (nseg.value, seg_len.value) if rc == 0 else None
    return _coef_layouts[key]


def rotate_render_fwd_coef(d, rot, tau, img=None, raysum=None, u_rot=None, seg=None):
    D, H, W = d.shape
    V = rot.shape[0]
    nseg, _ = render_coef_layout(V, D, H, W)
    if img is None:
        img = _empty((V, H, W), d)
    if raysum is None:
        raysum = _empty((V, H, W), d)
    if u_rot is None:
        u_rot = _empty((V, D, H, W), d)
    if seg is None:
        seg = _empty((3, V, nseg, H, W), d)
    _lib.call("nfs_rotate_render_fwd_coef", _ptr(d), _ptr(rot), _ptr(img), _ptr(raysum), _ptr(u_rot), _ptr(seg), V, D, H, W,
              float(tau), _stream())
    return img, raysum, u_rot, seg


def render_ray_coef(g_img, seg, tau, ab=None, bounds=None):
    V, H, W = g_img.shape
    nseg = seg.shape[2]
    if ab is None:
        ab = _empty((V, nseg, H, W, 2), g_img)
    if bounds is None:
        bounds = _empty((_lib.lib().nfs_render_ray_coef_bounds(V, H, W),), g_img)
    _lib.call("nfs_render_ray_coef", _ptr(g_img), _ptr(seg), _ptr(ab), _ptr(bounds), V, H, W, float(tau), _stream())
    return ab, bounds


_LIVE_WS = {}


def rotate_bwd_coef(u_rot, ab, rot, bounds, g_d_acc=None, overwrite=False, live=None, dilate=1):
    V, D, H, W = u_rot.shape
    nseg, seg_len = render_coef_layout(V, D, H, W)
    if g_d_acc is None:
        overwrite = True
        g_d_acc = _empty((D, H, W), u_rot)
    if live is not None:
        key = (u_rot.device, D, H, W, int(_stream(u_rot.device) or 0))
        ws = _LIVE_WS.get(key)
        if ws is None:
            ws = _LIVE_WS[key] = _zeros((int(_lib.lib().nfs_rotate_live_workspace_ints(D, H, W)),), u_rot)
        _lib.call("nfs_rotate_bwd_coef_live", _ptr(u_rot), _ptr(ab), _ptr(rot), _ptr(g_d_acc), V, D, H, W, nseg, seg_len,
                  _ptr(bounds), int(bounds.numel()), int(bool(overwrite)), _ptr(live), int(dilate), _ptr(ws), _stream())
    else:
        _lib.call("nfs_rotate_bwd_coef", _ptr(u_rot), _ptr(ab), _ptr(rot), _ptr(g_d_acc), V, D, H, W, nseg, seg_len,
                  _ptr(bounds), int(bounds.numel()), int(bool(overwrite)), _stream())
    return g_d_acc


def rotate_render_bwd(d, rot, raysum, g_img, tau, liquid=False, g_d_acc=None):
    D, H, W = d.shape
    V = rot.shape[0]
    if g_d_acc is None:
        g_d_acc = _zeros(d.shape, d)
    _lib.call("nfs_rotate_render_bwd", _ptr(d), _ptr(rot), _ptr(raysum), _ptr(g_img), _ptr(g_d_acc), V, D, H, W,
              float(tau), int(liquid), _stream())
    return g_d_acc


def maxnorm_fwd(img, groups, out=None, gmax=None):
    n = img.numel() // groups
    if out is None:
        out = _empty(img.shape, img)
    if gmax is None:
        gmax = _empty((groups,), img)
    _lib.call("nfs_maxnorm_fwd", _ptr(img), _ptr(out), _ptr(gmax), groups, n, _stream())
    return out, gmax


def maxnorm_bwd(img, gmax, g_out, g_img=None):
    groups = gmax.numel()
    n = img.numel() // groups
    if g_img is None:
        g_img = _empty(img.shape, img)
    ws = _empty((64 * groups,), img)
    _lib.call("nfs_maxnorm_bwd", _ptr(img), _ptr(gmax), _ptr(g_out), _ptr(g_img), groups, n, _ptr(ws), _stream())
    return g_img


def maxnorm_input_fwd(img, groups):
    V, H, W = img.shape
    x = _empty((V, H, W, 3), img)
    gmax = _empty((groups,), img)
    _lib.call("nfs_maxnorm_input_fwd", _ptr(img), _ptr(x), _ptr(gmax), groups, img.numel() // groups, _stream())
    return x, gmax


def maxnorm_input_bwd(img, gmax, g_x):
    groups = gmax.numel()
    g_img = _empty(img.shape, img)
    ws = _empty((64 * groups,), img)
    _lib.call("nfs_maxnorm_input_bwd", _ptr(img), _ptr(gmax), _ptr(g_x), _ptr(g_img), groups, img.numel() // groups,
              _ptr(ws), _stream())
    return g_img



def loss_net_input_fwd(img, H2=None, W2=None, want_d_img=True, want_x=True):
    B, H, W, Cin = img.shape
    H2 = H if H2 is None else H2
    W2 = W if W2 is None else W2
    d_img = _empty((B, H2, W2, 3), img) if want_d_img else None
    x = _empty((B, H2, W2, 3), img) if want_x else None
    _lib.call("nfs_loss_net_input_fwd", _ptr(img), _ptr(d_img), _ptr(x), B, H, W, Cin, H2, W2, _stream())
    return d_img, x


def loss_net_input_bwd(g_x, H, W, Cin):
    B, H2, W2, _ = g_x.shape
    g_img = _empty((B, H, W, Cin), g_x)
    _lib.call("nfs_loss_net_input_bwd", _ptr(g_x), _ptr(g_img), B, H, W, Cin, H2, W2, _stream())
    return g_img



def gemm_mode(mode=None):
    return int(_lib.lib().nfs_gemm_mode(-1 if mode is None else int(mode)))


def conv3x3_pack(w_hwio, kind):
    _, _, Ci, Co = w_hwio.shape
    n = _lib.lib().nfs_conv3x3_packed_floats(Ci, Co, kind)
    packed = _empty((n,), w_hwio)
    _lib.call("nfs_conv3x3_pack", _ptr(w_hwio), _ptr(packed), Ci, Co, kind, _stream())
    return packed


_conv_ws = {}


def conv_workspace(device, floats):
    if torch.cuda.is_current_stream_capturing():
        return torch.empty(int(floats), dtype=torch.float32, device=device)
    key = (device.type, device.index, _stream(device))
    cur = _conv_ws.get(key)
    if cur is None or cur.numel() < floats:
        cur = torch.empty(int(floats), dtype=torch.float32, device=device)
        _conv_ws[key] = cur
    return cur


def _conv_ws_for(B, H, W, Ci, Co, device, splitk):
    if not splitk:
        return None, 0
    want = _lib.lib().nfs_conv3x3_workspace_floats(B, H, W, Ci, Co)
    ws = conv_workspace(device, want)
    return ws, ws.numel()


def conv3x3_relu_bits_words(B, H, W, Ci, Co, pooled):
    return int(_lib.lib().nfs_conv3x3_relu_bits_words(B, H, W, Ci, Co, int(bool(pooled))))


def conv3x3_relu_bits(B, H, W, Ci, Co, pooled, device):
    n = _lib.lib().nfs_conv3x3_relu_bits_words(B, H, W, Ci, Co, int(bool(pooled)))
    return torch.empty(n, dtype=torch.float32, device=device) if n > 0 else None


def conv3x3_fwd(x, packed, bias, Co, relu=True, out=None, splitk=True, relu_bits=None):
    B, H, W, Ci = x.shape
    if out is None:
        out = _empty((B, H, W, Co), x)
    ws, nws = _conv_ws_for(B, H, W, Ci, Co, x.device, splitk)
    _lib.call("nfs_conv3x3_fwd", _ptr(x), _ptr(packed), _ptr(bias), _ptr(out), B, H, W, Ci, Co, int(relu),
              _ptr(ws), nws, _ptr(relu_bits if splitk else None), _stream())
    return out


def conv3x3_dgrad(gy, packed, Ci, x_in=None, addend=None, out=None, splitk=True, relu_bits=None,
                  addend_unmasked=False):
    B, H, W, Co = gy.shape
    if out is None:
        out = _empty((B, H, W, Ci), gy)
    ws, nws = _conv_ws_for(B, H, W, Ci, Co, gy.device, splitk)
    _lib.call("nfs_conv3x3_dgrad", _ptr(gy), _ptr(packed), _ptr(x_in), _ptr(addend), _ptr(out), B, H, W, Ci, Co,
              _ptr(ws), nws, _ptr(relu_bits if (splitk and x_in is not None) else None), int(bool(addend_unmasked)),
              _stream())
    return out


def conv3x3_fwd_pool(x, packed, bias, Co, relu=True, relu_bits=None, want_y=True):
    B, H, W, Ci = x.shape
    out = _empty((B, H, W, Co), x) if (want_y or relu_bits is None) else None
    pooled = _empty((B, H // 2, W // 2, Co), x)
    ws, nws = _conv_ws_for(B, H, W, Ci, Co, x.device, True)
    _lib.call("nfs_conv3x3_fwd_pool", _ptr(x), _ptr(packed), _ptr(bias), _ptr(out), _ptr(pooled), B, H, W, Ci, Co,
              int(relu), _ptr(ws), nws, _ptr(relu_bits), _stream())
    return out, pooled


def conv3x3_dgrad_pool(gy_pool, x_out, packed, Ci, x_in=None, addend=None, relu_bits=None, hw=None,
                       addend_unmasked=False):
    if x_out is not None:
        B, H, W, Co = x_out.shape
    else:
        assert relu_bits is not None and hw is not None
        B, Co = gy_pool.shape[0], gy_pool.shape[-1]
        H, W = hw
    out = _empty((B, H, W, Ci), gy_pool)
    ws, nws = _conv_ws_for(B, H, W, Ci, Co, gy_pool.device, True)
    _lib.call("nfs_conv3x3_dgrad_pool", _ptr(gy_pool), _ptr(x_out), _ptr(packed), _ptr(x_in), _ptr(addend), _ptr(out),
              B, H, W, Ci, Co, _ptr(ws), nws, _ptr(relu_bits), int(bool(addend_unmasked)), _stream())
    return out


def avgpool2_fwd(x, out=None):
    B, H, W, Cn = x.shape
    if out is None:
        out = _empty((B, H // 2, W // 2, Cn), x)
    _lib.call("nfs_avgpool2_fwd", _ptr(x), _ptr(out), B, H, W, Cn, _stream())
    return out


def avgpool2_bwd(gy, x_shape, x=None, addend=None, out=None):
    B, H, W, Cn = x_shape
    if out is None:
        out = _empty(tuple(x_shape), gy)
    _lib.call("nfs_avgpool2_bwd", _ptr(gy), _ptr(x), _ptr(addend), _ptr(out), B, H, W, Cn, _stream())
    return out



def gram_fwd(F, scale, scale_dev=None, G=None, two_pass=True):
    B, Cn = F.shape[0], F.shape[-1]
    HW = F.numel() // (B * Cn)
    ws, nws = None, 0
    if two_pass:
        nws = _lib.lib().nfs_gram_workspace_floats(B, HW, Cn)
        ws = conv_workspace(F.device, nws)
        nws = ws.numel()
    if G is None:
        G = _empty((B, Cn, Cn), F) if two_pass else _zeros((B, Cn, Cn), F)
    elif not two_pass:
        G.zero_()
    _lib.call("nfs_gram_fwd", _ptr(F), _ptr(G), B, HW, Cn, _ptr(scale_dev), float(scale), _ptr(ws), nws, _stream())
    return G


def style_loss_fwd(G, Gs, weight, loss_acc, Dmat=None):
    B, Cn, _ = G.shape
    if Dmat is None:
        Dmat = _empty(G.shape, G)
    _lib.call("nfs_style_loss_fwd", _ptr(G), _ptr(Gs), _ptr(loss_acc), _ptr(Dmat), B, Gs.shape[0], Cn, float(weight),
              _stream())
    return Dmat


def gram_style_group(Fs, Gss, weights, relu_masks, want_G=False, channels=None):
    import ctypes
    n = len(Fs)
    if n > 8:
        a = gram_style_group(Fs[:8], Gss[:8], weights[:8], relu_masks[:8], want_G, channels and channels[:8])
        b = gram_style_group(Fs[8:], Gss[8:], weights[8:], relu_masks[8:], want_G, channels and channels[8:])
        return torch.cat([a[0], b[0]]), a[1] + b[1], (a[2] + b[2] if want_G else None)
    arr = (_lib.GramLayer * n)()
    keep = []
    B = Fs[0].shape[0]
    for l, (F, Gs, w, rm) in enumerate(zip(Fs, Gss, weights, relu_masks)):
        Cn = F.shape[-1]
        HW = F.numel() // (B * Cn)
        Dm = _empty((B, Cn, Cn), F)
        dF = _empty(F.shape, F)
        G = _empty((B, Cn, Cn), F) if want_G else None
        keep.append((Dm, dF, G))
        y = arr[l]
        y.F, y.Gs, y.G, y.Dmat, y.dF = _ptr(F), _ptr(Gs), _ptr(G), _ptr(Dm), _ptr(dF)
        y.B, y.Bs, y.HW, y.C = B, Gs.shape[0], HW, Cn
        y.scale, y.weight, y.relu_mask = 1.0 / (2.0 * HW * (channels[l] if channels else Cn)), float(w), int(bool(rm))
    L = _lib.lib()
    ap = ctypes.cast(arr, ctypes.c_void_p)
    P = L.nfs_gram_style_group_parts(ap, n)
    nws = L.nfs_gram_style_group_workspace_floats(ap, n)
    if P < 0 or nws < 0:
        raise ValueError("gram_style_group: 1..8 layers of one batch size with C a multiple of 64")
    ws = conv_workspace(Fs[0].device, max(nws, 1))
    parts = _empty((P, B), Fs[0])
    _lib.call("nfs_gram_style_group_fwd", ap, n, _ptr(parts), _ptr(ws), ws.numel(), _stream())
    _lib.call("nfs_gram_group_bwd", ap, n, _stream())
    return parts, [k[1] for k in keep], ([k[2] for k in keep] if want_G else None)


def content_loss(F, weight, loss_acc, g_acc, channel=0, target=None, amp=100.0, signed=False):
    B, Cn = F.shape[0], F.shape[-1]
    HW = F.numel() // (B * Cn)
    mode = 2 if target is not None else (0 if channel else 1)
    Bt = target.shape[0] if target is not None else 0
    _lib.call("nfs_content_loss_signed" if signed else "nfs_content_loss", _ptr(F), _ptr(target), _ptr(loss_acc),
              _ptr(g_acc), B, Bt, HW, Cn, int(channel or 0),
              mode, float(weight), float(amp), _stream())
    return g_acc


def resize_bicubic_tf1(x, oh, ow):
    B, H, W, Cn = x.shape
    out = _empty((B, oh, ow, Cn), x)
    _lib.call("nfs_resize_bicubic_tf1", _ptr(x), _ptr(out), B, H, W, Cn, int(oh), int(ow), _stream())
    return out


def style_mask_apply(F, mask):
    B, Cn = F.shape[0], F.shape[-1]
    HW = F.numel() // (B * Cn)
    Fm = _empty(F.shape, F)
    scale = _empty((B,), F)
    _lib.call("nfs_style_mask_apply", _ptr(F), _ptr(mask), _ptr(Fm), _ptr(scale), B, HW, Cn, _stream())
    return Fm, scale


def style_mask_bwd(dFm, mask, F):
    B, Cn = F.shape[0], F.shape[-1]
    HW = F.numel() // (B * Cn)
    out = _empty(F.shape, F)
    _lib.call("nfs_style_mask_bwd", _ptr(dFm), _ptr(mask), _ptr(F), _ptr(out), B, HW, Cn, _stream())
    return out


import os as _os
_HIST_WIDE = _os.environ.get("NFS_HIST_WIDE", "1") != "0"


def hist_loss(F, templ, weight, loss_acc, g_acc=None, relu_mask=False, mask=None):
    B, Cn = F.shape[0], F.shape[-1]
    HW = F.numel() // (B * Cn)
    Bt = templ.shape[0]
    HWt = templ.numel() // (Bt * Cn)
    assert templ.shape[-1] == Cn
    if mask is not None:
        assert mask.numel() == B * HW and mask.is_contiguous(), "mask must be [B,h,w] of the feature's size"
    if Cn <= 4 or (Cn % 4 == 0 and Cn <= 128 and _HIST_WIDE):
        nws = _lib.lib().nfs_hist_loss_wide_workspace_floats(B, Cn, HW, HWt)
        ws = conv_workspace(F.device, nws)
        _lib.call("nfs_hist_loss_wide", _ptr(F), _ptr(templ), _ptr(mask), _ptr(loss_acc), _ptr(g_acc), _ptr(ws), nws, B,
                  Bt, HW, HWt, Cn, float(weight), int(bool(relu_mask)), _stream())
        return g_acc
    if mask is not None:
        _lib.call("nfs_hist_loss_masked", _ptr(F), _ptr(templ), _ptr(mask), _ptr(loss_acc), _ptr(g_acc), B, Bt, HW, HWt,
                  Cn, float(weight), int(bool(relu_mask)), _stream())
        return g_acc
    _lib.call("nfs_hist_loss", _ptr(F), _ptr(templ), _ptr(loss_acc), _ptr(g_acc), B, Bt, HW, HWt, Cn, float(weight),
              int(bool(relu_mask)), _stream())
    return g_acc


def gram_bwd(F, Dmat, scale, scale_dev=None, relu_mask=True, out=None):
    B, Cn = F.shape[0], F.shape[-1]
    HW = F.numel() // (B * Cn)
    if out is None:
        out = _empty(F.shape, F)
    _lib.call("nfs_gram_bwd", _ptr(F), _ptr(Dmat), _ptr(out), B, HW, Cn, _ptr(scale_dev), float(scale),
              int(relu_mask), _stream())
    return out


def tv_loss(d_img, weight, loss_acc, g_acc=None):
    B, H, W, Cn = d_img.shape
    _lib.call("nfs_tv_loss", _ptr(d_img), _ptr(loss_acc), _ptr(g_acc), B, H, W, Cn, float(weight), _stream())



def make_splat_cfg(nd, res, domain, radius, support, rest_density, nsize, clip, mode):
    c = SplatCfg()
    c.nd = nd
    for k in range(3):
        c.res[k] = int(res[k]) if k < nd else 1
        c.domain[k] = float(domain[k]) if k < nd else 1.0
    c.radius = float(radius); c.support = float(support); c.rest_density = float(rest_density)
    c.nsize = int(nsize); c.clip = int(bool(clip)); c.mode = int(mode)
    return c


def p2g_fwd(p, cfg, attr=None, pd=None):
    N = p.shape[0]
    Cn = 1 if attr is None else attr.shape[-1]
    res = [cfg.res[k] for k in range(cfg.nd)]
    grid = _zeros(tuple(res) + (Cn,), p)
    wsum = _zeros(tuple(res) + (1,), p) if cfg.mode == 2 else None
    _lib.call("nfs_p2g_fwd", _ptr(p), _ptr(attr), _ptr(pd), _ptr(grid), _ptr(wsum), N, Cn, C.byref(cfg), _stream())
    return (grid, wsum) if cfg.mode == 2 else grid


def p2g_bwd(p, cfg, g_grid, attr=None, pd=None, g_wsum=None, need_p=True, need_attr=False, need_pd=False):
    N = p.shape[0]
    Cn = 1 if attr is None else attr.shape[-1]
    g_p = _empty(p.shape, p) if need_p else None
    g_attr = _empty(attr.shape, p) if need_attr else None
    g_pd = _empty((N,), p) if need_pd else None
    _lib.call("nfs_p2g_bwd", _ptr(p), _ptr(attr), _ptr(pd), _ptr(g_grid), _ptr(g_wsum), _ptr(g_p), _ptr(g_attr),
              _ptr(g_pd), N, Cn, C.byref(cfg), _stream())
    return g_p, g_attr, g_pd


def p2g_has_instance(cfg):
    rc = _lib.lib().nfs_p2g_has_instance(C.byref(cfg))
    if rc < 0:
        raise _lib.NfsError("nfs_p2g_has_instance", rc, _lib.lib().nfs_last_error().decode())
    return bool(rc)


def p2g_wavg_bwd(p, cfg, xsum, wsum, g_out, attr, eps=1e-6, need_p=True, need_attr=True):
    if not p2g_has_instance(cfg):
        return None
    N = p.shape[0]
    Cn = attr.shape[-1]
    g_p = _empty(p.shape, p) if need_p else None
    g_attr = _empty(attr.shape, p) if need_attr else None
    _lib.call("nfs_p2g_wavg_bwd", _ptr(p), _ptr(attr), _ptr(xsum), _ptr(wsum), _ptr(g_out), _ptr(g_p), _ptr(g_attr), N,
              Cn, float(eps), C.byref(cfg), _stream())
    return g_p, g_attr


def p2g_wavg_finish(xsum, wsum, eps=1e-6):
    Cn = xsum.shape[-1]
    n = wsum.numel()
    out = _empty(xsum.shape, xsum)
    _lib.call("nfs_p2g_wavg_finish", _ptr(xsum), _ptr(wsum), _ptr(out), n, Cn, float(eps), _stream())
    return out


def p2g_wavg_finish_bwd(xsum, wsum, g_out, eps=1e-6):
    Cn = xsum.shape[-1]
    n = wsum.numel()
    g_x = _empty(xsum.shape, xsum); g_w = _empty(wsum.shape, xsum)
    _lib.call("nfs_p2g_wavg_finish_bwd", _ptr(xsum), _ptr(wsum), _ptr(g_out), _ptr(g_x), _ptr(g_w), n, Cn,
              float(eps), _stream())
    return g_x, g_w



def _written(*tensors):
    for t in tensors:
# ... 242 lines not shown
```

neural-flow-style_amd/vgg.py:

```python
from __future__ import annotations

import math
import os
import sys
from collections import OrderedDict

import numpy as np
import torch

from . import ops

_R_MEAN = 0.485 * 255
_G_MEAN = 0.456 * 255
_B_MEAN = 0.406 * 255

VGG19_BLOCKS = (("conv1", 2, 64), ("conv2", 2, 128), ("conv3", 4, 256), ("conv4", 4, 512), ("conv5", 4, 512))
VGG16_BLOCKS = (("conv1", 2, 64), ("conv2", 2, 128), ("conv3", 3, 256), ("conv4", 3, 512), ("conv5", 3, 512))


def layer_sequence(blocks=VGG19_BLOCKS):
    seq, cin = [], 3
    for blk, reps, cout in blocks:
        for i in range(reps):
            seq.append(("%s_%d" % (blk, i + 1), "conv", cin, cout))
            cin = cout
        seq.append(("pool" + blk[-1], "pool", cout, cout))
    return seq


def synthetic_weights(seed=123, blocks=VGG19_BLOCKS, upto=None):
    rng = np.random.RandomState(seed)
    out = OrderedDict()
    for name, kind, cin, cout in layer_sequence(blocks):
        if kind != "conv":
            continue
        w = rng.randn(3, 3, cin, cout) * math.sqrt(2.0 / (9 * cin))
        b = rng.randn(cout) * 0.01
        out[name] = (w.astype(np.float32), b.astype(np.float32))
        if name == upto:
            break
    return out


def load_npz_weights(path, blocks=VGG19_BLOCKS, scope="vgg_19", upto=None):
    z = np.load(path)
    out = OrderedDict()
    for name, kind, cin, cout in layer_sequence(blocks):
        if kind != "conv":
            continue
        forms = (("%s/weights" % name, "%s/biases" % name),
                 ("%s/%s/%s/weights" % (scope, name[:5], name), "%s/%s/%s/biases" % (scope, name[:5], name)),
                 (name + "_w", name + "_b"))
        for wk, bk in forms:
            if wk in z and bk in z:
                break
        else:
            raise KeyError("%s: no weights for layer %s (looked for %s)" % (path, name, ", ".join(f[0] for f in forms)))
        w, b = np.asarray(z[wk], np.float32), np.asarray(z[bk], np.float32)
        if w.shape != (3, 3, cin, cout) or b.shape != (cout,):
            raise ValueError("%s: layer %s has shapes %s / %s, expected (3,3,%d,%d) HWIO / (%d,)"
                             % (path, name, w.shape, b.shape, cin, cout, cout))
        out[name] = (w, b)
        if name == upto:
            break
    return out


class _Activations(OrderedDict):

    def __init__(self):
        OrderedDict.__init__(self)
        self.relu_bits = {}
        self.hw = {}


class VGG(object):

    def __init__(self, weights, device, blocks=VGG19_BLOCKS):
        self.device = torch.device(device)
        self.seq = [s for s in layer_sequence(blocks)]
        self.params = {}
        for name, (w, b) in weights.items():
            wt = torch.as_tensor(w, dtype=torch.float32).to(self.device).contiguous()
            self.params[name] = dict(
                fwd=ops.conv3x3_pack(wt, 0), dgrad=ops.conv3x3_pack(wt, 1),
                bias=torch.as_tensor(b, dtype=torch.float32).to(self.device).contiguous(),
                cin=wt.shape[2], cout=wt.shape[3])
        self.names = list(weights.keys())

    def plan(self, upto):
        idx = [i for i, s in enumerate(self.seq) if s[0] == upto]
        if not idx:
            raise KeyError(upto)
        plan = self.seq[:idx[0] + 1]
        for name, kind, _, _ in plan:
            if kind == "conv" and name not in self.params:
                raise KeyError("no weights for %s" % name)
        return plan

    def forward(self, x, upto, on_layer=None, keep=None):
        acts = _Activations()
        cur = x
        plan = self.plan(upto)
        pooled = None
        bits = acts.relu_bits
        for li, (name, kind, cin, cout) in enumerate(plan):
            if kind == "conv":
                p = self.params[name]
                nxt_pool = li + 1 < len(plan) and plan[li + 1][1] == "pool"
                B_, H_, W_ = cur.shape[0], cur.shape[1], cur.shape[2]
                below_conv = li > 0 and plan[li - 1][1] == "conv"
                if nxt_pool and cin % 32 == 0 and cur.shape[1] >= 2 and cur.shape[2] >= 2:
                    rb = ops.conv3x3_relu_bits(B_, H_, W_, cin, cout, True, cur.device) if below_conv else None
                    want_y = rb is None or keep is None or name in keep
                    acts.hw[name] = (H_, W_)
                    cur, pooled = ops.conv3x3_fwd_pool(cur, p["fwd"], p["bias"], cout, relu=True, relu_bits=rb,
                                                       want_y=want_y)
                else:
                    rb = ops.conv3x3_relu_bits(B_, H_, W_, cin, cout, False, cur.device) if below_conv else None
                    cur = ops.conv3x3_fwd(cur, p["fwd"], p["bias"], cout, relu=True, relu_bits=rb)
                if rb is not None:
                    bits[name] = rb
            else:
                cur = pooled if pooled is not None else ops.avgpool2_fwd(cur)
                pooled = None
            acts[name] = cur
            if on_layer is not None:
                on_layer(name, cur)
        return acts

    def masks_addend_of(self, name, acts_shape):
        names = [s_[0] for s_ in self.seq]
        i = names.index(name)
        if i + 1 >= len(self.seq) or self.seq[i + 1][1] != "conv":
            return False
        _, _, cin, cout = self.seq[i + 1]
        B, h, w, _ = acts_shape
        nxt_pool = i + 2 < len(self.seq) and self.seq[i + 2][1] == "pool"
        return ops.conv3x3_relu_bits_words(B, h, w, cin, cout, nxt_pool) > 0

    def backward(self, acts, style_grads, upto, unmasked=()):
        assert upto not in unmasked, "the top layer's gradient enters the chain directly: it must be masked"
        plan = self.plan(upto)
        g = style_grads[upto]
        pooled_from = None
        for li in range(len(plan) - 1, -1, -1):
            name, kind, cin, cout = plan[li]
            below = plan[li - 1] if li > 0 else None
            if kind == "conv" and pooled_from == name:
                pooled_from = None
                p = self.params[name]
                bname, bkind = below[0], below[1]
                assert bkind == "conv"
                g = ops.conv3x3_dgrad_pool(g, acts[name], p["dgrad"], cin, x_in=acts[bname],
                                           addend=style_grads.get(bname), relu_bits=getattr(acts, "relu_bits", {}).get(name),
                                           hw=getattr(acts, "hw", {}).get(name),
                                           addend_unmasked=bname in unmasked and bname in style_grads)
                continue
            if kind == "conv":
                p = self.params[name]
                if below is None:
                    return ops.conv3x3_dgrad(g, p["dgrad"], cin)
                bname, bkind = below[0], below[1]
                if bkind == "conv":
                    g = ops.conv3x3_dgrad(g, p["dgrad"], cin, x_in=acts[bname], addend=style_grads.get(bname),
                                          relu_bits=getattr(acts, "relu_bits", {}).get(name),
                                          addend_unmasked=bname in unmasked and bname in style_grads)
                else:
                    g = ops.conv3x3_dgrad(g, p["dgrad"], cin)
            else:
                bname = below[0]
                xb = acts[bname]
                hw = (xb.shape[1], xb.shape[2]) if xb is not None else getattr(acts, "hw", {})[bname]
                b2 = plan[li - 2] if li > 1 else None
                if (style_grads.get(bname) is None and b2 is not None and b2[1] == "conv" and below[2] % 64 == 0
                        and hw[0] >= 2 and hw[1] >= 2):
                    pooled_from = bname
                else:
                    assert xb is not None, "the output of %s is needed here: list it in ``keep``" % bname
                    g = ops.avgpool2_bwd(g, xb.shape, x=xb, addend=style_grads.get(bname))
        raise AssertionError("unreachable")


def load_vgg(model_path, device, seed=123, synthetic=None):
    name = os.path.basename(model_path).split(".")[0]
    blocks = VGG16_BLOCKS if "16" in name else VGG19_BLOCKS
    scope = "vgg_16" if "16" in name else "vgg_19"
    npz = os.path.splitext(model_path)[0] + ".npz"
    if synthetic is None:
        synthetic = os.environ.get("NFS_SYNTHETIC_VGG", "0") == "1"
    if os.path.exists(npz):
        w = load_npz_weights(npz, blocks, scope)
        src = npz
    elif synthetic:
        w = synthetic_weights(seed, blocks)
        src = "synthetic(seed=%d)" % seed
    else:
        raise FileNotFoundError(
            "%s not found%s.  Convert the slim checkpoint to an .npz with keys 'conv1_1/weights' [3,3,Cin,Cout], "
            "'conv1_1/biases', ... (INTEGRATION.md), or opt in to seeded SYNTHETIC weights with config.synthetic_weights"
            "=True / NFS_SYNTHETIC_VGG=1 (results are then not a stylisation by VGG-19)"
            % (npz, " (a TensorFlow checkpoint %s is present but cannot be read without TensorFlow)" % model_path
               if os.path.exists(model_path) or os.path.exists(model_path + ".index") else ""))
    net = VGG(w, device, blocks)
    net.source = src
    print("loss network: %s weights from %s" % (scope, src), file=sys.stderr)
    return net
```

Before: 446.0.

## Fuse grey max-norm input into conv1_1 and fold its backward into ray coefficients

Adds a grey-input path in which conv1_1 reads the single-channel rendered image directly. Per-group max normalisation and mean subtraction are folded into packed weights summed over the three input channels, so the separate maxnorm, loss-net-input and 3-channel conv kernels disappear. The backward pass gets a matching grey dgrad kernel that emits per-block partials, and a fused kernel that finishes the max-norm gradient and computes the ray coefficients in one pass. The gram group forward also gains a last-block ticket reduction that writes the total loss on device. The cost is extra kernels, redundant per-block max reductions over each group's image, and atomic-ticket state that has to reset correctly between calls.

```diff
diff --git a/include/nfs_hip.h b/include/nfs_hip.h
--- a/include/nfs_hip.h
+++ b/include/nfs_hip.h
@@ -169,6 +169,12 @@
 int nfs_maxnorm_input_fwd(const float* img, float* x, float* gmax, int G, int n, nfs_stream_t stream);
 int nfs_maxnorm_input_bwd(const float* img, const float* gmax, const float* g_x, float* g_img, int G, int n,
                           float* workspace, nfs_stream_t stream);
+int nfs_grey_conv1_fwd(const float* img, const float* packed_grey, const float* bias, float* y, float* gmax, int V, int H,
+                       int W, int G, int relu, nfs_stream_t stream);
+int nfs_grey_conv1_bwd(const float* gy, const float* packed_grey_dgrad, const float* img, const float* gmax, float* g255,
+                       float* part, int V, int H, int W, int G, int nb, nfs_stream_t stream);
+int nfs_grey_ray_coef(const float* img, const float* gmax, const float* g255, const float* part, int nb, const float* seg,
+                      float* ab, float* bounds, float* g_img, int V, int H, int W, int G, float tau, nfs_stream_t stream);
 
 
 int nfs_loss_net_input_fwd(const float* img, float* d_img, float* x,
@@ -226,7 +232,7 @@
 int64_t nfs_gram_style_group_workspace_floats(const nfs_gram_layer_t* layers, int n);
 int nfs_gram_style_group_parts(const nfs_gram_layer_t* layers, int n);
 int nfs_gram_style_group_fwd(const nfs_gram_layer_t* layers, int n, float* loss_parts, float* workspace,
-                             int64_t workspace_floats, nfs_stream_t stream);
+                             int64_t workspace_floats, float* total_out, unsigned* ticket, nfs_stream_t stream);
 int nfs_gram_group_bwd(const nfs_gram_layer_t* layers, int n, nfs_stream_t stream);
 
 int nfs_content_loss(const float* F, const float* target, float* loss_acc, float* g_acc, int B, int Bt,
diff --git a/neural-flow-style_amd/_lib.py b/neural-flow-style_amd/_lib.py
--- a/neural-flow-style_amd/_lib.py
+++ b/neural-flow-style_amd/_lib.py
@@ -107,6 +107,9 @@
     "nfs_maxnorm_bwd": [_P, _P, _P, _P, _I, _I, _P, _P],
     "nfs_maxnorm_input_fwd": [_P, _P, _P, _I, _I, _P],
     "nfs_maxnorm_input_bwd": [_P, _P, _P, _P, _I, _I, _P, _P],
+    "nfs_grey_conv1_fwd": [_P, _P, _P, _P, _P, _I, _I, _I, _I, _I, _P],
+    "nfs_grey_conv1_bwd": [_P, _P, _P, _P, _P, _P, _I, _I, _I, _I, _I, _P],
+    "nfs_grey_ray_coef": [_P, _P, _P, _P, _I, _P, _P, _P, _P, _I, _I, _I, _I, _F, _P],
     "nfs_loss_net_input_fwd": [_P, _P, _P, _I, _I, _I, _I, _I, _I, _P],
     "nfs_loss_net_input_bwd": [_P, _P, _I, _I, _I, _I, _I, _I, _P],
     "nfs_conv3x3_packed_floats": [_I, _I, _I],
@@ -143,7 +146,7 @@
     "nfs_relu_mask_add": [_P, _I, _P, _I, _P, _I, _P, _I, _L, _I, _P],
     "nfs_gram_style_group_workspace_floats": [_P, _I],
     "nfs_gram_style_group_parts": [_P, _I],
-    "nfs_gram_style_group_fwd": [_P, _I, _P, _P, _L, _P],
+    "nfs_gram_style_group_fwd": [_P, _I, _P, _P, _L, _P, _P, _P],
     "nfs_gram_group_bwd": [_P, _I, _P],
     "nfs_hist_loss_masked": [_P, _P, _P, _P, _P, _I, _I, _I, _I, _I, _F, _I, _P],
     "nfs_hist_loss_wide_workspace_floats": [_I, _I, _I, _I],
@@ -176,7 +179,7 @@
             "nfs_conv2d_workspace_floats": C.c_int64, "nfs_conv2d_group_workspace_floats": C.c_int64}
 
 _lib = None
-ABI_VERSION = 154
+ABI_VERSION = 155
 
 
 def build(verbose=False):
diff --git a/neural-flow-style_amd/csrc/api.hip b/neural-flow-style_amd/csrc/api.hip
--- a/neural-flow-style_amd/csrc/api.hip
+++ b/neural-flow-style_amd/csrc/api.hip
@@ -11,7 +11,7 @@
 }
 
 extern "C" {
-int nfs_version(void) { return 154; }
+int nfs_version(void) { return 155; }
 const char* nfs_last_error(void) { return nfs::g_err; }
 int nfs_device_cus(void) {
   int dev = 0;
diff --git a/neural-flow-style_amd/csrc/gram.hip b/neural-flow-style_amd/csrc/gram.hip
--- a/neural-flow-style_amd/csrc/gram.hip
+++ b/neural-flow-style_amd/csrc/gram.hip
@@ -28,6 +28,10 @@
   GramArgs L[GR_MAXL];
   int ustart[GR_MAXL + 1];
   int n;
+  float* total = nullptr;
+  const float* parts = nullptr;
+  unsigned* ticket = nullptr;
+  int nparts = 0;
 };
 
 constexpr int GR_KC = 32;
@@ -220,11 +224,32 @@
   gram_tn_block<TS>(a, smem, (int)blockIdx.x, (int)gridDim.x);
 }
 
+__device__ __forceinline__ void gram_group_total(const GramGroupArgs& g) {
+  __shared__ int last;
+  __shared__ float red[16];
+  __syncthreads();
+  if (threadIdx.x == 0) {
+    __threadfence();
+    last = atomicAdd(g.ticket, 1u) == gridDim.x - 1 ? 1 : 0;
+  }
+  __syncthreads();
+  if (!last) return;
+  __threadfence();
+  float s = 0.f;
+  for (int k = threadIdx.x; k < g.nparts; k += 256) s += g.parts[k];
+  s = block_sum(s, red);
+  if (threadIdx.x == 0) {
+    *g.total = s;
+    *g.ticket = 0u;
+  }
+}
+
 __global__ void __launch_bounds__(256, 2) gram_tn_group_kernel(GramGroupArgs g) {
   extern __shared__ __attribute__((aligned(16))) float smem[];
   int l = 0;
   while (l + 1 < g.n && (int)blockIdx.x >= g.ustart[l + 1]) ++l;
   gram_tn_block<64>(g.L[l], smem, (int)blockIdx.x - g.ustart[l], g.ustart[l + 1] - g.ustart[l]);
+  if (g.total) gram_group_total(g);
 }
 
 constexpr int GRD_ROWS = 4;
@@ -289,6 +314,7 @@
   int l = 0;
   while (l + 1 < g.n && (int)blockIdx.x >= g.ustart[l + 1]) ++l;
   gram_reduce_block(g.L[l], (int)blockIdx.x - g.ustart[l]);
+  if (g.total) gram_group_total(g);
 }
 
 __global__ void __launch_bounds__(256) style_loss_kernel(const float* __restrict__ G, const float* __restrict__ Gs,
@@ -477,7 +503,8 @@
 }
 
 int nfs_gram_style_group_fwd(const nfs_gram_layer_t* layers, int n, float* loss_parts, float* workspace,
-                             int64_t workspace_floats, nfs_stream_t stream) {
+                             int64_t workspace_floats, float* total_out, unsigned* ticket, nfs_stream_t stream) {
+  NFS_REQUIRE(!total_out || ticket, "nfs_gram_style_group_fwd: total_out needs a ticket word");
   GramGroupPlan P;
   NFS_REQUIRE(gram_group_plan(layers, n, P) == 0,
               "nfs_gram_style_group_fwd: 1..8 layers with F, Gs, Dmat set, one batch size, C a multiple of 64");
@@ -491,6 +518,10 @@
   for (int k = 0; k < P.rd.n; ++k) {
     P.rd.L[k].part = loss_parts;
     P.rd.L[k].ws = workspace + reinterpret_cast<int64_t>(P.rd.L[k].ws) / (int64_t)sizeof(float);
+  }
+  if (total_out) {
+    GramGroupArgs& lastk = P.rd_blocks > 0 ? P.rd : P.tn;
+    lastk.total = total_out; lastk.parts = loss_parts; lastk.ticket = ticket; lastk.nparts = P.parts * layers[0].B;
   }
   const size_t lds = 4 * GR_KC * 64 * sizeof(float);
   hipLaunchKernelGGL(gram_tn_group_kernel, dim3((unsigned)P.tn_blocks), dim3(256), lds, as_stream(stream), P.tn);
diff --git a/neural-flow-style_amd/csrc/render.hip b/neural-flow-style_amd/csrc/render.hip
--- a/neural-flow-style_amd/csrc/render.hip
+++ b/neural-flow-style_amd/csrc/render.hip
@@ -709,6 +709,31 @@
   }
 }
 
+__device__ __forceinline__ float ray_coef_of(float g, const float* __restrict__ seg, float2* __restrict__ ab, int V,
+                                             int HW, int v, int px, float tau) {
+  const int64_t plane = (int64_t)V * RR_SEG * HW, at0 = (int64_t)v * RR_SEG * HW + px;
+  const float ntau = -tau * 1.44269504088896341f;
+  float S[RR_SEG], Is[RR_SEG], um[RR_SEG], E[RR_SEG], F[RR_SEG];
+  float P = 0.f, Itot = 0.f, bound = 0.f;
+#pragma unroll
+  for (int s2 = 0; s2 < RR_SEG; ++s2) {
+    S[s2] = seg[at0 + (int64_t)s2 * HW];
+    Is[s2] = seg[plane + at0 + (int64_t)s2 * HW];
+    um[s2] = seg[2 * plane + at0 + (int64_t)s2 * HW];
+    E[s2] = __builtin_amdgcn_exp2f(P * ntau);
+    F[s2] = Itot;
+    Itot = fmaf(E[s2], Is[s2], Itot);
+    P += S[s2];
+  }
+#pragma unroll
+  for (int s2 = 0; s2 < RR_SEG; ++s2) {
+    const float A = g * E[s2], B = g * tau * (Itot - F[s2]);
+    ab[at0 + (int64_t)s2 * HW] = make_float2(A, B);
+    bound = fmaxf(bound, fmaf(fabsf(A), um[s2], fabsf(B)));
+  }
+  return bound;
+}
+
 __global__ void __launch_bounds__(256) render_ray_coef_kernel(const float* __restrict__ g_img,
                                                               const float* __restrict__ seg, float2* __restrict__ ab,
                                                               int V, int HW, float tau, float* __restrict__ bounds) {
@@ -717,27 +742,43 @@
   float bound = 0.f;
   if (gid < total) {
     const int v = (int)(gid / HW), px = (int)(gid - (int64_t)v * HW);
-    const int64_t plane = (int64_t)V * RR_SEG * HW, at0 = (int64_t)v * RR_SEG * HW + px;
-    const float ntau = -tau * 1.44269504088896341f, g = g_img[gid];
-    float S[RR_SEG], Is[RR_SEG], um[RR_SEG], E[RR_SEG], F[RR_SEG];
-    float P = 0.f, Itot = 0.f;
-#pragma unroll
-    for (int s2 = 0; s2 < RR_SEG; ++s2) {
-      S[s2] = seg[at0 + (int64_t)s2 * HW];
-      Is[s2] = seg[plane + at0 + (int64_t)s2 * HW];
-      um[s2] = seg[2 * plane + at0 + (int64_t)s2 * HW];
-      E[s2] = __builtin_amdgcn_exp2f(P * ntau);
-      F[s2] = Itot;
-      Itot = fmaf(E[s2], Is[s2], Itot);
-      P += S[s2];
-    }
-#pragma unroll
-    for (int s2 = 0; s2 < RR_SEG; ++s2) {
-      const float A = g * E[s2], B = g * tau * (Itot - F[s2]);
-      ab[at0 + (int64_t)s2 * HW] = make_float2(A, B);
-      bound = fmaxf(bound, fmaf(fabsf(A), um[s2], fabsf(B)));
-    }
-  }
+    bound = ray_coef_of(g_img[gid], seg, ab, V, HW, v, px, tau);
+  }
+  bound = block_max(bound, red);
+  if (threadIdx.x == 0) bounds[blockIdx.x] = bound > 0.f ? fminf(bound, 3.0e38f) : 0.f;
+}
+
+__global__ void __launch_bounds__(256) grey_ray_coef_kernel(const float* __restrict__ img, const float* __restrict__ gmax,
+                                                            const float* __restrict__ g255, const float* __restrict__ part,
+                                                            int nb, int vpg, const float* __restrict__ seg,
+                                                            float2* __restrict__ ab, float* __restrict__ g_img, int V, int HW,
+                                                            float tau, float* __restrict__ bounds) {
+  __shared__ float red[16];
+  const int64_t total = (int64_t)V * HW, gid0 = (int64_t)blockIdx.x * blockDim.x, gid = gid0 + threadIdx.x;
+  const int64_t last = gid0 + blockDim.x - 1 < total - 1 ? gid0 + blockDim.x - 1 : total - 1;
+  const int v = gid < total ? (int)(gid / HW) : -1, mine = v < 0 ? -1 : v / vpg;
+  const int g_first = (int)(gid0 / HW) / vpg, g_last = (int)(last / HW) / vpg;
+  float S = 0.f, T = 1.f;
+  for (int grp = g_first; grp <= g_last; ++grp) {
+    const float* pp = part + (int64_t)grp * vpg * nb * 2;
+    float s = 0.f, ti = 0.f;
+    for (int k = threadIdx.x; k < vpg * nb; k += blockDim.x) {
+      s += pp[2 * k];
+      ti += pp[2 * k + 1];
+    }
+    s = block_sum(s, red);
+    ti = block_sum(ti, red);
+    if (grp == mine) { S = s; T = ti; }
+  }
+  float bound = 0.f;
+  if (gid < total) {
+    const float m = gmax[mine];
+    float g = g255[gid] / m;
+    if (img[gid] == m) g -= S / (m * m) / T;
+    if (g_img) g_img[gid] = g;
+    if (seg) bound = ray_coef_of(g, seg, ab, V, HW, v, (int)(gid - (int64_t)v * HW), tau);
+  }
+  if (!seg) return;
   bound = block_max(bound, red);
   if (threadIdx.x == 0) bounds[blockIdx.x] = bound > 0.f ? fminf(bound, 3.0e38f) : 0.f;
 }
@@ -937,6 +978,18 @@
   return check_launch("nfs_maxnorm_fwd");
 }
 
+int nfs_grey_ray_coef(const float* img, const float* gmax, const float* g255, const float* part, int nb, const float* seg,
+                      float* ab, float* bounds, float* g_img, int V, int H, int W, int G, float tau, nfs_stream_t stream) {
+  NFS_REQUIRE(img && gmax && g255 && part, "nfs_grey_ray_coef: null pointer");
+  NFS_REQUIRE(seg ? (ab && bounds) : (g_img != nullptr), "nfs_grey_ray_coef: seg needs ab and bounds; without seg, g_img");
+  NFS_REQUIRE(V > 0 && H > 0 && W > 0 && nb >= 1, "nfs_grey_ray_coef: non-positive dimension");
+  NFS_REQUIRE(G > 0 && V % G == 0, "nfs_grey_ray_coef: the views must divide into G equal groups");
+  const int64_t n = (int64_t)V * H * W;
+  hipLaunchKernelGGL(grey_ray_coef_kernel, dim3(blocks_for(n, 256)), dim3(256), 0, as_stream(stream), img, gmax, g255, part,
+                     nb, V / G, seg, reinterpret_cast<float2*>(ab), g_img, V, H * W, tau, bounds);
+  return check_launch("nfs_grey_ray_coef");
+}
+
 int nfs_maxnorm_input_fwd(const float* img, float* x, float* gmax, int G, int n, nfs_stream_t stream) {
   NFS_REQUIRE(img && x && gmax, "nfs_maxnorm_input_fwd: null pointer");
   NFS_REQUIRE(G > 0 && n > 0, "nfs_maxnorm_input_fwd: non-positive size");
diff --git a/neural-flow-style_amd/csrc/vgg.hip b/neural-flow-style_amd/csrc/vgg.hip
--- a/neural-flow-style_amd/csrc/vgg.hip
+++ b/neural-flow-style_amd/csrc/vgg.hip
@@ -436,6 +436,171 @@
     }
   }
   __syncthreads();
+  }
+}
+
+constexpr float GREY_M0 = 114.75f;
+__global__ void __launch_bounds__(256) grey_conv1_fwd_kernel(const float* __restrict__ img, float* __restrict__ gmax,
+                                                             const float* __restrict__ w,
+                                                             const float* __restrict__ bias, float* __restrict__ y,
+                                                             int H, int W, int vpg, int relu, int tiles_x, int tiles_y) {
+  constexpr int PN = (C3F_TH + 2) * C3F_PW;
+  __shared__ float patch[2 * PN + 4];
+  __shared__ __attribute__((aligned(16))) float otile[C3F_TH * C3F_TW * C3F_OS];
+  __shared__ float red[16];
+  const int t = threadIdx.x, lane = t & 63, wid = t >> 6, i = lane & 31, h = lane >> 5;
+  const int b = blockIdx.y, group = b / vpg;
+  const int n = vpg * H * W;
+  const float* xg = img + (int64_t)group * n;
+  float m = -INFINITY;
+  if ((reinterpret_cast<uintptr_t>(xg) & 15) == 0) {
+    const float4* x4 = reinterpret_cast<const float4*>(xg);
+    const int n4 = n >> 2;
+    for (int e = t; e < n4; e += 256) {
+      const float4 v = x4[e];
+      m = fmaxf(m, fmaxf(fmaxf(v.x, v.y), fmaxf(v.z, v.w)));
+    }
+    for (int e = 4 * n4 + t; e < n; e += 256) m = fmaxf(m, xg[e]);
+  } else {
+    for (int e = t; e < n; e += 256) m = fmaxf(m, xg[e]);
+  }
+  m = block_max(m, red);
+  if (blockIdx.x == 0 && b == group * vpg && t == 0) gmax[group] = m;
+  float bfr[9][2];
+#pragma unroll
+  for (int s2 = 0; s2 < 9; ++s2)
+#pragma unroll
+    for (int nt = 0; nt < 2; ++nt) bfr[s2][nt] = w[(2 * s2 + h) * 64 + nt * 32 + i];
+  float bv2[2];
+#pragma unroll
+  for (int nt = 0; nt < 2; ++nt) bv2[nt] = bias ? bias[nt * 32 + i] : 0.f;
+  const float* xb = img + (int64_t)b * H * W;
+  for (int tile_id = blockIdx.x; tile_id < tiles_x * tiles_y; tile_id += gridDim.x) {
+  const int tx = tile_id % tiles_x, ty = tile_id / tiles_x;
+  const int y0 = ty * C3F_TH, x0 = tx * C3F_TW;
+  for (int e = t; e < PN; e += 256) {
+    const int r = e / C3F_PW, c = e - r * C3F_PW;
+    const int gy_ = y0 - 1 + r, gx_ = x0 - 1 + c;
+    const bool in = gy_ >= 0 && gy_ < H && gx_ >= 0 && gx_ < W;
+    patch[e] = in ? __fsub_rn(__fmul_rn(xb[(int64_t)gy_ * W + gx_] / m, 255.f), GREY_M0) : 0.f;
+    patch[PN + e] = in ? 1.f : 0.f;
+  }
+  __syncthreads();
+  const int mrow = wid * 32 + i;
+  const int base = (mrow / C3F_TW) * C3F_PW + (mrow % C3F_TW);
+  f32x16 acc[2];
+#pragma unroll
+  for (int nt = 0; nt < 2; ++nt)
+#pragma unroll
+    for (int r = 0; r < 16; ++r) acc[nt][r] = 0.f;
+#pragma unroll
+  for (int s2 = 0; s2 < 9; ++s2) {
+    const int k = 2 * s2 + h, tap = k < 9 ? k : k - 9;
+    const float av = patch[(k < 9 ? 0 : PN) + base + (tap / 3) * C3F_PW + tap % 3];
+    acc[0] = __builtin_amdgcn_mfma_f32_32x32x2f32(av, bfr[s2][0], acc[0], 0, 0, 0);
+    acc[1] = __builtin_amdgcn_mfma_f32_32x32x2f32(av, bfr[s2][1], acc[1], 0, 0, 0);
+  }
+#pragma unroll
+  for (int nt = 0; nt < 2; ++nt) {
+    const float bv = bv2[nt];
+#pragma unroll
+    for (int r = 0; r < 16; ++r) {
+      const int row = wid * 32 + (r & 3) + 8 * (r >> 2) + 4 * h;
+      float v = acc[nt][r] + bv;
+      if (relu) v = fmaxf(v, 0.f);
+      otile[row * C3F_OS + nt * 32 + i] = v;
+    }
+  }
+  __syncthreads();
+  for (int f = t; f < C3F_TH * C3F_TW * 16; f += 256) {
+    const int row = f >> 4, q = f & 15;
+    const int gy_ = y0 + row / C3F_TW, gx_ = x0 + row % C3F_TW;
+    if (gy_ < H && gx_ < W)
+      *reinterpret_cast<float4*>(y + (((int64_t)b * H + gy_) * W + gx_) * 64 + 4 * q) =
+          *reinterpret_cast<const float4*>(otile + row * C3F_OS + 4 * q);
+  }
+  __syncthreads();
+  }
+}
+
+typedef float f32x4 __attribute__((ext_vector_type(4)));
+constexpr int GCD_TS = 9;
+__global__ void __launch_bounds__(256) grey_conv1_bwd_kernel(const float* __restrict__ gy,
+                                                             const float* __restrict__ wd,
+                                                             const float* __restrict__ img,
+                                                             const float* __restrict__ gmax, float* __restrict__ g255,
+                                                             float* __restrict__ part, int H, int W, int vpg,
+                                                             int tiles_x, int tiles_y) {
+  static_assert(C3D_PW == 16 && C3D_PH == 16, "a halo'd row is one M tile");
+  __shared__ float Tt[C3D_M * GCD_TS];
+  __shared__ float red[16];
+  const int t = threadIdx.x, lane = t & 63, wid = t >> 6, i = lane & 15, kq = lane >> 4;
+  const int b = blockIdx.y;
+  float bw[4][4];
+#pragma unroll
+  for (int j = 0; j < 4; ++j)
+#pragma unroll
+    for (int u = 0; u < 4; ++u) bw[j][u] = i < 9 ? wd[i * 64 + 16 * j + 4 * kq + u] : 0.f;
+  const float m = gmax[b / vpg];
+  float s_acc = 0.f, ties_acc = 0.f;
+  for (int tile_id = blockIdx.x; tile_id < tiles_x * tiles_y; tile_id += gridDim.x) {
+  const int tx = tile_id % tiles_x, ty = tile_id / tiles_x;
+  const int y0 = ty * C3D_TH, x0 = tx * C3D_TW;
+  float4 av[4][4];
+#pragma unroll
+  for (int mt = 0; mt < 4; ++mt) {
+    const int qy = y0 - 1 + wid * 4 + mt, qx = x0 - 1 + i;
+    const bool ok = qy >= 0 && qy < H && qx >= 0 && qx < W;
+    const float* gp = gy + (((int64_t)b * H + (ok ? qy : 0)) * W + (ok ? qx : 0)) * 64 + 4 * kq;
+#pragma unroll
+    for (int j = 0; j < 4; ++j) av[mt][j] = ok ? *reinterpret_cast<const float4*>(gp + 16 * j) : make_float4(0.f, 0.f, 0.f, 0.f);
+  }
+  f32x4 acc[4];
+#pragma unroll
+  for (int mt = 0; mt < 4; ++mt)
+#pragma unroll
+    for (int r = 0; r < 4; ++r) acc[mt][r] = 0.f;
+#pragma unroll
+  for (int j = 0; j < 4; ++j) {
+#pragma unroll
+    for (int mt = 0; mt < 4; ++mt) acc[mt] = __builtin_amdgcn_mfma_f32_16x16x4f32(av[mt][j].x, bw[j][0], acc[mt], 0, 0, 0);
+#pragma unroll
+    for (int mt = 0; mt < 4; ++mt) acc[mt] = __builtin_amdgcn_mfma_f32_16x16x4f32(av[mt][j].y, bw[j][1], acc[mt], 0, 0, 0);
+#pragma unroll
+    for (int mt = 0; mt < 4; ++mt) acc[mt] = __builtin_amdgcn_mfma_f32_16x16x4f32(av[mt][j].z, bw[j][2], acc[mt], 0, 0, 0);
+#pragma unroll
+    for (int mt = 0; mt < 4; ++mt) acc[mt] = __builtin_amdgcn_mfma_f32_16x16x4f32(av[mt][j].w, bw[j][3], acc[mt], 0, 0, 0);
+  }
+  if (i < 9) {
+#pragma unroll
+    for (int mt = 0; mt < 4; ++mt)
+#pragma unroll
+      for (int r = 0; r < 4; ++r) Tt[((wid * 4 + mt) * 16 + 4 * kq + r) * GCD_TS + i] = acc[mt][r];
+  }
+  __syncthreads();
+  if (t < C3D_TH * C3D_TW) {
+    const int ly = t / C3D_TW, lx = t % C3D_TW;
+    const int py = y0 + ly, px = x0 + lx;
+    if (py < H && px < W) {
+      float o = 0.f;
+#pragma unroll
+      for (int dy = 0; dy < 3; ++dy)
+#pragma unroll
+        for (int dx = 0; dx < 3; ++dx) o += Tt[((ly + dy) * C3D_PW + lx + dx) * GCD_TS + dy * 3 + dx];
+      const int64_t at = ((int64_t)b * H + py) * W + px;
+      const float g = __fmul_rn(o, 255.f), xi = img[at];
+      g255[at] = g;
+      s_acc += g * xi;
+      ties_acc += (xi == m) ? 1.f : 0.f;
+    }
+  }
+  __syncthreads();
+  }
+  s_acc = block_sum(s_acc, red);
+  ties_acc = block_sum(ties_acc, red);
+  if (t == 0) {
+    part[((int64_t)b * gridDim.x + blockIdx.x) * 2] = s_acc;
+    part[((int64_t)b * gridDim.x + blockIdx.x) * 2 + 1] = ties_acc;
   }
 }
 
@@ -715,6 +880,34 @@
                         const_cast<uint32_t*>(relu_bits), nullptr);
 }
 
+int nfs_grey_conv1_fwd(const float* img, const float* packed_grey, const float* bias, float* y, float* gmax, int V, int H,
+                       int W, int G, int relu, nfs_stream_t stream) {
+  NFS_REQUIRE(img && packed_grey && y && gmax, "nfs_grey_conv1_fwd: null pointer");
+  NFS_REQUIRE(V > 0 && H > 0 && W > 0, "nfs_grey_conv1_fwd: non-positive dimension");
+  NFS_REQUIRE(G > 0 && V % G == 0, "nfs_grey_conv1_fwd: the views must divide into G equal groups");
+  NFS_REQUIRE((int64_t)V * H * W < ((int64_t)1 << 31) / 64, "nfs_grey_conv1_fwd: too many pixels");
+  const int tiles_x = (W + C3F_TW - 1) / C3F_TW, tiles_y = (H + C3F_TH - 1) / C3F_TH;
+  static const int total = [] { const char* e = getenv("NFS_GREY_FWD_BLOCKS"); return e ? atoi(e) : 512; }();
+  int nb = total / V;
+  nb = nb < 1 ? 1 : (nb > tiles_x * tiles_y ? tiles_x * tiles_y : nb);
+  hipLaunchKernelGGL(grey_conv1_fwd_kernel, dim3((unsigned)nb, (unsigned)V), dim3(256), 0, as_stream(stream), img, gmax,
+                     packed_grey, bias, y, H, W, V / G, relu, tiles_x, tiles_y);
+  return check_launch("nfs_grey_conv1_fwd");
+}
+
+int nfs_grey_conv1_bwd(const float* gy, const float* packed_grey_dgrad, const float* img, const float* gmax, float* g255,
+                       float* part, int V, int H, int W, int G, int nb, nfs_stream_t stream) {
+  NFS_REQUIRE(gy && packed_grey_dgrad && img && gmax && g255 && part, "nfs_grey_conv1_bwd: null pointer");
+  NFS_REQUIRE(V > 0 && H > 0 && W > 0, "nfs_grey_conv1_bwd: non-positive dimension");
+  NFS_REQUIRE(G > 0 && V % G == 0, "nfs_grey_conv1_bwd: the views must divide into G equal groups");
+  NFS_REQUIRE((int64_t)V * H * W < ((int64_t)1 << 31) / 64, "nfs_grey_conv1_bwd: too many pixels");
+  const int tiles_x = (W + C3D_TW - 1) / C3D_TW, tiles_y = (H + C3D_TH - 1) / C3D_TH;
+  NFS_REQUIRE(nb >= 1 && nb <= 65535, "nfs_grey_conv1_bwd: nb (blocks per view = partials per view) out of range");
+  hipLaunchKernelGGL(grey_conv1_bwd_kernel, dim3((unsigned)nb, (unsigned)V), dim3(256), 0, as_stream(stream), gy,
+                     packed_grey_dgrad, img, gmax, g255, part, H, W, V / G, tiles_x, tiles_y);
+  return check_launch("nfs_grey_conv1_bwd");
+}
+
 int nfs_conv3x3_fwd_pool(const float* x, const float* packed_fwd, const float* bias, float* y, float* y_pool, int B, int H,
                          int W, int Ci, int Co, int relu, float* workspace, int64_t workspace_floats,
                          uint32_t* relu_bits, nfs_stream_t stream) {
diff --git a/neural-flow-style_amd/engine.py b/neural-flow-style_amd/engine.py
--- a/neural-flow-style_amd/engine.py
+++ b/neural-flow-style_amd/engine.py
@@ -226,17 +226,20 @@
         return (name != self.top and name != self.content_layer and os.environ.get("NFS_NO_DEFER_MASK") is None
                 and self.net.masks_addend_of(name, F.shape))
 
-    def _vgg_loss_grad(self, x, total_out=None):
+    def _vgg_loss_grad(self, x, total_out=None, grey=None):
         sg = {}
+        src = x if grey is None else grey[0]
+        fkw = {} if grey is None else {"grey": grey}
+        bkw = {} if grey is None else {"to_first": True}
         unmasked = set()
         if not self.layers:
-            acts = self.net.forward(x, self.top, keep=self._keep())
-            loss = torch.zeros(x.shape[0], dtype=torch.float32, device=x.device)
+            acts = self.net.forward(x, self.top, keep=self._keep(), **fkw)
+            loss = torch.zeros(src.shape[0], dtype=torch.float32, device=src.device)
             self._content_job(acts, sg, loss)
             self._hist_job(acts, sg, loss)
-            return self.net.backward(acts, sg, self.top, unmasked=unmasked), loss
+            return self.net.backward(acts, sg, self.top, unmasked=unmasked, **bkw), loss
         if self.gram_grouped:
-            acts = self.net.forward(x, self.top, keep=self._keep())
+            acts = self.net.forward(x, self.top, keep=self._keep(), **fkw)
             Fs = [acts[n] for n in self.layers]
             masks = []
             for n, F in zip(self.layers, Fs):
@@ -244,28 +247,33 @@
                 if d:
                     unmasked.add(n)
                 masks.append(_post_relu(n) and not d)
+            fold = (total_out is not None and len(Fs) <= 8 and os.environ.get("NFS_GREY_CONV1", "1") != "0")
+            if fold and getattr(self, "_gram_ticket", None) is None:
+                self._gram_ticket = torch.zeros(1, dtype=torch.float32, device=src.device)
             parts, dFs, _ = ops.gram_style_group(Fs, [self.style_grams[n] for n in self.layers],
                                                  [w * self.w_style for w in self.w_layers], masks,
-                                                 channels=[_channels(acts, n, F) for n, F in zip(self.layers, Fs)])
+                                                 channels=[_channels(acts, n, F) for n, F in zip(self.layers, Fs)],
+                                                 total=(total_out, self._gram_ticket) if fold else None)
             sg.update(zip(self.layers, dFs))
             if total_out is not None:
-                torch.sum(parts.view(-1), dim=0, keepdim=True, out=total_out)
-                return self.net.backward(acts, sg, self.top, unmasked=unmasked), None
+                if not fold:
+                    torch.sum(parts.view(-1), dim=0, keepdim=True, out=total_out)
+                return self.net.backward(acts, sg, self.top, unmasked=unmasked, **bkw), None
             loss = parts.sum(0)
             self._content_job(acts, sg, loss)
             self._hist_job(acts, sg, loss)
-            return self.net.backward(acts, sg, self.top, unmasked=unmasked), loss
-        loss = torch.zeros(x.shape[0], dtype=torch.float32, device=x.device)
+            return self.net.backward(acts, sg, self.top, unmasked=unmasked, **bkw), loss
+        loss = torch.zeros(src.shape[0], dtype=torch.float32, device=src.device)
         if not self.gram_side_stream:
-            acts = self.net.forward(x, self.top, keep=self._keep())
+            acts = self.net.forward(x, self.top, keep=self._keep(), **fkw)
             for name in self.layers:
                 sg[name] = self._gram_job(name, acts[name], loss, unmasked, _channels(acts, name, acts[name]))
             self._content_job(acts, sg, loss)
             self._hist_job(acts, sg, loss)
-            return self.net.backward(acts, sg, self.top, unmasked=unmasked), loss
-        main = torch.cuda.current_stream(x.device)
+            return self.net.backward(acts, sg, self.top, unmasked=unmasked, **bkw), loss
+        main = torch.cuda.current_stream(src.device)
         if self._side is None:
-            self._side = torch.cuda.Stream(device=x.device)
+            self._side = torch.cuda.Stream(device=src.device)
         side = self._side
         side.wait_stream(main)
 
@@ -288,11 +296,11 @@
             if not capturing:
                 sg[name].record_stream(main)
 
-        acts = self.net.forward(x, self.top, on_layer=on_layer, keep=self._keep())
+        acts = self.net.forward(x, self.top, on_layer=on_layer, keep=self._keep(), **fkw)
         main.wait_stream(side)
         self._content_job(acts, sg, loss)
         self._hist_job(acts, sg, loss)
-        return self.net.backward(acts, sg, self.top, unmasked=unmasked), loss
+        return self.net.backward(acts, sg, self.top, unmasked=unmasked, **bkw), loss
 
     def _batch_views(self, V):
         return float(V) if self.v_batch is None else float(max(int(self.v_batch), 1))
@@ -330,25 +338,38 @@
         d_rot, seg = self.d_rot, self._seg
         self.d_rot = self._seg = None
         V = img.shape[0]
-        if fused_in:
+        groups = max(V // self.v_batch, 1)
+        grey_in = (fused_in and getattr(self.net, "takes_grey", lambda: False)() and V % groups == 0
+                   and os.environ.get("NFS_GREY_CONV1", "1") != "0")
+        if grey_in:
+            dimg = None
+            gmax = torch.empty(groups, dtype=torch.float32, device=img.device)
+            g_x, loss = self._vgg_loss_grad(None, total_out=total_out, grey=(img, groups, gmax))
+        elif fused_in:
             dimg = None
             x, gmax = ops.maxnorm_input_fwd(img, max(V // self.v_batch, 1))
         else:
             dimg, x = ops.loss_net_input_fwd(norm.unsqueeze(-1), H2, W2, want_d_img=self.w_tv > 0 or hist_in)
-        g_x, loss = self._vgg_loss_grad(x, total_out=total_out)
+        if not grey_in:
+            g_x, loss = self._vgg_loss_grad(x, total_out=total_out)
         if hist_in:
             self._hist_input(dimg, loss, g_x)
         if self.w_tv > 0:
             tv = torch.zeros(1, dtype=torch.float32, device=d.device)
             ops.tv_loss(dimg, self.w_tv * V / self._batch_views(V), tv, g_x)
             loss = loss + tv / V
-        if fused_in:
+        coef_form = bool(self.rotate and d_rot is not None and seg is not None)
+        if grey_in:
+            g255, part = ops.grey_conv1_bwd(g_x, self.net.params[self.net.seq[0][0]]["grey_dgrad"], img, gmax)
+            ab, bounds, g_img = ops.grey_ray_coef(img, gmax, g255, part, seg=seg if coef_form else None, tau=self.tau)
+        elif fused_in:
             g_img = ops.maxnorm_input_bwd(img, gmax, g_x)
         else:
             g_norm = ops.loss_net_input_bwd(g_x, H, W, 1).reshape(V, H, W)
             g_img = g_norm if self.liquid else ops.maxnorm_bwd(img, gmax, g_norm)
         if self.rotate and d_rot is not None and seg is not None:
-            ab, bounds = ops.render_ray_coef(g_img, seg, self.tau)
+            if not grey_in:
+                ab, bounds = ops.render_ray_coef(g_img, seg, self.tau)
             ops.rotate_bwd_coef(d_rot, ab, rot, bounds, g_d_acc=g_d, overwrite=overwrite, live=live, dilate=dilate)
         elif self.rotate and d_rot is not None:
             g_rot, g_max = ops.render_bwd(d_rot, rs, g_img, self.tau, self.mode, g_d=d_rot, want_max=True)
diff --git a/neural-flow-style_amd/ops.py b/neural-flow-style_amd/ops.py
--- a/neural-flow-style_amd/ops.py
+++ b/neural-flow-style_amd/ops.py
@@ -509,6 +509,59 @@
     return g_img
 
 
+GREY_M0 = 114.75
+_INPUT_MEAN = (0.485 * 255, 0.456 * 255, 0.406 * 255)
+
+
+def grey_conv1_pack(w_hwio):
+    assert tuple(w_hwio.shape) == (3, 3, 3, 64), "the grey path is conv1_1's: Ci = 3, Co = 64"
+    w = w_hwio.detach().to("cpu", torch.float64).reshape(9, 3, 64)
+    ws = w.sum(1)
+    ms = sum((_INPUT_MEAN[c] - GREY_M0) * w[:, c] for c in range(3))
+    fwd = torch.cat([ws, -ms], 0).to(torch.float32).to(w_hwio.device).contiguous()
+    dgrad = ws.flip(0).to(torch.float32).to(w_hwio.device).contiguous()
+    return fwd, dgrad
+
+
+def grey_conv1_blocks(V, H, W):
+    return max(1, min(((H + 13) // 14) * ((W + 13) // 14), 512 // V))
+
+
+def grey_conv1_fwd(img, groups, packed, bias, relu=True, y=None, gmax=None):
+    V, H, W = img.shape
+    if y is None:
+        y = _empty((V, H, W, 64), img)
+    if gmax is None:
+        gmax = _empty((groups,), img)
+    _lib.call("nfs_grey_conv1_fwd", _ptr(img), _ptr(packed), _ptr(bias), _ptr(y), _ptr(gmax), V, H, W, groups,
+              int(bool(relu)), _stream())
+    return y, gmax
+
+
+def grey_conv1_bwd(gy, packed_dgrad, img, gmax, g255=None, part=None):
+    V, H, W = img.shape
+    if g255 is None:
+        g255 = _empty((V, H, W), img)
+    if part is None:
+        part = _empty((V, grey_conv1_blocks(V, H, W), 2), img)
+    _lib.call("nfs_grey_conv1_bwd", _ptr(gy), _ptr(packed_dgrad), _ptr(img), _ptr(gmax), _ptr(g255), _ptr(part), V, H, W,
+              gmax.numel(), part.shape[1], _stream())
+    return g255, part
+
+
+def grey_ray_coef(img, gmax, g255, part, seg=None, tau=0.0, ab=None, bounds=None, want_g_img=False):
+    V, H, W = img.shape
+    g_img = _empty((V, H, W), img) if (want_g_img or seg is None) else None
+    if seg is not None:
+        if ab is None:
+            ab = _empty((V, seg.shape[2], H, W, 2), img)
+        if bounds is None:
+            bounds = _empty((_lib.lib().nfs_render_ray_coef_bounds(V, H, W),), img)
+    _lib.call("nfs_grey_ray_coef", _ptr(img), _ptr(gmax), _ptr(g255), _ptr(part), part.shape[1], _ptr(seg), _ptr(ab),
+              _ptr(bounds), _ptr(g_img), V, H, W, gmax.numel(), float(tau), _stream())
+    return ab, bounds, g_img
+
+
 
 def loss_net_input_fwd(img, H2=None, W2=None, want_d_img=True, want_x=True):
     B, H, W, Cin = img.shape
@@ -660,9 +713,10 @@
     return Dmat
 
 
-def gram_style_group(Fs, Gss, weights, relu_masks, want_G=False, channels=None):
+def gram_style_group(Fs, Gss, weights, relu_masks, want_G=False, channels=None, total=None):
     import ctypes
     n = len(Fs)
+    assert total is None or n <= 8, "total: one launch group (at most 8 layers)"
     if n > 8:
         a = gram_style_group(Fs[:8], Gss[:8], weights[:8], relu_masks[:8], want_G, channels and channels[:8])
         b = gram_style_group(Fs[8:], Gss[8:], weights[8:], relu_masks[8:], want_G, channels and channels[8:])
@@ -689,7 +743,8 @@
         raise ValueError("gram_style_group: 1..8 layers of one batch size with C a multiple of 64")
     ws = conv_workspace(Fs[0].device, max(nws, 1))
     parts = _empty((P, B), Fs[0])
-    _lib.call("nfs_gram_style_group_fwd", ap, n, _ptr(parts), _ptr(ws), ws.numel(), _stream())
+    _lib.call("nfs_gram_style_group_fwd", ap, n, _ptr(parts), _ptr(ws), ws.numel(), _ptr(total[0]) if total else None,
+              _ptr(total[1]) if total else None, _stream())
     _lib.call("nfs_gram_group_bwd", ap, n, _stream())
     return parts, [k[1] for k in keep], ([k[2] for k in keep] if want_G else None)
 
diff --git a/neural-flow-style_amd/vgg.py b/neural-flow-style_amd/vgg.py
--- a/neural-flow-style_amd/vgg.py
+++ b/neural-flow-style_amd/vgg.py
@@ -71,6 +71,7 @@
     def __init__(self):
         OrderedDict.__init__(self)
         self.relu_bits = {}
+        self.gmax = None
         self.hw = {}
 
 
@@ -86,6 +87,8 @@
                 fwd=ops.conv3x3_pack(wt, 0), dgrad=ops.conv3x3_pack(wt, 1),
                 bias=torch.as_tensor(b, dtype=torch.float32).to(self.device).contiguous(),
                 cin=wt.shape[2], cout=wt.shape[3])
+            if tuple(wt.shape) == (3, 3, 3, 64):
+                self.params[name]["grey_fwd"], self.params[name]["grey_dgrad"] = ops.grey_conv1_pack(wt)
         self.names = list(weights.keys())
 
     def plan(self, upto):
@@ -98,7 +101,11 @@
                 raise KeyError("no weights for %s" % name)
         return plan
 
-    def forward(self, x, upto, on_layer=None, keep=None):
+    def takes_grey(self):
+        name, kind = self.seq[0][0], self.seq[0][1]
+        return kind == "conv" and "grey_fwd" in self.params.get(name, {})
+
+    def forward(self, x, upto, on_layer=None, keep=None, grey=None):
         acts = _Activations()
         cur = x
         plan = self.plan(upto)
@@ -108,8 +115,16 @@
             if kind == "conv":
                 p = self.params[name]
                 nxt_pool = li + 1 < len(plan) and plan[li + 1][1] == "pool"
+                below_conv = li > 0 and plan[li - 1][1] == "conv"
+                if li == 0 and grey is not None:
+                    assert x is None, "forward(grey=) forms the loss-net input itself"
+                    cur, acts.gmax = ops.grey_conv1_fwd(grey[0], grey[1], p["grey_fwd"], p["bias"], relu=True,
+                                                        gmax=grey[2] if len(grey) > 2 else None)
+                    acts[name] = cur
+                    if on_layer is not None:
+                        on_layer(name, cur)
+                    continue
                 B_, H_, W_ = cur.shape[0], cur.shape[1], cur.shape[2]
-                below_conv = li > 0 and plan[li - 1][1] == "conv"
                 if nxt_pool and cin % 32 == 0 and cur.shape[1] >= 2 and cur.shape[2] >= 2:
                     rb = ops.conv3x3_relu_bits(B_, H_, W_, cin, cout, True, cur.device) if below_conv else None
                     want_y = rb is None or keep is None or name in keep
@@ -139,7 +154,7 @@
         nxt_pool = i + 2 < len(self.seq) and self.seq[i + 2][1] == "pool"
         return ops.conv3x3_relu_bits_words(B, h, w, cin, cout, nxt_pool) > 0
 
-    def backward(self, acts, style_grads, upto, unmasked=()):
+    def backward(self, acts, style_grads, upto, unmasked=(), to_first=False):
         assert upto not in unmasked, "the top layer's gradient enters the chain directly: it must be masked"
         plan = self.plan(upto)
         g = style_grads[upto]
@@ -160,7 +175,7 @@
             if kind == "conv":
                 p = self.params[name]
                 if below is None:
-                    return ops.conv3x3_dgrad(g, p["dgrad"], cin)
+                    return g if to_first else ops.conv3x3_dgrad(g, p["dgrad"], cin)
                 bname, bkind = below[0], below[1]
                 if bkind == "conv":
                     g = ops.conv3x3_dgrad(g, p["dgrad"], cin, x_in=acts[bname], addend=style_grads.get(bname),
```

After: 436.1. -2.2%, worse.
